# Bernat-C/MRI-Diffusion-SuperResolution

Hardware: AMD Instinct MI355X
Metric: MRI slices/sec (50-step DDIM, 256^2, bs=32) (higher is better)
Workload: dtype bf16; 1 GPU; configs[1]: 256x256 1-ch synthetic MRI slices -> 4x32x32 latents, SD-1.5-size UNet (859.5M params, random init) + rank-4 LoRA, 50-step DDIM, bs=32 per GPU; ddim_steps=50, parallelism=slice-sharded x1 (no collective), lora=explicit adapters, down-projection + rank-r update inside the projection GEMMs, tile_table=profiles/r03_tune_cache.tsv, hipgraph=True

## Files before the change

### include/mrisr.h

```cpp
#ifndef MRISR_H
#define MRISR_H
#include <stddef.h>
#include <stdint.h>

#ifdef __cplusplus
extern "C" {
#endif

typedef enum { MRISR_F32 = 0, MRISR_BF16 = 1, MRISR_F16 = 2, MRISR_I64 = 3 } mrisr_dtype;
typedef enum { MRISR_NCHW = 0, MRISR_NHWC = 1 } mrisr_layout;

typedef struct {
    void* data;
    int32_t dtype;
    int32_t layout;
    int32_t ndim;
    int64_t shape[4];
} mrisr_tensor;

typedef struct {
    int32_t in_channels;
    int32_t out_channels;
    int32_t num_levels;
    int32_t block_out_channels[4];
// ... 246 lines not shown
                        const float* bias_dev, int n, int act, mrisr_tensor* y_rows, void* stream);
int mrisr_op_groupnorm(const mrisr_tensor* x_nhwc, const mrisr_tensor* x2_nhwc, const float* gamma_dev,
                       const float* beta_dev, int groups, float eps, int silu, mrisr_tensor* y_nhwc, void* stream);
int mrisr_op_layernorm(const mrisr_tensor* x_rows, const float* gamma_dev, const float* beta_dev, float eps,
                       mrisr_tensor* y_rows, void* stream);
int mrisr_op_attention(const mrisr_tensor* q, const mrisr_tensor* k, const mrisr_tensor* v, int heads, int flash,
                       mrisr_tensor* out, void* stream);

int mrisr_op_attention_bwd(const mrisr_tensor* q, const mrisr_tensor* k, const mrisr_tensor* v, const mrisr_tensor* dout,
                           int heads, mrisr_tensor* dq, mrisr_tensor* dk, mrisr_tensor* dv, void* stream);

int mrisr_op_groupnorm_bwd(int dtype, const void* x0, int c0, const void* x1, int c1, int B, int HW, const float* gamma_dev,
                           const float* beta_dev, int groups, float eps, int silu, const void* dy, void* dx0, int acc0, void* dx1,
                           int acc1, float* g_gamma, float* g_beta, void* stream);
int mrisr_op_layernorm_bwd(int dtype, const void* x, const void* dy, void* dx, const float* gamma_dev, int M, int C, float eps,
                           int accumulate, float* g_gamma, float* g_beta, void* stream);
int mrisr_op_geglu(int dtype, int backward, const void* pre, const void* dout, void* out, int64_t M, int half, void* stream);
int mrisr_op_pointwise_bwd(int kind, int dtype, const void* a, const void* b, void* out, float* out_f32, int64_t n, int B, int H, int W,
                           int C, int flag, int ld_out, int off, void* stream);
int mrisr_op_lora_wgrad(int dtype, const void* P, int ldp, const float* Q, int ldq, int M, int C, int mode, int r, int nmod, int secN,
                        float* out0, float* out1, float* out2, float scale, void* stream);
int mrisr_op_lora_wgrad_geglu(int dtype, const void* P, int ldp, const float* Q, int ldq, int M, int half, int r, float* out, float scale,
                              void* stream);
int mrisr_op_lora_wgrad_hr(int dtype, const void* P, int ldp, const void* Q, int ldq, int M, int C, int mode, int r, int nmod, int secN,
                           float* out0, float* out1, float* out2, float scale, int geglu_half, void* stream);
int mrisr_op_dora_scale(int dtype, const float* W, const float* A, const float* B, const float* mag, float scale, float* g, void* out, int ld,
                        int n, int k, int r, int geglu_half, int merged, void* stream);
int mrisr_op_dora_mag_grad(int dtype, const void* P, int ldp, const void* Y, int ldy, const void* R, int ldr, const float* bias, const float* mag,
                           float* gm, int M, int C, int geglu_half, void* stream);
int mrisr_op_attn_identity(int dtype, const void* vt, void* out, int B, int H, int N, int hd, int npad, int dpad, int first_sample, int n_samples,
                           void* stream);
int mrisr_op_freeu(int dtype, const void* hidden, const void* skip, void* hidden_out, void* skip_out, int B, int H, int W, int Ch, int Cs,
                   float b, float s, void* stream);
int mrisr_op_transpose(int dtype, const void* src, void* dst, int R, int C, int ld_src, int ld_dst, int64_t bs_src, int64_t bs_dst,
                       int batch, int r_valid, void* stream);
int mrisr_op_softmax_bwd(int dtype, const void* p, const float* dp, void* ds, int ld, int64_t rows, int nk, float scale, void* stream);
int mrisr_op_small_dense_bwd(int dtype, int which, const float* dY, int ldy, const void* xw, int ldx, int rows, int N, int K, int silu_in,
                             const float* pre, int ldpre, float* out, float* gB, int ld_out, void* stream);
int mrisr_op_conv_wgrad(int dtype, const void* x, int xB, int xH, int xW, int cin_src, const void* dY, int ldy, int col0, int cout_src,
                        int ks, int stride, float* gW, float* gB, int cout, int cin, int geglu_half, void* stream);
int mrisr_op_conv_dgrad(int dtype, const void* dy, int B, int H, int W, int cout, const float* w_oihw_dev, int cin, int mode, void* dx,
                        int accumulate, void* stream);
int mrisr_op_conv_lora_down(int dtype, const void* x_nhwc, int B, int H, int W, int cin, const float* a_dev, int r, float* z, int route,
                            void* stream);
int mrisr_op_conv_lora_dgrad(int dtype, const float* dz, int B, int H, int W, int r, const float* a_dev, int cin, void* dx_nhwc, int accumulate,
                             void* stream);
int mrisr_op_conv3x3_lora(const mrisr_tensor* x, const float* w_oihw_dev, const float* bias_dev, const float* a_dev, const float* b_dev, int r,
                          float scale, const float* rowvec_dev, const mrisr_tensor* resid, int cout, int splitk, int tile, mrisr_tensor* y,
                          void* stream);


int mrisr_op_guided_step(int step_kind, mrisr_tensor* x, mrisr_tensor* x2, const mrisr_tensor* eps2, const mrisr_tensor* lr,
                         const mrisr_tensor* noise, const float* coef_row_host, float clip, float guidance_scale,
                         float guidance_rescale, void* stream);

int mrisr_op_pag_step(int step_kind, mrisr_tensor* x, mrisr_tensor* x3, const mrisr_tensor* eps3, const mrisr_tensor* lr,
                      const mrisr_tensor* noise, const float* coef_row_host, float clip, float guidance_scale, float pag_scale,
                      float guidance_rescale, void* stream);

int mrisr_op_pag_multistep_step(int step_kind, mrisr_tensor* x, mrisr_tensor* x3, const mrisr_tensor* eps3, const mrisr_tensor* lr,
                                mrisr_tensor* hist, mrisr_tensor* xc, const float* row_host, int solver_order, int slot, float guidance_scale,
                                float pag_scale, float guidance_rescale, void* stream);

int mrisr_op_multistep_step(int step_kind, mrisr_tensor* x, mrisr_tensor* x2, const mrisr_tensor* eps, const mrisr_tensor* lr,
                            mrisr_tensor* hist, mrisr_tensor* xc, const float* row_host, int solver_order, int slot, float guidance_scale,
                            float guidance_rescale, void* stream);
// ... 10 lines not shown
```

### include/mrisr_debug.h

```cpp
#ifndef MRISR_DEBUG_H
#define MRISR_DEBUG_H
#ifdef __cplusplus
extern "C" {
#endif

void mrisr_debug_force_split(int splitk);
void mrisr_debug_force_tile(int tile);
void mrisr_debug_prefer_tile(int tile);
void mrisr_debug_gemm_flags(int flags);
void mrisr_debug_set_tile_eff(int tile, double eff);
void mrisr_debug_set_tuned(const char* key, int tile, int splitk);
void mrisr_debug_gn_fused(int on);

int mrisr_autotune_stats(int* shapes, double* ms);
void mrisr_autotune_release(void);

int mrisr_bench_gemm(int M, int N, int K, int conv, int B, int H, int W, int stride, int ups, int c1, int tile, int splitk,
                     int iters, float* ms_out);

void mrisr_debug_sk_inkernel(int on);

void mrisr_debug_subpix(int min_rows);

void mrisr_debug_temb_table(int on);

void mrisr_debug_mlp_proj(int on);

void mrisr_debug_gn_slabs(int on);

void mrisr_debug_sc_fused(int on);

void mrisr_debug_ff_proj_fused(int on);

void mrisr_debug_xattn_tail(int on);
void mrisr_debug_xattn_tail_stamps(void* dev_buf);

int mrisr_bench_mlp(int M, int hidden, int iters, float* ms_out);

#ifdef __cplusplus
}
#endif
#endif
```

### mri-diffusion-superresolution_amd/csrc/capi_ops.hip

```cpp
#include <algorithm>
#include <cmath>
#include <cstring>
#include <memory>
#include <vector>

#include "api.h"
#include "model.h"
#include "train_ops.h"

using namespace mrisr;

namespace {
struct OpScratch {
    std::vector<std::unique_ptr<DevBuf>> bufs;
    void* alloc(size_t bytes, bool zero = false) {
        bufs.emplace_back(new DevBuf());
        if (bufs.back()->reserve(bytes ? bytes : 1, zero)) return nullptr;
        return bufs.back()->p;
    }
};
template <typename T>
int op_gemm_run(OpScratch& sc, hipStream_t st, GemmArgs& g) {
    return gemm_run<T>(g, st, false, [&sc](size_t n) { return sc.alloc(n); });
}
// ... 12 lines not shown
        const int dd = (int)(i % hd);
        const int h = (int)((i / hd) % H);
        const int tok = (int)((i / ((long long)hd * H)) % N);
        const int b = (int)(i / ((long long)hd * H * N));
        const size_t bh = (size_t)b * H + h;
        if (!tr) dst[(bh * npad + tok) * dpad + dd] = x[i];
        else dst[(bh * dpad + dd) * npad + tok] = x[i];
    }
}

template <typename T>
static int op_conv3x3_t(const mrisr_tensor* x, const mrisr_tensor* x2, const float* w, const float* bias, int cout,
                        int stride, int ups, int act, int splitk, mrisr_tensor* y, hipStream_t st) {
    const int B = (int)x->shape[0], C0 = (int)x->shape[1], H = (int)x->shape[2], W = (int)x->shape[3];
    const int C1 = x2 ? (int)x2->shape[1] : 0;
    const int Cin = C0 + C1;
    DevBuf wp, part;
    TRY(wp.reserve((size_t)cout * Cin * 9 * sizeof(T), false));
    TRY(launch_pack_conv3x3<T>(w, wp.p, cout, Cin, 3, st));
    if (!x2 && !ups && Cin % (128 / (int)sizeof(T)) != 0) {
        DirectConvArgs a;
        a.x = x->data; a.w = wp.p; a.bias = bias; a.y = y->data; a.B = B; a.Hin = H; a.Win = W; a.Cin = Cin;
        a.Hout = (H - 1) / stride + 1; a.Wout = (W - 1) / stride + 1; a.Cout = cout; a.ks = 3; a.stride = stride; a.pad = 1; a.act = act;
        MRISR_REQUIRE(y->shape[1] == cout && y->shape[2] == a.Hout && y->shape[3] == a.Wout, "conv output shape");
        TRY(launch_direct_conv<T>(a, st));
        MRISR_CHECK_HIP(hipStreamSynchronize(st));
        return 0;
    }
    if (ups == 2) {
        MRISR_REQUIRE(sizeof(T) == 2 && !x2 && stride == 1 && act == ACT_NONE && (4 * Cin) % 64 == 0 && cout % 8 == 0, "sub-pixel upsample conv: bf16, single source");
        MRISR_REQUIRE(y->shape[1] == cout && y->shape[2] == 2 * H && y->shape[3] == 2 * W, "conv output shape");
        DevBuf sp, planes;
        TRY(sp.reserve((size_t)16 * cout * Cin * sizeof(T), false));
        TRY(planes.reserve((size_t)4 * B * H * W * cout * sizeof(T), false));
        TRY(launch_pack_conv_subpix<T>(w, sp.p, cout, Cin, st));
        GemmArgs g;
        ga_rows(g, x->data, C0, C0); ga_conv3(g, B, H, W); g.kw = 2; g.subpix = 1;
        ga_batch(g, 4, 0, (long long)cout * 4 * Cin, (long long)B * H * W * cout); ga_weight(g, sp.p, B * H * W, cout, 4 * Cin);
        g.bias = bias; ga_out(g, planes.p, cout);
        TRY(gemm_run<T>(g, st, false, devbuf_alloc(part)));
        TRY(launch_subpix_shuffle<T>(planes.p, y->data, B, H, W, cout, st));
        MRISR_CHECK_HIP(hipStreamSynchronize(st));
        return 0;
    }
    GemmArgs g;
    ga_rows(g, x->data, C0, C0);
    if (x2) ga_rows2(g, x2->data, C1, C1);
    ga_conv3(g, B, H, W, stride, ups);
    MRISR_REQUIRE(y->shape[1] == cout && y->shape[2] == g.Hout && y->shape[3] == g.Wout, "conv output shape");
    ga_weight(g, wp.p, B * g.Hout * g.Wout, cout, 9 * Cin); g.bias = bias; g.act = act; ga_out(g, y->data, cout);
    TRY(op_plan<T>(g, splitk, false, part));
    TRY(launch_gemm<T>(g, st));
    MRISR_CHECK_HIP(hipStreamSynchronize(st));
    return 0;
}

extern "C" void mrisr_debug_force_tile(int t);
struct ForcedTile {
    explicit ForcedTile(int t) { mrisr_debug_force_tile(t); }
    ~ForcedTile() { mrisr_debug_force_tile(0); }
    ForcedTile(const ForcedTile&) = delete;
    ForcedTile& operator=(const ForcedTile&) = delete;
};

static int op_conv3x3_sc_t(const mrisr_tensor* x, const mrisr_tensor* x2, const float* w, const float* bias, const mrisr_tensor* xs,
                           const mrisr_tensor* xs2, const float* w_sc, const float* bias_sc, int cout, int splitk, int tile, int fused,
                           mrisr_tensor* y, hipStream_t st) {
    typedef bf16 T;
    const int B = (int)x->shape[0], C0 = (int)x->shape[1], H = (int)x->shape[2], W = (int)x->shape[3];
    const int C1 = x2 ? (int)x2->shape[1] : 0, Cin = C0 + C1;
    const int S0 = (int)xs->shape[1], S1 = xs2 ? (int)xs2->shape[1] : 0, Cs = S0 + S1;
    MRISR_REQUIRE(xs->shape[0] == B && xs->shape[2] == H && xs->shape[3] == W && (!xs2 || (xs2->shape[0] == B && xs2->shape[2] == H && xs2->shape[3] == W)),
                  "shortcut sources: the conv input's batch and image size");
    MRISR_REQUIRE(y->shape[1] == cout && y->shape[2] == H && y->shape[3] == W, "conv output shape");
// ... 826 lines not shown
    hipStream_t st = (hipStream_t)stream;
    MRISR_REQUIRE(src && dst && R >= 1 && C >= 1 && batch >= 1 && batch <= 65535, "transpose: null / empty operand");
    MRISR_REQUIRE(ld_src >= C && ld_dst >= R && r_valid >= 0 && r_valid <= R, "transpose: pitches cover the rows, r_valid <= R");
    MRISR_REQUIRE(batch == 1 || (bs_src >= (long long)(R - 1) * ld_src + C && bs_dst >= (long long)(C - 1) * ld_dst + R),
                  "transpose: batch strides cover one matrix");
    TRY(BWD_DISPATCH(dtype, launch_transpose, src, dst, R, C, ld_src, ld_dst, (long long)bs_src, (long long)bs_dst, batch, r_valid, st));
    MRISR_CHECK_HIP(hipStreamSynchronize(st));
    return 0;
    API_END
}

int mrisr_op_attn_identity(int dtype, const void* vt, void* out, int B, int H, int N, int hd, int npad, int dpad, int first_sample, int n_samples,
                           void* stream) {
    API_BEGIN
    TRY(bwd_dtype_ok(dtype));
    hipStream_t st = (hipStream_t)stream;
    TRY(BWD_DISPATCH(dtype, launch_attn_identity, vt, out, B, H, N, hd, npad, dpad, first_sample, n_samples, st));
    MRISR_CHECK_HIP(hipStreamSynchronize(st));
    return 0;
    API_END
}

int mrisr_op_freeu(int dtype, const void* hidden, const void* skip, void* hidden_out, void* skip_out, int B, int H, int W, int Ch, int Cs, float b,
                   float s, void* stream) {
    API_BEGIN
    TRY(bwd_dtype_ok(dtype));
    hipStream_t st = (hipStream_t)stream;
    TRY(BWD_DISPATCH(dtype, launch_freeu, hidden, skip, hidden_out, skip_out, B, H, W, Ch, Cs, b, s, st));
    MRISR_CHECK_HIP(hipStreamSynchronize(st));
    return 0;
    API_END
}

int mrisr_op_softmax_bwd(int dtype, const void* p, const float* dp, void* ds, int ld, int64_t rows, int nk, float scale, void* stream) {
    API_BEGIN
    TRY(bwd_dtype_ok(dtype));
    hipStream_t st = (hipStream_t)stream;
    MRISR_REQUIRE(p && dp && ds && rows >= 1 && nk >= 1 && nk <= ld, "softmax backward: null / empty operand, nk <= ld");
    MRISR_REQUIRE(ld % 4 != 0 || ld > 4096 || (al16(p) && al16(dp) && al16(ds)), "softmax backward: aligned rows for the vector kernel");
    TRY(BWD_DISPATCH(dtype, launch_softmax_bwd, p, dp, ds, ld, (long long)rows, nk, scale, st));
    MRISR_CHECK_HIP(hipStreamSynchronize(st));
    return 0;
    API_END
}

int mrisr_op_small_dense_bwd(int dtype, int which, const float* dY, int ldy, const void* xw, int ldx, int rows, int N, int K, int silu_in,
                             const float* pre, int ldpre, float* out, float* gB, int ld_out, void* stream) {
    API_BEGIN
    TRY(bwd_dtype_ok(dtype));
    hipStream_t st = (hipStream_t)stream;
    MRISR_REQUIRE(dY && xw && out && (which == 0 || which == 1), "small dense backward: null operand, which 0 / 1");
    MRISR_REQUIRE(rows >= 1 && rows <= 64 && N >= 1 && K >= 1 && ldy >= N, "small dense backward: 1..64 rows, dY pitch covers N");
    if (which == 0) {
        MRISR_REQUIRE(ldx >= K, "small wgrad: X pitch covers K");
        TRY(launch_small_wgrad(dY, ldy, static_cast<const float*>(xw), ldx, rows, N, K, silu_in ? 1 : 0, out, gB, st));
    } else {
        MRISR_REQUIRE(ld_out >= K && (!pre || ldpre >= K), "small dgrad: dX / pre pitches cover K");
        TRY(BWD_DISPATCH(dtype, launch_small_dgrad, dY, ldy, xw, rows, N, K, pre, ldpre, out, ld_out, st));
    }
    MRISR_CHECK_HIP(hipStreamSynchronize(st));
    return 0;
    API_END
}

int mrisr_op_conv_wgrad(int dtype, const void* x, int xB, int xH, int xW, int cin_src, const void* dY, int ldy, int col0, int cout_src,
                        int ks, int stride, float* gW, float* gB, int cout, int cin, int geglu_half, void* stream) {
// ... 216 lines not shown
```

### mri-diffusion-superresolution_amd/csrc/common.h

```cpp
#pragma once
#include <hip/hip_runtime.h>
#include <stdint.h>
#include <string>

#include "lora_hr.h"

namespace mrisr {

typedef __bf16 bf16;
typedef __attribute__((ext_vector_type(8))) __bf16 bf16x8;
typedef __attribute__((ext_vector_type(4))) __bf16 bf16x4;
typedef __attribute__((ext_vector_type(4))) float f32x4;
typedef __attribute__((ext_vector_type(16))) float f32x16;

enum DType : int { DT_F32 = 0, DT_BF16 = 1, DT_F16 = 2, DT_I64 = 3 };

template <typename T> struct TypeTag;
template <> struct TypeTag<float> { static constexpr int id = DT_F32; };
template <> struct TypeTag<bf16> { static constexpr int id = DT_BF16; };

__device__ __forceinline__ float to_f32(float x) { return x; }
__device__ __forceinline__ float to_f32(bf16 x) { return (float)x; }
template <typename T> __device__ __forceinline__ T from_f32(float x);
template <> __device__ __forceinline__ float from_f32<float>(float x) { return x; }
// ... 38 lines not shown
        hipError_t _e = (expr);                                                                    \
        if (_e != hipSuccess) {                                                                    \
            ::mrisr::set_error(std::string(#expr) + ": " + hipGetErrorString(_e));                 \
            return 1;                                                                              \
        }                                                                                          \
    } while (0)
#define MRISR_REQUIRE(cond, msg)                                                                   \
    do {                                                                                           \
        if (!(cond)) {                                                                             \
            ::mrisr::set_error(std::string("requirement failed: ") + #cond + " - " + (msg));       \
            return 2;                                                                              \
        }                                                                                          \
    } while (0)

enum GemmAct : int { ACT_NONE = 0, ACT_RELU = 1, ACT_SILU = 2, ACT_GEGLU = 3 };
enum GemmOut : int { OUT_ROWS = 0, OUT_HEADS = 1, OUT_F32 = 2, OUT_NONE = 3  };

struct GemmArgs {
    const void* a0 = nullptr;
    const void* a1 = nullptr;
    int c0 = 0, c1 = 0;
    int lda0 = 0, lda1 = 0;
    int conv = 0;
    int B = 0, Hin = 0, Win = 0, Hout = 0, Wout = 0, stride = 1, ups = 0;
    int pad = 1;
    int zstuff = 0;
    const void* s0 = nullptr;
    const void* s1 = nullptr;
    int cs0 = 0, cs1 = 0;
    int lds0 = 0, lds1 = 0;
    const void* w = nullptr;
    int M = 0, N = 0, K = 0;
    int kw = 3, subpix = 0;
    int batch = 1;
    long long a_bs = 0, w_bs = 0;
    int heads = 1;
    long long o_bs = 0, o_hs = 0;
    int splitk = 1;
    float* partial = nullptr;
    unsigned* sk_counters = nullptr;
    int defer_reduce = 0;
    int pretouch = 0;
    float alpha = 1.0f;
    const float* bias = nullptr;
    const float* rowvec = nullptr;
    int rowvec_div = 1, rowvec_ld = 0;
    int act = ACT_NONE;
    const void* resid = nullptr;
    int ldr = 0;
    int out_mode = OUT_ROWS;
    void* out = nullptr;
    int ldo = 0;
    void* sec_ptr[3] = {nullptr, nullptr, nullptr};
    int sec_tr[3] = {0, 0, 0};
    int secC = 0, hd = 0, dpad = 0, ntok = 0, npad = 0, nheads = 0;
    double alg_flops = 0.0, alg_bytes = 0.0;
    int tile = 0;
    int stage_out = 1;
    const float* lora_z = nullptr;
    const float* lora_b = nullptr;
    int lora_r = 0, lora_zld = 0, lora_secN = 1;
    const void* lora_a = nullptr;
    int lora_R = 0;
    float* lora_zout = nullptr;
    const float* ln_gamma = nullptr;
    const float* ln_beta = nullptr;
// ... 17 lines not shown
    const float* ln_gamma = nullptr; const float* ln_beta = nullptr; float ln_eps = 1e-5f;
    const void* w1 = nullptr; const float* b1 = nullptr;
    const void* w2p = nullptr; const float* b2 = nullptr;
    const void* resid = nullptr; int ldr = 0;
    void* out = nullptr; int ldo = 0;
    int C = 0, H = 0, N2 = 0;
    const void* wp = nullptr; const float* bp = nullptr;
    const void* xres = nullptr; int ldxr = 0;
    void* out2 = nullptr; int ldo2 = 0;
};
bool mlp_fused_ok(int C, int H, int N2);
bool mlp_proj_enabled();
int launch_pack_mlp_w2(const void* w2_bf16, void* dst, int N2, int H, hipStream_t st);
int launch_mlp_fused(const MlpArgs& m, hipStream_t st);
struct XTailArgs {
    const void* ao = nullptr; int ldao = 0;
    void* t = nullptr; int ldt = 0;
    int M = 0, ntok = 0;
    const void* w1 = nullptr; const float* b1 = nullptr; const void* a1 = nullptr; const float* lb1 = nullptr;
    const float* ln_g = nullptr; const float* ln_b = nullptr; float ln_eps = 1e-5f;
    const void* wq = nullptr; const float* bq = nullptr; const void* aq = nullptr; const float* lbq = nullptr;
    const void* kvp = nullptr; int nk = 0; float scale = 1.f;
    const void* w2 = nullptr; const float* b2 = nullptr; const void* a2 = nullptr; const float* lb2 = nullptr;
    int lora_r = 0;
};
int xattn_tail_prepare();
bool xattn_tail_enabled();
bool xattn_tail_ok(int C, int heads, int M, int ntok, int nk);
size_t xattn_tail_kv_bytes(int B);
int launch_pack_xattn_kv(const void* kc, const void* vtc, void* dst, int B, int ctx_pad, int dpad, int nk, hipStream_t st);
int launch_xattn_tail(const XTailArgs& x, hipStream_t st);
bool gemm_tile_lora_in_kernel(int tile, int r, int R);
int gemm_rp_tile(const GemmArgs& g);
bool gemm_sc_tail_ok(const GemmArgs& g);
bool sc_fused_enabled();
bool ff_proj_fused_enabled();
int gemm_choose(GemmArgs& g, bool is_bf16);

struct GroupNormArgs {
    const void* x0 = nullptr;
    const void* x1 = nullptr;
    int c0 = 0, c1 = 0;
    int B = 0, HW = 0, groups = 32;
    float eps = 1e-5f;
    const float* gamma = nullptr;
    const float* beta = nullptr;
    int silu = 0;
    void* y = nullptr;
    float* partial = nullptr;
    int nsplit = 1;
};
extern int g_plan_salt;
int groupnorm_nsplit(int B, int HW);
struct GnSlabSrc {
    const float* partial = nullptr;
    int splitk = 1;
    float alpha = 1.f;
    const float* bias = nullptr;
    const float* rowvec = nullptr;
    int rowvec_ld = 0, rowvec_div = 1;
    const void* resid = nullptr;
    int ldr = 0;
    void* raw_out = nullptr;
};
bool groupnorm_slabs_ok(int C, int groups, int HW);
int launch_groupnorm_slabs(const GroupNormArgs& a, const GnSlabSrc& s, hipStream_t st);
bool gn_fused_geometry(int c0, int c1, int groups, int HW, int* slab, int* slots, int* rl, int* nv, int ve = 8);
template <typename T> int launch_groupnorm(const GroupNormArgs& a, hipStream_t st);
template <typename T>
int launch_layernorm(const void* x, void* y, const float* gamma, const float* beta, int M, int C, float eps,
                     hipStream_t st);
template <typename T>
int launch_softmax_rows(const float* s, int ld, void* p, int ldp, long long rows, int nk, hipStream_t st);

struct GroupNormBwdArgs {
    const void* x0 = nullptr;
    const void* x1 = nullptr;
    int c0 = 0, c1 = 0, B = 0, HW = 0, groups = 32;
    float eps = 1e-5f;
    const float* gamma = nullptr;
    const float* beta = nullptr;
    int silu = 0;
    const void* dy = nullptr;
    void* dx0 = nullptr;
    void* dx1 = nullptr;
    int acc0 = 0, acc1 = 0;
    const float* fwd_partial = nullptr;
    float* bwd_partial = nullptr;
    int nsplit = 1;
};
template <typename T> int launch_groupnorm_bwd(const GroupNormBwdArgs& a, hipStream_t st);
template <typename T>
int launch_layernorm_bwd(const void* x, const void* dy, void* dx, const float* gamma, int M, int C, float eps, int accumulate,
                         hipStream_t st);
template <typename T> int launch_geglu_bwd(const void* pre, const void* dout, void* dpre, long long M, int half, hipStream_t st);
template <typename T> int launch_geglu_fwd(const void* pre, void* out, long long M, int half, hipStream_t st);
template <typename T>
int launch_rows_to_heads(const void* x, int ldx, int col_off, void* dst, int B, int N, int H, int hd, int npad, int dpad, hipStream_t st);
// ... 95 lines not shown
    void* dv = nullptr;
    int ldq = 0, ldkv = 0;
    int B = 0, H = 0, nq = 0, nk = 0, npad = 0, nkpad = 0, hd = 0, dpad = 0;
    float scale = 1.0f;
};
int launch_attention_bwd_bf16(const AttnBwdArgs& a, hipStream_t st);
int launch_attention_bwd_prep(const void* dO_rows, const void* O_rows, void* doh, float* dsum, int B, int N, int H, int hd, int npad,
                              int dpad, hipStream_t st);

template <typename T>
int launch_gemv_rows(const float* x, int ldx, const void* w, const float* bias, float* y, int ldy, int rows, int N,
                     int K, int silu_in, hipStream_t st, int f32_inputs = 0);
template <typename T>
int launch_lora_down(const void* x, int ldx, const void* A, float* z, int M, int K, int R, hipStream_t st);
int conv_lora_kpad(int R);
size_t conv_lora_down_scratch_bytes(int M, int cin, int R, int elem_size, int route = 0);
template <typename T>
int launch_conv_lora_down(const void* x, const void* A, float* z, int B, int H, int W, int cin, int R, float* scratch, hipStream_t st, int route = 0);
template <typename T>
int launch_conv_lora_dgrad(const float* dz, const void* A, const void* bank, void* dx, int B, int H, int W, int cin, int R, int accumulate,
                           hipStream_t st);
template <typename T>
int launch_conv_lora_pack(const float* A, const float* Bm, float s, void* Av, void* bank, float* sB, void* sBT, int cin, int cout, int r, hipStream_t st);
template <typename T> int launch_cast_rows(const float* src, void* dst, long long n, hipStream_t st);
int launch_timestep_embedding(const long long* t, int t_is_scalar, float* out, int rows, int dim, hipStream_t st);
int launch_select_row(const float* table, const int* step, int first, float* out, int n, hipStream_t st);
struct DirectConvArgs {
    const void* x = nullptr;
    const void* w = nullptr;
    const float* bias = nullptr;
    void* y = nullptr;
    int B = 0, Hin = 0, Win = 0, Cin = 0, Hout = 0, Wout = 0, Cout = 0, ks = 3, stride = 1, pad = 1, act = 0;
    const void* add = nullptr;
};
template <typename T> int launch_direct_conv(const DirectConvArgs& a, hipStream_t st);
int direct_conv_prepare();
template <typename T>
int launch_nchw_to_nhwc(const void* src, int src_dtype, void* dst, int B, int C, int H, int W, hipStream_t st);
template <typename T>
int launch_nhwc_to_nchw(const void* src, void* dst, int dst_dtype, int B, int C, int H, int W, float scale,
                        hipStream_t st);
template <typename T> int launch_add_inplace(void* x, const void* y, long long n, hipStream_t st);
template <typename T> int launch_scale_inplace(void* p, float s, long long n, hipStream_t st);
template <typename T> int launch_pixel_unshuffle_nchw(const void* src, int src_dtype, void* dst, int B, int C, int H,
                                                      int W, int r, hipStream_t st);
template <typename T>
int launch_pack_rows(const float* src, int rows, int cols, void* dst, int ld_dst, int row_off, int col_off,
                     int row_map, int half, float scale, hipStream_t st);
template <typename T>
int launch_pack_conv3x3(const float* src, void* dst, int Cout, int Cin, int ks, hipStream_t st);
template <typename T>
int launch_pack_conv_subpix(const float* src, void* dst, int Cout, int Cin, hipStream_t st);
template <typename T>
int launch_subpix_shuffle(const void* planes, void* out, int B, int H, int W, int C, hipStream_t st);
template <typename T>
int launch_pack_conv3x3_padded(const float* src, void* dst, int Cout, int Cin, int ks, int Cout_pad, int Cin_pad, hipStream_t st);
int launch_pack_bias_geglu(const float* src, float* dst, int half, hipStream_t st);
int launch_compose_ff_proj(const float* wp, const float* w2, const float* b2, const float* bp, void* dst_bf16, int ld_dst, float* bias_dst,
                           int C, int K4, hipStream_t st);
template <typename T> int launch_fill_zero(void* p, long long n, hipStream_t st);
int launch_quant_rows_fp8(const void* src_bf16, int rows, int cols, void* dst8, float* scales, hipStream_t st);

int launch_ddim_step(float* x, const float* eps, const float* coef_table, const int* step_idx, long long n,
                     hipStream_t st);
int launch_ddpm_step(float* x, const float* eps, const float* noise, const float* coef_table, const int* step_idx, float clip,
                     long long n, hipStream_t st);
int launch_resshift_step(float* x, const float* eps, const float* lr, const float* noise, const float* coef_table,
                         const int* step_idx, long long n, hipStream_t st);
// ... 23 lines not shown
```

### mri-diffusion-superresolution_amd/csrc/gemm.hip

```cpp
#include "common.h"
#include "prof.h"

#include <cstdio>
#include <cstdlib>
#include <cstring>
#include <map>
#include <mutex>
#include <unordered_map>

namespace mrisr {

static void* g_zero_page = nullptr;
static constexpr size_t kZeroPageBytes = 128 * 1024;
const void* zero_page() { return g_zero_page; }
int init_zero_page() {
    if (g_zero_page) return 0;
    MRISR_CHECK_HIP(hipMalloc(&g_zero_page, kZeroPageBytes));
    MRISR_CHECK_HIP(hipMemset(g_zero_page, 0, kZeroPageBytes));
    return 0;
}

typedef const __attribute__((address_space(1))) void* gptr_t;
typedef __attribute__((address_space(3))) void* lptr_t;

// ... 385 lines not shown
    preload_cols<NF>(g, n0 + wn0 + fg * 4, pb);
    if (g.act == ACT_GEGLU) {
#pragma unroll
        for (int i = 0; i < NF; i += 2)
#pragma unroll
            for (int j = 0; j < MF; ++j) {
                const int m = m0 + wm0 + j * 16 + fr;
                const int n = n0 + wn0 + i * 16 + fg * 4;
                if (m < g.M && n < g.N) {
                    float v[4] = {acc[i][j][0], acc[i][j][1], acc[i][j][2], acc[i][j][3]};
                    float vg[4] = {acc[i + 1][j][0], acc[i + 1][j][1], acc[i + 1][j][2], acc[i + 1][j][3]};
                    epilogue4<T>(g, z, m, n, v, vg, nullptr, nullptr, false, true, nullptr, 0, 0, 0, pb[i], pb[i + 1 < NF ? i + 1 : i]);
                }
            }
        return;
    }
#pragma unroll
    for (int i = 0; i < NF; ++i)
#pragma unroll
        for (int j = 0; j < MF; ++j) {
            const int m = m0 + wm0 + j * 16 + fr;
            const int n = n0 + wn0 + i * 16 + fg * 4;
            if (m < g.M && n < g.N) {
                float v[4] = {acc[i][j][0], acc[i][j][1], acc[i][j][2], acc[i][j][3]};
                epilogue4<T>(g, z, m, n, v, nullptr, nullptr, nullptr, false, true, nullptr, 0, 0, 0, pb[i]);
            }
        }
}

template <int BM, int BN, int NT = 256>
__device__ __forceinline__ void copy_out_tile(const GemmArgs& g, const bf16* otile, int pitch, int m0, int n0, int z, bool add_resid) {
    __syncthreads();
    constexpr int CPR = BN / 8;
    bf16* out = reinterpret_cast<bf16*>(g.out) + (size_t)z * g.o_bs;
    const bf16* res = add_resid ? reinterpret_cast<const bf16*>(g.resid) + (size_t)z * g.o_bs : nullptr;
    constexpr int TOTAL = BM * CPR, IT = (TOTAL + NT - 1) / NT, BATCH = IT < 5 ? IT : 5;
    for (int it0 = 0; it0 < IT; it0 += BATCH) {
        bf16x8 rv[BATCH];
#pragma unroll
        for (int u = 0; u < BATCH; ++u) {
            const int idx = (int)threadIdx.x + (it0 + u) * NT;
            const int row = idx / CPR, ch = idx - row * CPR;
            const int m = m0 + row, n = n0 + ch * 8;
            if (res && idx < TOTAL && m < g.M && n + 8 <= g.N) rv[u] = *reinterpret_cast<const bf16x8*>(res + (size_t)m * g.ldr + n);
        }
#pragma unroll
        for (int u = 0; u < BATCH; ++u) {
            const int idx = (int)threadIdx.x + (it0 + u) * NT;
            const int row = idx / CPR, ch = idx - row * CPR;
            const int m = m0 + row, n = n0 + ch * 8;
            if (idx >= TOTAL || m >= g.M || n >= g.N) continue;
            const bf16* src = otile + row * pitch + ch * 8;
            bf16* dst = out + (size_t)m * g.ldo + n;
            if (n + 8 <= g.N) {
                bf16x8 v = *reinterpret_cast<const bf16x8*>(src);
                if (res) {
#pragma unroll
                    for (int e = 0; e < 8; ++e) v[e] = (bf16)((float)v[e] + (float)rv[u][e]);
                }
                *reinterpret_cast<bf16x8*>(dst) = v;
            } else {
                bf16x4 v = *reinterpret_cast<const bf16x4*>(src);
                if (res) {
                    const bf16x4 r = *reinterpret_cast<const bf16x4*>(res + (size_t)m * g.ldr + n);
#pragma unroll
                    for (int e = 0; e < 4; ++e) v[e] = (bf16)((float)v[e] + (float)r[e]);
                }
                *reinterpret_cast<bf16x4*>(dst) = v;
            }
        }
    }
}

template <int BM, int BN>
__device__ __forceinline__ void copy_out_heads(const GemmArgs& g, const bf16* otile, int m0, int n0, bool tr) {
    __syncthreads();
    const int s = n0 / g.secC;
    bf16* base = reinterpret_cast<bf16*>(s == 0 ? g.sec_ptr[0] : (s == 1 ? g.sec_ptr[1] : g.sec_ptr[2]));
    if (!tr) {
        constexpr int CPR = BN / 8, P = BN + 8;
        for (int idx = threadIdx.x; idx < BM * CPR; idx += 256) {
            const int row = idx / CPR, ch = idx - row * CPR;
            const int m = m0 + row, n = n0 + ch * 8;
            if (m >= g.M || n >= g.N) continue;
            const int c = n - s * g.secC, h = c / g.hd, dd = c - h * g.hd;
            const int b = m / g.ntok, tok = m - b * g.ntok;
// ... 2611 lines not shown
#define TILE_PREPARE_HALO(a, b, c, d, e) 0
#define TILE_PREPARE_HALO8(a, b, c, d, e) 0
#define TILE_PREPARE_WS(a, b, c, d, e) 0
#define TILE_PREPARE_RP(a, b, c, d, e) 0
#define X(id, fam, a, b, c, d, e, eff, cand) if (TILE_PREPARE_##fam(a, b, c, d, e)) return 1;
    TILES(X)
#undef X
    if (direct_conv_prepare()) return 1;
    if (xattn_tail_prepare()) return 1;
    return mlp_fused_prepare();
}

static long long tile_count(const GemmArgs& g) { return (long long)((g.M + 63) / 64) * ((g.N + 63) / 64); }
static constexpr int kSkCounters = 16384;
static int g_sk_inkernel = -1;
extern "C" void mrisr_debug_sk_inkernel(int on) { g_sk_inkernel = on; }
static std::mutex g_sk_mu;
static std::unordered_map<hipStream_t, unsigned*> g_sk_map;
static unsigned* sk_counters_for(hipStream_t st) {
    static const int env = [] { const char* e = getenv("MRISR_SK_INKERNEL"); return e ? atoi(e) : 0; }();
    if (g_sk_inkernel < 0 ? !env : !g_sk_inkernel) return nullptr;
    std::lock_guard<std::mutex> lk(g_sk_mu);
    auto it = g_sk_map.find(st);
    if (it != g_sk_map.end()) return it->second;
    hipStreamCaptureStatus cs = hipStreamCaptureStatusNone;
    if (st && (hipStreamIsCapturing(st, &cs) != hipSuccess || cs != hipStreamCaptureStatusNone)) return nullptr;
    unsigned* p = nullptr;
    if (hipMalloc(&p, kSkCounters * sizeof(unsigned)) != hipSuccess) return nullptr;
    if (hipMemset(p, 0, kSkCounters * sizeof(unsigned)) != hipSuccess || hipDeviceSynchronize() != hipSuccess) { (void)hipFree(p); return nullptr; }
    g_sk_map[st] = p;
    return p;
}

template <typename T>
int launch_gemm(const GemmArgs& g_in, hipStream_t st) {
    constexpr bool is_bf16 = sizeof(T) == 2;
    constexpr int BK = 128 / (int)sizeof(T);
    GemmArgs g = g_in;
    MRISR_REQUIRE(g.K % BK == 0, "K must be a multiple of the 128-byte K tile");
    MRISR_REQUIRE(g.N % 4 == 0, "N must be a multiple of 4");
    MRISR_REQUIRE(g.c0 % BK == 0 && g.c1 % BK == 0, "channel extents must be multiples of the K tile");
    MRISR_REQUIRE(g.splitk == 1 || g.partial != nullptr, "split-K needs a partial buffer");
    MRISR_REQUIRE(g.splitk == 1 || g.act != ACT_GEGLU, "GEGLU epilogue cannot be split");
    MRISR_REQUIRE(zero_page() != nullptr, "zero page not initialised");
    if (g.conv) { MRISR_REQUIRE(g.K == g.kw * g.kw * (g.c0 + g.c1) + g.cs0 + g.cs1 && (g.kw == 3 || g.kw == 2), "conv K"); }
    else { MRISR_REQUIRE(g.K == g.c0 + g.c1, "plain K"); }
    if (g.kw != 3 || g.subpix) {
        MRISR_REQUIRE(is_bf16 && g.conv && !g.c1 && g.stride == 1 && !g.ups && !g.zstuff && g.splitk == 1 && (!g.subpix || g.batch == 4),
                      "2 x 2 / sub-pixel conv: bf16 buffer-addressed kernels, single source, stride 1, un-split, four parity batches");
    }
    int tile = g.tile ? g.tile : g_force_tile, s;
    if (!tile) plan(g, is_bf16, g.splitk, &tile, &s);
    tile = tile_for_launch(g, is_bf16, tile);
    const char* why = nullptr;
    MRISR_REQUIRE(tile_admits(g, is_bf16, tile, &why), why);
    static const int stage_env = [] { const char* e = getenv("MRISR_STAGE_OUT"); return e ? atoi(e) : 2; }();
    g.stage_out = stage_env;
    g.dbg = g_gemm_flags;
    {
        static const int on = [] { const char* e = getenv("MRISR_PRETOUCH"); return e ? atoi(e) : 1; }();
        static const long long min_b = [] { const char* e = getenv("MRISR_PRETOUCH_MIN_KB"); return (e ? atoll(e) : 512ll) * 1024; }();
        static const int cap = [] { const char* e = getenv("MRISR_PRETOUCH_CAP"); return e ? atoi(e) : 32; }();
        g.pretouch = (on && is_bf16 && g.batch == 1 && (long long)g.N * g.K * 2 >= min_b) ? cap : 0;
    }
    g.sk_counters = nullptr;
    if (g.splitk > 1 && is_bf16 && !g.defer_reduce && find_tile(tile)->reduces_in_kernel() && !g.cs0) {
        const long long ntiles = tile_count(g) * (long long)g.batch;
        if (ntiles > 0 && ntiles <= kSkCounters) g.sk_counters = sk_counters_for(st);
    }
    int rc = 1;
    switch (tile) {
#define X(id, fam, a, b, c, d, e, eff, cand) case id: rc = TILE_LAUNCH_##fam(a, b, c, d, e)(g, st); break;
        TILES(X)
#undef X
    }
    if (rc) return rc;
    if (g.splitk > 1 && !g.sk_counters && !g.defer_reduce) return launch_splitk_reduce<T>(g, st);
    return 0;
}

template <typename T>
int launch_splitk_reduce(const GemmArgs& g, hipStream_t st) {
    const long long total = (long long)g.M * (g.N / 4);
    int blocks = (int)((total + 255) / 256);
    if (blocks > 4096) blocks = 4096;
    ProfScope ps("splitk_reduce", 0.0, (double)g.batch * g.M * g.N * (4.0 * g.splitk + sizeof(T)), st);
    hipLaunchKernelGGL(splitk_reduce_kernel<T>, dim3(blocks, 1, g.batch), dim3(256), 0, st, g);
    MRISR_CHECK_HIP(hipGetLastError());
    return 0;
}

template int launch_gemm<float>(const GemmArgs&, hipStream_t);
template int launch_gemm<bf16>(const GemmArgs&, hipStream_t);
template int launch_splitk_reduce<float>(const GemmArgs&, hipStream_t);
template int launch_splitk_reduce<bf16>(const GemmArgs&, hipStream_t);

}
```

### mri-diffusion-superresolution_amd/csrc/misc.hip

```cpp
#include "common.h"
#include "prof.h"

namespace mrisr {

__device__ __forceinline__ float wsum(float v) {
#pragma unroll
    for (int o = 32; o > 0; o >>= 1) v += __shfl_xor(v, o);
    return v;
}

template <typename T, int RB>
__global__ __launch_bounds__(256) void gemv_rows_kernel(const float* __restrict__ x, int ldx,
                                                        const T* __restrict__ w, const float* __restrict__ bias,
                                                        float* __restrict__ y, int ldy, int rows, int N, int K,
                                                        int silu_in) {
    constexpr int VE = 16 / (int)sizeof(T);
    const int lane = threadIdx.x & 63;
    const int n = blockIdx.x * 4 + (threadIdx.x >> 6);
    if (n >= N) return;
    for (int r0 = 0; r0 < rows; r0 += RB) {
        float acc[RB];
#pragma unroll
        for (int r = 0; r < RB; ++r) acc[r] = 0.f;
        for (int k = lane * VE; k < K; k += 64 * VE) {
// ... 372 lines not shown
        }
    }
}

__global__ __launch_bounds__(256) void conv_in_mfma_kernel(const DirectConvArgs a) {
    extern __shared__ __attribute__((aligned(16))) char sm_raw[];
    bf16* wl = reinterpret_cast<bf16*>(sm_raw);
    const int OP = a.Cout + 8;
    bf16* ot = wl + (size_t)a.Cout * 40 + (size_t)(threadIdx.x >> 6) * 16 * OP;
    float* bl = reinterpret_cast<float*>(wl + (size_t)a.Cout * 40 + (size_t)4 * 16 * OP);
    const bf16* x = reinterpret_cast<const bf16*>(a.x);
    const bf16* w = reinterpret_cast<const bf16*>(a.w);
    bf16* y = reinterpret_cast<bf16*>(a.y);
    for (int i = threadIdx.x; i < a.Cout * 10; i += 256) {
        const int n = i / 10, j = i - n * 10;
        const uint2 v = j < 9 ? *reinterpret_cast<const uint2*>(w + (size_t)n * 36 + j * 4) : make_uint2(0u, 0u);
        *reinterpret_cast<uint2*>(wl + (size_t)n * 40 + j * 4) = v;
    }
    for (int i = threadIdx.x; i < a.Cout; i += 256) bl[i] = a.bias ? a.bias[i] : 0.f;
    __syncthreads();
    const int lane = threadIdx.x & 63, fr = lane & 15, fg = lane >> 4;
    const int M = a.B * a.Hout * a.Wout;
    const int ngroups = (M + 15) / 16;
    const int NFR = a.Cout / 16, CPR = a.Cout / 8;
    for (int pg = blockIdx.x * 4 + (threadIdx.x >> 6); pg < ngroups; pg += gridDim.x * 4) {
        const int m = pg * 16 + fr;
        bf16x8 af0 = bf16x8{0, 0, 0, 0, 0, 0, 0, 0}, af1 = af0;
        if (m < M) {
            const int ox = m % a.Wout, oy = (m / a.Wout) % a.Hout, b = m / (a.Wout * a.Hout);
            auto tap4 = [&](int t) -> uint2 {
                const int ky = t / 3, kx = t - ky * 3;
                const int iy = oy + ky - 1, ix = ox + kx - 1;
                if (iy < 0 || iy >= a.Hin || ix < 0 || ix >= a.Win) return make_uint2(0u, 0u);
                return *reinterpret_cast<const uint2*>(x + (((size_t)b * a.Hin + iy) * a.Win + ix) * 4);
            };
            const uint2 p0 = tap4(fg * 2), p1 = tap4(fg * 2 + 1);
            af0 = __builtin_bit_cast(bf16x8, make_uint4(p0.x, p0.y, p1.x, p1.y));
            if (fg == 0) {
                const uint2 p8 = tap4(8);
                af1 = __builtin_bit_cast(bf16x8, make_uint4(p8.x, p8.y, 0u, 0u));
            }
        }
        for (int i = 0; i < NFR; ++i) {
            const bf16* wr = wl + (size_t)(i * 16 + fr) * 40;
            const bf16x8 wf0 = *reinterpret_cast<const bf16x8*>(wr + fg * 8);
            bf16x8 wf1 = bf16x8{0, 0, 0, 0, 0, 0, 0, 0};
            if (fg == 0) wf1 = *reinterpret_cast<const bf16x8*>(wr + 32);
            f32x4 acc = f32x4{0.f, 0.f, 0.f, 0.f};
            acc = __builtin_amdgcn_mfma_f32_16x16x32_bf16(wf0, af0, acc, 0, 0, 0);
            acc = __builtin_amdgcn_mfma_f32_16x16x32_bf16(wf1, af1, acc, 0, 0, 0);
            const int n = i * 16 + fg * 4;
            const f32x4 b4 = *reinterpret_cast<const f32x4*>(bl + n);
            bf16x4 ad = bf16x4{0, 0, 0, 0};
            if (a.add && m < M) ad = *reinterpret_cast<const bf16x4*>(reinterpret_cast<const bf16*>(a.add) + (size_t)m * a.Cout + n);
            bf16x4 o;
#pragma unroll
            for (int r = 0; r < 4; ++r) {
                float v = acc[r] + b4[r];
                if (a.act == ACT_SILU) v = silu_f(v);
                else if (a.act == ACT_RELU) v = fmaxf(v, 0.f);
                o[r] = (bf16)(v + (float)ad[r]);
            }
            *reinterpret_cast<bf16x4*>(ot + fr * OP + n) = o;
        }
        asm volatile("s_waitcnt lgkmcnt(0)" ::: "memory");
        __builtin_amdgcn_wave_barrier();
        for (int c = lane; c < 16 * CPR; c += 64) {
            const int row = c / CPR, col = (c - row * CPR) * 8;
            const int mo = pg * 16 + row;
            if (mo >= M) continue;
            *reinterpret_cast<bf16x8*>(y + (size_t)mo * a.Cout + col) = *reinterpret_cast<const bf16x8*>(ot + row * OP + col);
        }
        asm volatile("s_waitcnt lgkmcnt(0)" ::: "memory");
        __builtin_amdgcn_wave_barrier();
    }
}

int direct_conv_prepare() {
    static bool done = false;
    if (!done) {
        MRISR_CHECK_HIP(hipFuncSetAttribute((const void*)conv_in_mfma_kernel, hipFuncAttributeMaxDynamicSharedMemorySize, 80 * 1024));
        done = true;
    }
    return 0;
}

template <typename T>
int launch_direct_conv(const DirectConvArgs& a, hipStream_t st) {
    const size_t wbytes = (size_t)a.ks * a.ks * a.Cin * a.Cout * sizeof(T);
    if (sizeof(T) == 2 && a.ks == 3 && a.Cin == 4 && a.stride == 1 && a.pad == 1 && a.Cout % 16 == 0 && a.Hout == a.Hin && a.Wout == a.Win) {
        const size_t smem = ((size_t)a.Cout * 40 + (size_t)4 * 16 * (a.Cout + 8)) * 2 + (size_t)a.Cout * 4;
        if (smem <= 80 * 1024 && (long long)a.B * a.Hout * a.Wout * a.Cout < (1ll << 31)) {
            if (direct_conv_prepare()) return 1;
            const long long M = (long long)a.B * a.Hout * a.Wout;
            long long blocks = ((M + 15) / 16 + 3) / 4;
            if (blocks > 256) blocks = 256;
            ProfScope ps("conv_in_mfma", 2.0 * M * a.Cout * 36, 2.0 * (M * 4.0 + (double)M * a.Cout), st);
            hipLaunchKernelGGL(conv_in_mfma_kernel, dim3((unsigned)blocks), dim3(256), smem, st, a);
            MRISR_CHECK_HIP(hipGetLastError());
            return 0;
        }
    }
    if (a.Cout % 8 == 0 && wbytes <= 48 * 1024) {
        const long long items = (long long)a.B * a.Hout * a.Wout * (a.Cout / 8);
        long long blocks = (items + 255) / 256;
        if (blocks > 2048) blocks = 2048;
        ProfScope ps("small_conv", 2.0 * items * 8 * a.ks * a.ks * a.Cin,
                     sizeof(T) * ((double)a.B * a.Hin * a.Win * a.Cin + (double)items * 8), st);
        hipLaunchKernelGGL(small_conv_kernel<T>, dim3((unsigned)blocks), dim3(256), wbytes, st, a);
        MRISR_CHECK_HIP(hipGetLastError());
        return 0;
    }
    const long long total = (long long)a.B * a.Hout * a.Wout * a.Cout;
    long long blocks = (total + 255) / 256;
    if (blocks > 65535 * 4) blocks = 65535 * 4;
    ProfScope ps("direct_conv", 2.0 * total * a.ks * a.ks * a.Cin,
                 sizeof(T) * ((double)a.B * a.Hin * a.Win * a.Cin + (double)total), st);
    hipLaunchKernelGGL(direct_conv_kernel<T>, dim3((unsigned)blocks), dim3(256), 0, st, a);
    MRISR_CHECK_HIP(hipGetLastError());
    return 0;
}


__device__ __forceinline__ float load_any(const void* p, int dt, size_t i) {
// ... 340 lines not shown
```

### mri-diffusion-superresolution_amd/csrc/norm.hip

```cpp
#include "common.h"
#include "prof.h"

namespace mrisr {

template <typename T> struct Vec;
template <> struct Vec<bf16> {
    static constexpr int N = 8;
    typedef bf16x8 type;
};
template <> struct Vec<float> {
    static constexpr int N = 4;
    typedef f32x4 type;
};

template <typename T, int VPT>
__global__ __launch_bounds__(256) void gn_stats_kernel(const GroupNormArgs a, int slots, int RL) {
    constexpr int VE = Vec<T>::N;
    typedef typename Vec<T>::type vec_t;
    extern __shared__ float sm[];
    const int C = a.c0 + a.c1;
    const int b = blockIdx.y, sp = blockIdx.x;
    const int tid = threadIdx.x;
    const int slot = tid % slots, rl = tid / slots;
    const int rows_per = (a.HW + a.nsplit - 1) / a.nsplit;
// ... 133 lines not shown
template <int NVM, int VE, bool SLAB = false, int NT = 256>
__global__ __launch_bounds__(NT) void gn_fused_kernel(const GroupNormArgs a, int slab, int slots, int RL, int nslab, int xcd_map, const GnSlabSrc ss = GnSlabSrc()) {
    typedef bf16 T;
    typedef __attribute__((ext_vector_type(VE))) __bf16 vec_t;
    __shared__ float part[NT * 16];
    __shared__ float seg[2 * 1280];
    __shared__ double gsum[2 * 80];
    __shared__ float mean_s[80], rstd_s[80];
    const int C = a.c0 + a.c1;
    const int Cg = C / a.groups;
    int b, sl;
    if (xcd_map) {
        const int L = blockIdx.x;
        b = (L & 7) + 8 * (L / (8 * nslab));
        sl = (L >> 3) % nslab;
    } else {
        b = blockIdx.x / nslab;
        sl = blockIdx.x - b * nslab;
    }
    const int ch0 = sl * slab;
    const int tid = threadIdx.x;
    const int slot = tid % slots, rl = tid / slots;
    const bool active = rl < RL;
    const int ch = ch0 + slot * VE;
    const T* src;
    int ld;
    if (ch < a.c0) { src = reinterpret_cast<const T*>(a.x0) + (size_t)b * a.HW * a.c0 + ch; ld = a.c0; }
    else { src = reinterpret_cast<const T*>(a.x1) + (size_t)b * a.HW * a.c1 + (ch - a.c0); ld = a.c1; }
    vec_t xv[NVM];
    float s1[VE], s2[VE];
#pragma unroll
    for (int e = 0; e < VE; ++e) s1[e] = s2[e] = 0.f;
    if (active) {
        if constexpr (SLAB) {
            typedef __attribute__((ext_vector_type(VE))) float fvec_t;
            const size_t MN = (size_t)a.B * a.HW * C;
            fvec_t bv;
#pragma unroll
            for (int e = 0; e < VE; ++e) bv[e] = 0.f;
            if (ss.bias) bv = *reinterpret_cast<const fvec_t*>(ss.bias + ch);
#pragma unroll
            for (int i = 0; i < NVM; ++i) {
                const int r = rl + i * RL;
                if (r < a.HW) {
                    const size_t mrow = (size_t)b * a.HW + r;
                    const float* pp = ss.partial + mrow * C + ch;
                    fvec_t v;
#pragma unroll
                    for (int e = 0; e < VE; ++e) v[e] = 0.f;
                    for (int sp = 0; sp < ss.splitk; ++sp) {
                        const fvec_t t = *reinterpret_cast<const fvec_t*>(pp + (size_t)sp * MN);
#pragma unroll
                        for (int e = 0; e < VE; ++e) v[e] += t[e];
                    }
#pragma unroll
                    for (int e = 0; e < VE; ++e) v[e] = v[e] * ss.alpha + bv[e];
                    if (ss.rowvec) {
                        const fvec_t t = *reinterpret_cast<const fvec_t*>(ss.rowvec + (mrow / ss.rowvec_div) * ss.rowvec_ld + ch);
#pragma unroll
                        for (int e = 0; e < VE; ++e) v[e] += t[e];
                    }
                    if (ss.resid) {
                        const vec_t t = *reinterpret_cast<const vec_t*>(reinterpret_cast<const T*>(ss.resid) + mrow * ss.ldr + ch);
#pragma unroll
                        for (int e = 0; e < VE; ++e) v[e] += (float)t[e];
                    }
#pragma unroll
                    for (int e = 0; e < VE; ++e) xv[i][e] = (bf16)v[e];
                    if (ss.raw_out) *reinterpret_cast<vec_t*>(reinterpret_cast<T*>(ss.raw_out) + mrow * C + ch) = xv[i];
                }
            }
        } else {
#pragma unroll
        for (int i = 0; i < NVM; ++i) {
            const int r = rl + i * RL;
            if (r < a.HW) xv[i] = *reinterpret_cast<const vec_t*>(src + (size_t)r * ld);
        }
        }
#pragma unroll
        for (int i = 0; i < NVM; ++i) {
            if (rl + i * RL < a.HW) {
#pragma unroll
                for (int e = 0; e < VE; ++e) {
                    const float f = (float)xv[i][e];
                    s1[e] += f;
                    s2[e] += f * f;
                }
            }
        }
    }
#pragma unroll
    for (int e = 0; e < VE; ++e) {
        part[tid * 16 + e] = s1[e];
        part[tid * 16 + 8 + e] = s2[e];
    }
    __syncthreads();
    const int nout = 2 * slab;
    int nseg = NT / nout;
    if (nseg < 1) nseg = 1;
    if (nseg > RL) nseg = RL;
    const int seg_len = (RL + nseg - 1) / nseg;
    for (int t = tid; t < nout * nseg; t += NT) {
// ... 167 lines not shown
            }
#undef GN_GO
            MRISR_CHECK_HIP(hipGetLastError());
            return 0;
        }
    }
    {
    ProfScope ps(prof_intern(n1), 0.0, act_bytes, st);
    switch (vpt) {
        case 1: hipLaunchKernelGGL((gn_stats_kernel<T, 1>), grid, dim3(256), smem, st, a, slots, RL); break;
        case 2: hipLaunchKernelGGL((gn_stats_kernel<T, 2>), grid, dim3(256), smem, st, a, slots, RL); break;
        case 3: hipLaunchKernelGGL((gn_stats_kernel<T, 3>), grid, dim3(256), smem, st, a, slots, RL); break;
        default: hipLaunchKernelGGL((gn_stats_kernel<T, 4>), grid, dim3(256), smem, st, a, slots, RL); break;
    }
    }
    MRISR_CHECK_HIP(hipGetLastError());
    int bx = 1024 / (a.B > 0 ? a.B : 1) + 1;
    int rows_per_block = (a.HW + bx - 1) / bx;
    if (rows_per_block < RL) rows_per_block = RL;
    bx = (a.HW + rows_per_block - 1) / rows_per_block;
    ProfScope ps2(prof_intern(n2), 0.0, 2.0 * act_bytes, st);
    switch (vpt) {
        case 1: hipLaunchKernelGGL((gn_apply_kernel<T, 1>), dim3(bx, a.B), dim3(256), 0, st, a, slots, RL, rows_per_block); break;
        case 2: hipLaunchKernelGGL((gn_apply_kernel<T, 2>), dim3(bx, a.B), dim3(256), 0, st, a, slots, RL, rows_per_block); break;
        case 3: hipLaunchKernelGGL((gn_apply_kernel<T, 3>), dim3(bx, a.B), dim3(256), 0, st, a, slots, RL, rows_per_block); break;
        default: hipLaunchKernelGGL((gn_apply_kernel<T, 4>), dim3(bx, a.B), dim3(256), 0, st, a, slots, RL, rows_per_block); break;
    }
    MRISR_CHECK_HIP(hipGetLastError());
    return 0;
}

static int g_gn_slabs = -1;
extern "C" void mrisr_debug_gn_slabs(int on) { g_gn_slabs = on; ++g_plan_salt; }
static bool gn_slabs_geometry(int C, int groups, int HW, int B, int* ve, int* slab, int* slots, int* rl, int* nv) {
    if (!gn_fused_geometry(C, 0, groups, HW, slab, slots, rl, nv, 8)) return false;
    *ve = 8;
    int s4 = 0, sl4 = 0, rl4 = 0, nv4 = 0;
    if (B * (C / *slab) < 512 && gn_fused_geometry(C, 0, groups, HW, &s4, &sl4, &rl4, &nv4, 4) && C / s4 > C / *slab) {
        *ve = 4; *slab = s4; *slots = sl4; *rl = rl4; *nv = nv4;
    }
    return *nv <= 8;
}
bool groupnorm_slabs_ok(int C, int groups, int HW) {
    static const int env = [] { const char* e = getenv("MRISR_GN_SLABS"); return e ? atoi(e) : 1; }();
    if (g_gn_slabs < 0 ? !env : !g_gn_slabs) return false;
    if (C % groups || groups > 64 || C % 8) return false;
    int ve, slab, slots, rl, nv;
    return gn_slabs_geometry(C, groups, HW, 32, &ve, &slab, &slots, &rl, &nv);
}
int launch_groupnorm_slabs(const GroupNormArgs& a, const GnSlabSrc& s, hipStream_t st) {
    const int C = a.c0;
    MRISR_REQUIRE(a.c1 == 0 && a.x1 == nullptr && C % a.groups == 0 && a.groups <= 64 && C % 8 == 0, "GroupNorm from slabs: one source, whole groups");
    MRISR_REQUIRE(s.partial && s.splitk >= 1 && a.partial != nullptr && a.nsplit >= 1 && (!s.rowvec || s.rowvec_div >= 1) && (!s.resid || s.ldr % 8 == 0), "GroupNorm from slabs: operands");
    int ve, slab, slots, rl, nv;
    MRISR_REQUIRE(gn_slabs_geometry(C, a.groups, a.HW, a.B, &ve, &slab, &slots, &rl, &nv), "GroupNorm from slabs: geometry (groupnorm_slabs_ok)");
    const int nslab = C / slab;
    const int xmap = (a.B % 8) == 0 ? 1 : 0;
    std::string nf = "groupnorm_from_slabs";
    if (prof_enabled() && prof_shapes()) {
        char buf[96];
        snprintf(buf, sizeof(buf), " B=%d HW=%d C=%d s=%d", a.B, a.HW, C, s.splitk);
        nf += buf;
    }
    const double act_bytes = (double)a.B * a.HW * C * 2.0;
    ProfScope ps(prof_intern(nf), 0.0, act_bytes * (2.0 * s.splitk + 1.0 + (s.raw_out ? 1.0 : 0.0) + (s.resid ? 1.0 : 0.0)), st);
    const dim3 fg(a.B * nslab);
#define GNS_GO(NV, VEV) hipLaunchKernelGGL((gn_fused_kernel<NV, VEV, true>), fg, dim3(256), 0, st, a, slab, slots, rl, nslab, xmap, s)
    if (ve == 8) { if (nv <= 2) GNS_GO(2, 8); else if (nv <= 4) GNS_GO(4, 8); else GNS_GO(8, 8); }
    else { if (nv <= 2) GNS_GO(2, 4); else if (nv <= 4) GNS_GO(4, 4); else GNS_GO(8, 4); }
#undef GNS_GO
    MRISR_CHECK_HIP(hipGetLastError());
    return 0;
}

__device__ __forceinline__ float wave_sum(float v) {
#pragma unroll
    for (int o = 32; o > 0; o >>= 1) v += __shfl_xor(v, o);
    return v;
}
__device__ __forceinline__ float wave_max(float v) {
#pragma unroll
    for (int o = 32; o > 0; o >>= 1) v = fmaxf(v, __shfl_xor(v, o));
    return v;
}

template <typename T, int MAXV>
__global__ __launch_bounds__(256) void layernorm_kernel(const T* __restrict__ x, T* __restrict__ y,
                                                        const float* __restrict__ gamma,
                                                        const float* __restrict__ beta, int M, int C, float eps) {
    constexpr int VE = Vec<T>::N;
    typedef typename Vec<T>::type vec_t;
    const int lane = threadIdx.x & 63;
    const int row = blockIdx.x * 4 + (threadIdx.x >> 6);
    if (row >= M) return;
    const int nvec = C / VE;
    float v[MAXV][VE];
    float s = 0.f;
#pragma unroll
// ... 228 lines not shown
```

### mri-diffusion-superresolution_amd/csrc/runner.h

```cpp
#pragma once
#include <climits>
#include <cmath>
#include <cstdlib>

#include "api.h"
#include "gemm_args.h"
#include "model.h"

namespace mrisr {

extern int g_subpix_override;

inline bool fuse_ln() {
    static int v = -1;
    if (v < 0) { const char* e = getenv("MRISR_FUSE_LN"); v = (e && e[0] == '0') ? 0 : 1; }
    return v == 1;
}
inline bool lora_in_kernel() {
    static int v = -1;
    if (v < 0) { const char* e = getenv("MRISR_LORA_INKERNEL"); v = (e && e[0] == '0') ? 0 : 1; }
    return v == 1;
}

template <typename T>
struct Runner {
    Model& m;
    hipStream_t st;
    bool dry;
    Runner(Model& mm, hipStream_t s, bool d) : m(mm), st(s), dry(d) {}

    void* alloc(size_t bytes) {
        void* p = m.arena.alloc(bytes);
        if (!p) set_error("workspace arena exhausted");
        return p;
    }
    Act new_act(int B, int H, int W, int C) {
        Act a;
        a.B = B; a.H = H; a.W = W; a.C = C;
        a.p = alloc(a.numel() * sizeof(T));
        return a;
    }

    int gn(const Act& x0, const Act* x1, const NormW& nw, bool silu, float eps, Act* out, float** partial_out = nullptr,
           int* nsplit_out = nullptr) {
        const int C = x0.C + (x1 ? x1->C : 0);
        MRISR_REQUIRE(nw.c == C, "GroupNorm channel mismatch");
        *out = new_act(x0.B, x0.H, x0.W, C);
        GroupNormArgs a;
        a.x0 = x0.p; a.c0 = x0.C;
        a.x1 = x1 ? x1->p : nullptr; a.c1 = x1 ? x1->C : 0;
        a.B = x0.B; a.HW = x0.H * x0.W; a.groups = m.cfg.norm_num_groups; a.eps = eps;
        a.gamma = nw.g; a.beta = nw.b; a.silu = silu ? 1 : 0; a.y = out->p;
        a.nsplit = groupnorm_nsplit(a.B, a.HW);
        a.partial = static_cast<float*>(alloc((size_t)a.B * a.nsplit * a.groups * 2 * sizeof(float)));
        if (!out->p || !a.partial) return 7;
        if (partial_out) *partial_out = a.partial;
        if (nsplit_out) *nsplit_out = a.nsplit;
        if (dry) return 0;
        return launch_groupnorm<T>(a, st);
    }

    auto arena_alloc() { return [this](size_t n) { return alloc(n); }; }
    int run_gemm(GemmArgs& g) { return gemm_run<T>(g, st, dry, arena_alloc()); }

    int conv3(const Act& x, const Act* x1, const ConvW& cw, int stride, int ups, const float* rowvec, int rowvec_ld,
              int rowvec_div, const Act* resid, int act, Act* out, const float* lz = nullptr) {
        const int Cin = x.C + (x1 ? x1->C : 0);
        MRISR_REQUIRE(cw.cin == Cin && cw.ks == 3, "conv3x3 weight mismatch");
        GemmArgs g = conv3_args(x, x1, cw, stride, ups, rowvec, rowvec_ld, rowvec_div, resid, act);
        *out = new_act(x.B, g.Hout, g.Wout, cw.cout);
        if (!out->p) return 7;
        g.out = out->p;
        if (lz) ga_lora_epilogue(g, cw, lz);
        return run_gemm(g);
    }
    static GemmArgs conv3_args(const Act& x, const Act* x1, const ConvW& cw, int stride, int ups, const float* rowvec, int rowvec_ld,
                               int rowvec_div, const Act* resid, int act) {
        GemmArgs g;
        ga_rows(g, x); ga_rows2(g, x1); ga_conv3(g, x, stride, ups);
        ga_weight(g, cw.w, x.B * g.Hout * g.Wout, cw.cout, 9 * (x.C + (x1 ? x1->C : 0))); g.bias = cw.b; g.act = act;
        ga_rowvec(g, rowvec, rowvec_ld, rowvec_div); ga_resid(g, resid); g.ldo = cw.cout;
        return g;
    }
    int conv_lora_z(const Act& x, const ConvW& cw, float** z) {
        MRISR_REQUIRE(cw.r && cw.loraA && cw.loraB && x.C == cw.cin, "conv LoRA: adapter views");
        const int M = (int)x.rows();
        *z = static_cast<float*>(alloc((size_t)M * cw.r * sizeof(float)));
        const size_t sb = conv_lora_down_scratch_bytes(M, x.C, cw.r, (int)sizeof(T));
        float* scr = sb ? static_cast<float*>(alloc(sb)) : nullptr;
        if (!*z || (sb && !scr)) return 7;
        if (dry) return 0;
        return launch_conv_lora_down<T>(x.p, cw.loraA, *z, x.B, x.H, x.W, x.C, cw.r, scr, st);
    }

    int conv3_gn(const Act& x, const Act* x1, const ConvW& cw, const float* rowvec, int rowvec_ld, int rowvec_div, const Act* resid,
                 const NormW& nw, bool silu, float eps, Act* raw, Act* out) {
        const int Cin = x.C + (x1 ? x1->C : 0);
        MRISR_REQUIRE(cw.cin == Cin && cw.ks == 3 && nw.c == cw.cout, "conv3x3 + GroupNorm weight mismatch");
        GemmArgs g = conv3_args(x, x1, cw, 1, 0, rowvec, rowvec_ld, rowvec_div, resid, ACT_NONE);
        bool fuse = sizeof(T) == 2 && !m.keep && groupnorm_slabs_ok(cw.cout, m.cfg.norm_num_groups, x.H * x.W);
        if (fuse) {
            g.out = kUnallocated;
            TRY(gemm_choose(g, true));
            fuse = g.splitk > 1;
        }
        if (!fuse) {
            Act h;
            TRY(conv3(x, x1, cw, 1, 0, rowvec, rowvec_ld, rowvec_div, resid, ACT_NONE, &h));
            if (raw) *raw = h;
            return gn(h, nullptr, nw, silu, eps, out);
        }
        Act h;
        h.B = x.B; h.H = x.H; h.W = x.W; h.C = cw.cout; h.p = nullptr;
        if (raw) { h = new_act(x.B, x.H, x.W, cw.cout); if (!h.p) return 7; *raw = h; }
        *out = new_act(x.B, x.H, x.W, cw.cout);
        if (!out->p) return 7;
        GroupNormArgs a;
        a.x0 = nullptr; a.c0 = cw.cout; a.B = x.B; a.HW = x.H * x.W; a.groups = m.cfg.norm_num_groups; a.eps = eps;
        a.gamma = nw.g; a.beta = nw.b; a.silu = silu ? 1 : 0; a.y = out->p;
        a.nsplit = groupnorm_nsplit(a.B, a.HW);
        a.partial = static_cast<float*>(alloc((size_t)a.B * a.nsplit * a.groups * 2 * sizeof(float)));
        TRY(gemm_alloc_partial(g, arena_alloc()));
        if (!a.partial) return 7;
        if (dry) return 0;
        g.defer_reduce = 1;
        TRY(launch_gemm<T>(g, st));
        GnSlabSrc ss;
        ss.partial = g.partial; ss.splitk = g.splitk; ss.alpha = g.alpha; ss.bias = g.bias; ss.rowvec = g.rowvec; ss.rowvec_ld = g.rowvec_ld;
        ss.rowvec_div = g.rowvec_div; ss.resid = g.resid; ss.ldr = g.ldr; ss.raw_out = h.p;
        return launch_groupnorm_slabs(a, ss, st);
    }

    static int subpix_min_rows() {
        static const int v = [] { const char* e = getenv("MRISR_SUBPIX"); return e ? atoi(e) : 2048; }();
        return g_subpix_override >= 0 ? g_subpix_override : v;
    }
    int upsample_conv(const Act& x, const Level& lv, Act* out) {
        const int minr = subpix_min_rows();
        if (!(sizeof(T) == 2 && lv.up_sp && !m.keep && minr > 0 && (long long)x.rows() >= minr))
            return conv3(x, nullptr, lv.up, 1, 1, nullptr, 0, 1, nullptr, ACT_NONE, out);
        const ConvW& cw = lv.up;
        MRISR_REQUIRE(cw.cin == x.C, "upsampler weight mismatch");
        *out = new_act(x.B, 2 * x.H, 2 * x.W, cw.cout);
        if (!out->p) return 7;
        const size_t mk = m.arena.mark();
        const long long plane = (long long)x.rows() * cw.cout;
        T* planes = static_cast<T*>(alloc((size_t)4 * plane * sizeof(T)));
        if (!planes) return 7;
        GemmArgs g;
        ga_rows(g, x); ga_conv3(g, x); g.kw = 2; g.subpix = 1; ga_batch(g, 4, 0, (long long)cw.cout * 4 * cw.cin, plane);
        ga_weight(g, lv.up_sp, (int)x.rows(), cw.cout, 4 * x.C); g.bias = cw.b; ga_out(g, planes, cw.cout);
        g.alg_flops = 2.0 * 4.0 * g.M * (double)g.N * g.K;
        TRY(run_gemm(g));
        if (!dry) TRY(launch_subpix_shuffle<T>(planes, out->p, x.B, x.H, x.W, cw.cout, st));
        m.arena.release(mk);
        return 0;
    }

    int linear(const void* x, int M, int lda, const LinW& lw, int act, const void* resid, int ldr, GemmArgs* custom,
               void* out, int ldo, float** z_out = nullptr, const NormW* ln = nullptr, void* ln_scratch = nullptr) {
        GemmArgs g = custom ? *custom : GemmArgs();
        const size_t mk = m.arena.mark();
        ga_rows(g, x, lw.k, lda); ga_weight(g, lw.w, M, lw.n, lw.k); g.alg_flops = 2.0 * M * (double)lw.n * (lw.k + lw.r);
        g.bias = lw.b; g.act = act; ga_resid(g, resid, ldr);
        if (g.out_mode != OUT_HEADS) ga_out(g, out, ldo);
        if (lw.R && !(lw.r == 4 && lw.R <= 16 && lora_in_kernel())) g.no_rp = 1;
        if (lw.w8 && sizeof(T) == 2 && (!m.keep || m.cfg.fp8_train) && !g.no_rp) {
            GemmArgs probe = g;
            probe.w8 = lw.w8; probe.w_scale = lw.w_scale;
            if (lw.R) { probe.lora_a = lw.loraA; probe.lora_b = lw.loraB; probe.lora_r = lw.r; probe.lora_R = lw.R; probe.lora_a8 = lw.loraA8; probe.lora_a_scale = lw.loraA_scale; }
            if (gemm_rp_tile(probe)) { g.w8 = lw.w8; g.w_scale = lw.w_scale; g.lora_a8 = lw.loraA8; g.lora_a_scale = lw.loraA_scale; }
        }
        if (ln) {
            MRISR_REQUIRE(ln->c == lw.k && lda == lw.k, "LayerNorm width vs the projection's K");
            GemmArgs probe = g;
            if (lw.R) { probe.lora_a = lw.loraA; probe.lora_b = lw.loraB; probe.lora_r = lw.r; probe.lora_R = lw.R; }
            if (sizeof(T) == 2 && !m.keep && fuse_ln() && (!lw.R || (lw.R <= 16 && lora_in_kernel())) && gemm_rp_tile(probe)) {
                g.ln_gamma = ln->g; g.ln_beta = ln->b; g.ln_eps = 1e-5f;
            } else {
                MRISR_REQUIRE(ln_scratch, "LayerNorm scratch rows");
                TRY(layernorm(x, *ln, M, lw.k, ln_scratch));
                g.a0 = x = ln_scratch;
            }
        }
        if (!lw.R) {
// ... 51 lines not shown
        TRY(conv3(t->xn, nullptr, r.c1, 1, 0, m.tproj_out + r.temb_off, m.tproj_total, div, nullptr, ACT_NONE, &t->h, t->z1));
        TRY(gn(t->h, nullptr, r.n2, true, m.cfg.norm_eps, &t->hn, &t->p2, &t->ns2));
        Act res = x;
        if (r.has_sc) {
            GemmArgs g = resnet_shortcut_args(x, x1, r.sc.w, r.sc.b, r.cin, r.cout, o.p);
            TRY(run_gemm(g));
            res = o;
        } else {
            MRISR_REQUIRE(!x1, "concat input requires a shortcut conv");
        }
        if (r.c2.r) TRY(conv_lora_z(t->hn, r.c2, &t->z2));
        GemmArgs g = resnet_conv2_args(t->hn.p, x.B, x.H, x.W, r.cout, r.c2.w, r.c2.b, res.p, o.p);
        if (t->z2) ga_lora_epilogue(g, r.c2, t->z2);
        return run_gemm(g);
    }

    int resnet(const ResW& r, const Act& x, const Act* x1, Act* out, const NormW* next = nullptr, float next_eps = 0.f, Act* next_out = nullptr) {
        Act o = new_act(x.B, x.H, x.W, r.cout);
        if (!o.p) return 7;
        if (next_out) next_out->p = nullptr;
        if (r.c1.r || r.c2.r) {
            const size_t mk0 = m.arena.mark();
            ResTape t;
            TRY(resnet_literal(r, x, x1, o, &t));
            if (!m.keep) m.arena.release(mk0);
            *out = o;
            return 0;
        }
        GemmArgs g2;
        bool fuse2 = false;
        GroupNormArgs a2;
        GemmArgs gt = resnet_conv2_args(kUnallocated, x.B, x.H, x.W, r.cout, r.c2sc, r.b2sc, nullptr, o.p, r.cin, &x, x1);
        const bool sc_tail = sizeof(T) == 2 && !m.keep && r.has_sc && r.c2sc && sc_fused_enabled() && x.C + (x1 ? x1->C : 0) == r.cin && gemm_sc_tail_ok(gt);
        if (next && next_out && sizeof(T) == 2 && !m.keep && next->c == r.cout && groupnorm_slabs_ok(r.cout, m.cfg.norm_num_groups, x.H * x.W)) {
            g2 = sc_tail ? gt
                         : resnet_conv2_args(kUnallocated, x.B, x.H, x.W, r.cout, r.c2.w, r.c2.b, kUnallocated, kUnallocated);
            TRY(gemm_choose(g2, true));
            fuse2 = g2.splitk > 1;
            if (fuse2) {
                *next_out = new_act(x.B, x.H, x.W, r.cout);
                a2.nsplit = groupnorm_nsplit(x.B, x.H * x.W);
                a2.partial = static_cast<float*>(alloc((size_t)x.B * a2.nsplit * m.cfg.norm_num_groups * 2 * sizeof(float)));
                if (!next_out->p || !a2.partial) return 7;
            }
        }
        const size_t mk = m.arena.mark();
        Act xn, h, hn;
        TRY(gn(x, x1, r.n1, true, m.cfg.norm_eps, &xn));
        const int div = m.t_scalar ? INT_MAX : x.H * x.W;
        TRY(conv3_gn(xn, nullptr, r.c1, m.tproj_out + r.temb_off, m.tproj_total, div, nullptr, r.n2, true, m.cfg.norm_eps, nullptr, &hn));
        Act res = x;
        if (sc_tail) {
            res.p = nullptr;
        } else if (r.has_sc) {
            GemmArgs g = resnet_shortcut_args(x, x1, r.sc.w, r.sc.b, r.cin, r.cout, o.p);
            MRISR_REQUIRE(r.sc.R == 0, "shortcut has no LoRA");
            TRY(run_gemm(g));
            res = o;
        } else {
            MRISR_REQUIRE(!x1, "concat input requires a shortcut conv");
        }
        if (fuse2) {
            g2.a0 = hn.p; g2.resid = res.p; g2.out = o.p;
            TRY(gemm_alloc_partial(g2, arena_alloc()));
            if (!dry) {
                g2.defer_reduce = 1;
                TRY(launch_gemm<T>(g2, st));
                a2.x0 = nullptr; a2.c0 = r.cout; a2.B = x.B; a2.HW = x.H * x.W; a2.groups = m.cfg.norm_num_groups; a2.eps = next_eps;
                a2.gamma = next->g; a2.beta = next->b; a2.silu = 0; a2.y = next_out->p;
                GnSlabSrc ss;
                ss.partial = g2.partial; ss.splitk = g2.splitk; ss.alpha = g2.alpha; ss.bias = g2.bias; ss.resid = res.p; ss.ldr = r.cout; ss.raw_out = o.p;
                TRY(launch_groupnorm_slabs(a2, ss, st));
            }
        } else if (sc_tail) {
            gt.a0 = hn.p;
            TRY(run_gemm(gt));
        } else {
            GemmArgs g = resnet_conv2_args(hn.p, x.B, x.H, x.W, r.cout, r.c2.w, r.c2.b, res.p, o.p);
            TRY(run_gemm(g));
        }
        if (!m.keep) m.arena.release(mk);
        *out = o;
        return 0;
    }

    static AttnGeom attn_geom(const HeadBuf& hb, int nk, int nkpad) {
        AttnGeom s;
        s.B = hb.B; s.H = hb.H; s.N = hb.N; s.npad = hb.npad; s.hd = hb.hd; s.dpad = hb.dpad; s.nk = nk; s.nkpad = nkpad;
        return s;
    }
    int attention(const HeadBuf& hb, const void* k, const void* vt, int nk, int nkpad, void* out_rows) {
        const AttnGeom s = attn_geom(hb, nk, nkpad);
        const size_t mk = m.arena.mark();
        if (m.cfg.flash_attention && sizeof(T) == 2) {
            const bool fp8 = m.cfg.fp8_attention;
            AttnArgs a;
            TRY(attn_flash_args(a, s, hb.q, k, vt, out_rows, nullptr, fp8, arena_alloc()));
            const int rc = attn_flash_launch(a, fp8, dry, st);
            if (!m.keep) m.arena.release(mk);
            return rc;
        }
        const size_t cnt = (size_t)s.B * s.H * s.N * nkpad;
        float* S = static_cast<float*>(alloc(cnt * sizeof(float)));
        if (!S) return 7;
        void* P = S;
        if (sizeof(T) == 2) {
// ... 27 lines not shown
    void heads_args(GemmArgs* g, const HeadBuf& hb, void* s0, int tr0, void* s1, int tr1, void* s2, int tr2, int ntok,
                    int npad) {
        g->out_mode = OUT_HEADS;
        g->sec_ptr[0] = s0; g->sec_ptr[1] = s1; g->sec_ptr[2] = s2;
        g->sec_tr[0] = tr0; g->sec_tr[1] = tr1; g->sec_tr[2] = tr2;
        g->secC = hb.H * hb.hd; g->hd = hb.hd; g->dpad = hb.dpad; g->ntok = ntok; g->npad = npad; g->nheads = hb.H;
    }

    int project_context(XfW& x, const HeadBuf& hb) {
        GemmArgs g;
        heads_args(&g, hb, x.kc, 0, x.vtc, 1, nullptr, 0, m.ctx_len, m.ctx_pad);
        TRY(linear(m.ctx_rows, m.ws_B * m.ctx_len, m.cfg.cross_attention_dim, x.kv2, ACT_NONE, nullptr, 0, &g,
                   nullptr, 0));
        if (x.kvp && !dry && m.ctx_len <= 80 && hb.hd == 40 && sizeof(T) == 2)
            TRY(launch_pack_xattn_kv(x.kc, x.vtc, x.kvp, m.ws_B, m.ctx_pad, hb.dpad, m.ctx_len, st));
        return 0;
    }

    bool fused_middle(const XfW& xw, const HeadBuf& hb, int M) const {
        if (sizeof(T) != 2 || m.keep || !xw.q2p || !xw.kvp || !xattn_tail_enabled() || m.cfg.fp8_attention || !m.cfg.flash_attention) return false;
        if (!xattn_tail_ok(xw.C, hb.H, M, hb.N, m.ctx_len) || hb.hd != 40) return false;
        const int R = xw.out1.R;
        if (xw.q2.R != R || xw.out2.R != R) return false;
        if (R && !(R == 4 && xw.out1.r == 4 && xw.q2.r == 4 && xw.out2.r == 4 && lora_in_kernel())) return false;
        if (xw.out1.w8 || xw.q2.w8 || xw.out2.w8) return false;
        return true;
    }

    int transformer(XfW& xw, const Act& x, Act* out, const Act* pre_normed = nullptr) {
        const int C = xw.C, M = (int)x.rows();
        const HeadBuf& hb = m.head_buf(x.H * x.W, C);
        Act o = new_act(x.B, x.H, x.W, C);
        if (!o.p) return 7;
        const size_t mk = m.arena.mark();
        Act xn;
        if (pre_normed && pre_normed->p) xn = *pre_normed;
        else TRY(gn(x, nullptr, xw.norm, false, 1e-6f, &xn));
        T* t = static_cast<T*>(alloc((size_t)M * C * sizeof(T)));
        T* nrm = static_cast<T*>(alloc((size_t)M * C * sizeof(T)));
        T* ao = static_cast<T*>(alloc((size_t)M * C * sizeof(T)));
        if (!t || !nrm || !ao) return 7;
        TRY(linear(xn.p, M, C, xw.proj_in, ACT_NONE, nullptr, 0, nullptr, t, C));
        {
            GemmArgs g;
            heads_args(&g, hb, hb.q, 0, hb.k, 0, hb.vt, 1, hb.N, hb.npad);
            TRY(linear(t, M, C, xw.qkv, ACT_NONE, nullptr, 0, &g, nullptr, 0, nullptr, &xw.ln1, nrm));
        }
        TRY(self_attention(xw, hb, ao));
        if (fused_middle(xw, hb, M)) {
            XTailArgs a;
            a.ao = ao; a.ldao = C; a.t = t; a.ldt = C; a.M = M; a.ntok = hb.N;
            a.w1 = xw.out1.w; a.b1 = xw.out1.b; a.a1 = xw.out1.loraA; a.lb1 = xw.out1.loraB;
            a.ln_g = xw.ln2.g; a.ln_b = xw.ln2.b; a.ln_eps = 1e-5f;
            a.wq = xw.q2p; a.bq = xw.q2.b; a.aq = xw.q2.loraA; a.lbq = xw.q2.loraB;
            a.kvp = xw.kvp; a.nk = m.ctx_len; a.scale = 1.0f / sqrtf((float)hb.hd);
            a.w2 = xw.out2p; a.b2 = xw.out2.b; a.a2 = xw.out2.loraA; a.lb2 = xw.out2.loraB;
            a.lora_r = xw.out1.R ? 4 : 0;
            if (!dry) TRY(launch_xattn_tail(a, st));
        } else {
        TRY(linear(ao, M, C, xw.out1, ACT_NONE, t, C, nullptr, t, C));
        {
            GemmArgs g;
            heads_args(&g, hb, hb.q, 0, nullptr, 0, nullptr, 0, hb.N, hb.npad);
            TRY(linear(t, M, C, xw.q2, ACT_NONE, nullptr, 0, &g, nullptr, 0, nullptr, &xw.ln2, nrm));
        }
        TRY(attention(hb, xw.kc, xw.vtc, m.ctx_len, m.ctx_pad, ao));
        TRY(linear(ao, M, C, xw.out2, ACT_NONE, t, C, nullptr, t, C));
        }
        bool proj_done = false;
        if (xw.ff2p && !m.keep && mlp_fused_ok(C, 4 * C, C)) {
            MlpArgs a;
            a.x = t; a.ldx = C; a.M = M; a.ln_gamma = xw.ln3.g; a.ln_beta = xw.ln3.b; a.ln_eps = 1e-5f;
            a.w1 = xw.ff1.w; a.b1 = xw.ff1.b; a.w2p = xw.ff2p; a.b2 = xw.ff2.b;
            a.resid = t; a.ldr = C; a.out = t; a.ldo = C; a.C = C; a.H = 4 * C; a.N2 = C;
            if (xw.proj_outp && M % 128 == 0 && mlp_proj_enabled()) {
                a.wp = xw.proj_outp; a.bp = xw.proj_out.b; a.xres = x.p; a.ldxr = C; a.out2 = o.p; a.ldo2 = C;
                proj_done = true;
            }
            if (!dry) TRY(launch_mlp_fused(a, st));
        } else {
            T* ff = static_cast<T*>(alloc((size_t)M * 4 * C * sizeof(T)));
            if (!ff) return 7;
            if (xw.ff1.R) {
                T* pre = static_cast<T*>(alloc((size_t)M * 8 * C * sizeof(T)));
                if (!pre) return 7;
                TRY(linear(t, M, C, xw.ff1, ACT_NONE, nullptr, 0, nullptr, pre, 8 * C, nullptr, &xw.ln3, nrm));
                if (!dry) TRY(launch_geglu_fwd<T>(pre, ff, M, 4 * C, st));
            } else {
                TRY(linear(t, M, C, xw.ff1, ACT_GEGLU, nullptr, 0, nullptr, ff, 4 * C, nullptr, &xw.ln3, nrm));
            }
            if (sizeof(T) == 2 && !m.keep && xw.ffpo && !xw.ff2.R && !xw.proj_out.R && ff_proj_fused_enabled()) {
                GemmArgs g;
                ga_rows(g, ff, 4 * C, 4 * C); ga_rows2(g, t, C, C); ga_weight(g, xw.ffpo, M, C, 5 * C); g.bias = xw.bffpo;
                ga_resid(g, x.p, C); ga_out(g, o.p, C);
                g.no_rp = 1;
                g.alg_flops = 2.0 * M * (double)C * (5 * C);
                TRY(run_gemm(g));
                proj_done = true;
            } else {
                TRY(linear(ff, M, 4 * C, xw.ff2, ACT_NONE, t, C, nullptr, t, C));
            }
        }
        if (!proj_done) TRY(linear(t, M, C, xw.proj_out, ACT_NONE, x.p, C, nullptr, o.p, C));
        if (!m.keep) m.arena.release(mk);
        *out = o;
        return 0;
    }

    int time_embed(const long long* t_dev, int t_scalar, int B) {
        const int rows = t_scalar ? 1 : B;
        const int c0 = m.cfg.block_out_channels[0], temb = 4 * c0;
        float* s = static_cast<float*>(alloc((size_t)rows * c0 * sizeof(float)));
        float* y1 = static_cast<float*>(alloc((size_t)rows * temb * sizeof(float)));
        float* emb = static_cast<float*>(alloc((size_t)rows * temb * sizeof(float)));
        m.tproj_out = static_cast<float*>(alloc((size_t)rows * m.tproj_total * sizeof(float)));
        if (!s || !y1 || !emb || !m.tproj_out) return 7;
        m.t_scalar = t_scalar;
        m.te_s = s; m.te_y1 = y1; m.te_emb = emb;
        if (dry) return 0;
        if (m.tproj_table && t_scalar && !m.keep)
            return launch_select_row(m.tproj_table, m.tproj_step, m.tproj_first, m.tproj_out, m.tproj_total, st);
        TRY(launch_timestep_embedding(t_dev, t_scalar, s, rows, c0, st));
        TRY(launch_gemv_rows<T>(s, c0, m.te1.w, m.te1.b, y1, temb, rows, temb, c0, 0, st));
        TRY(launch_gemv_rows<T>(y1, temb, m.te2.w, m.te2.b, emb, temb, rows, temb, temb, 1, st));
        TRY(launch_gemv_rows<T>(emb, temb, m.tproj.w, m.tproj.b, m.tproj_out, m.tproj_total, rows, m.tproj_total, temb, 1, st));
        return 0;
    }

    int time_embed_table(const long long* ts_dev, int rows, float* scratch, float* table) {
        const int c0 = m.cfg.block_out_channels[0], temb = 4 * c0;
        for (int r0 = 0; r0 < rows; r0 += 64) {
            const int nr = std::min(64, rows - r0);
            float* s = scratch;
            float* y1 = s + (size_t)64 * c0;
            float* emb = y1 + (size_t)64 * temb;
            TRY(launch_timestep_embedding(ts_dev + r0, 0, s, nr, c0, st));
            TRY(launch_gemv_rows<T>(s, c0, m.te1.w, m.te1.b, y1, temb, nr, temb, c0, 0, st));
            TRY(launch_gemv_rows<T>(y1, temb, m.te2.w, m.te2.b, emb, temb, nr, temb, temb, 1, st));
            TRY(launch_gemv_rows<T>(emb, temb, m.tproj.w, m.tproj.b, table + (size_t)r0 * m.tproj_total, m.tproj_total, nr, m.tproj_total, temb, 1, st));
        }
        return 0;
    }

    int direct(const Act& x, const ConvW& cw, int stride, int act, const Act* add, Act* out) {
        const int pad = cw.ks / 2;
        const int Ho = (x.H + 2 * pad - cw.ks) / stride + 1, Wo = (x.W + 2 * pad - cw.ks) / stride + 1;
        *out = new_act(x.B, Ho, Wo, cw.cout);
        if (!out->p) return 7;
        MRISR_REQUIRE(cw.cin == x.C, "direct conv channel mismatch");
        DirectConvArgs a;
        a.x = x.p; a.w = cw.w; a.bias = cw.b; a.y = out->p; a.B = x.B; a.Hin = x.H; a.Win = x.W; a.Cin = x.C;
        a.Hout = Ho; a.Wout = Wo; a.Cout = cw.cout; a.ks = cw.ks; a.stride = stride; a.pad = pad; a.act = act;
        a.add = add ? add->p : nullptr;
        if (dry) return 0;
        return launch_direct_conv<T>(a, st);
    }

    int import_act(const mrisr_tensor& t, Act* out, bool copy_if_nhwc) {
        MRISR_REQUIRE(t.ndim == 4, "expected a 4-D tensor");
        const int B = (int)t.shape[0], C = (int)t.shape[1], H = (int)t.shape[2], W = (int)t.shape[3];
        if (t.layout == MRISR_NHWC) {
            MRISR_REQUIRE(t.dtype == m.cfg.compute_dtype, "NHWC tensors must be in the compute dtype");
            if (!copy_if_nhwc) {
                out->p = t.data; out->B = B; out->H = H; out->W = W; out->C = C;
                return 0;
            }
        }
        *out = new_act(B, H, W, C);
        if (!out->p) return 7;
        if (dry) return 0;
        if (t.layout == MRISR_NHWC) {
            MRISR_CHECK_HIP(hipMemcpyAsync(out->p, t.data, out->numel() * sizeof(T), hipMemcpyDeviceToDevice, st));
            return 0;
        }
        return launch_nchw_to_nhwc<T>(t.data, t.dtype, out->p, B, C, H, W, st);
    }
    int export_act(const Act& a, const mrisr_tensor& t, float scale) {
        MRISR_REQUIRE(t.ndim == 4 && t.shape[0] == a.B && t.shape[1] == a.C && t.shape[2] == a.H && t.shape[3] == a.W,
                      "output tensor shape mismatch");
        if (dry) return 0;
        if (t.layout == MRISR_NHWC) {
            MRISR_REQUIRE(t.dtype == m.cfg.compute_dtype && scale == 1.0f, "NHWC outputs: compute dtype, scale 1");
            MRISR_CHECK_HIP(hipMemcpyAsync(t.data, a.p, a.numel() * sizeof(T), hipMemcpyDeviceToDevice, st));
            return 0;
        }
        return launch_nhwc_to_nchw<T>(a.p, t.data, t.dtype, a.B, a.C, a.H, a.W, scale, st);
    }
    int add_external(Act& x, const mrisr_tensor& t) {
        const size_t mk = m.arena.mark();
        Act r;
        TRY(import_act(t, &r, false));
        MRISR_REQUIRE(r.B == x.B && r.C == x.C && r.H == x.H && r.W == x.W, "residual shape mismatch");
        if (!dry) TRY(launch_add_inplace<T>(x.p, r.p, (long long)x.numel(), st));
        if (!m.keep) m.arena.release(mk);
        return 0;
    }

    int encoder(Act x, const mrisr_tensor* intrablock, int n_intra, std::vector<Act>* skips, Act* out, int last_skip = -1) {
        skips->push_back(x);
        int ib = 0;
        auto done = [&] { return last_skip >= 0 && (int)skips->size() > last_skip; };
        for (int i = 0; i < m.cfg.num_levels && !done(); ++i) {
            Level& lv = m.down[i];
            const bool has_attn = !lv.xf.empty();
            const int block_last = (int)skips->size() - 1 + (int)lv.res.size() + (lv.has_down ? 1 : 0);
            for (size_t j = 0; j < lv.res.size() && !done(); ++j) {
                Act y, xn_next;
                xn_next.p = nullptr;
                if (has_attn) TRY(resnet(lv.res[j], x, nullptr, &y, &lv.xf[j].norm, 1e-6f, &xn_next));
                else TRY(resnet(lv.res[j], x, nullptr, &y));
                x = y;
                if (has_attn) {
                    TRY(transformer(lv.xf[j], x, &y, &xn_next));
                    x = y;
                    if (j + 1 == lv.res.size() && ib < n_intra) TRY(add_external(x, intrablock[ib++]));
                }
                skips->push_back(x);
            }
            if (lv.has_down && !done()) {
                Act y;
                TRY(conv3(x, nullptr, lv.down, 2, 0, nullptr, 0, 1, nullptr, ACT_NONE, &y));
                x = y;
                skips->push_back(x);
            }
            if (!has_attn && ib < n_intra && (last_skip < 0 || last_skip >= block_last)) {
                TRY(add_external(x, intrablock[ib++]));
            }
        }
        *out = x;
        return 0;
    }
    int mid(Act x, Act* out) {
        Act y, xn_next;
        xn_next.p = nullptr;
        TRY(resnet(m.mid_r0, x, nullptr, &y, &m.mid_xf.norm, 1e-6f, &xn_next));
        x = y;
        TRY(transformer(m.mid_xf, x, &y, &xn_next));
        x = y;
        TRY(resnet(m.mid_r1, x, nullptr, &y));
        *out = y;
        return 0;
    }

    int set_context(const mrisr_tensor& ehs) {
        MRISR_REQUIRE(ehs.ndim == 3 && ehs.shape[2] == m.cfg.cross_attention_dim, "encoder_hidden_states shape");
        MRISR_REQUIRE((int)ehs.shape[0] == m.ws_B && (int)ehs.shape[1] == m.ctx_len, "context shape vs planned workspace");
        if (!dry) TRY(launch_nchw_to_nhwc<T>(ehs.data, ehs.dtype, m.ctx_rows, m.ws_B * m.ctx_len, m.cfg.cross_attention_dim, 1, 1, st));
        auto each = [&](XfW& x) -> int { return project_context(x, m.head_buf_for_C(x.C)); };
        for (auto& lv : m.down) for (auto& x : lv.xf) TRY(each(x));
        TRY(each(m.mid_xf));
        for (auto& lv : m.up) for (auto& x : lv.xf) TRY(each(x));
        m.ctx_valid = true;
        return 0;
    }

    int freeu(const Act& x, const Act& sk, float b, float s) {
        MRISR_REQUIRE(!m.keep, "FreeU: not while a training forward is being recorded");
        MRISR_REQUIRE(x.B == sk.B && x.H == sk.H && x.W == sk.W, "FreeU: hidden and skip geometry differ");
        MRISR_REQUIRE(x.C % 16 == 0 && sk.C % 8 == 0, "FreeU: hidden channels must be a multiple of 16, skip channels of 8");
        if (dry) return 0;
        return launch_freeu<T>(x.p, sk.p, x.p, sk.p, x.B, x.H, x.W, x.C, sk.C, b, s, st);
    }

    int unet_forward(const mrisr_tensor& sample, const long long* t_dev, int t_scalar, const mrisr_tensor* ehs,
                     const mrisr_tensor* down_res, int n_down, const mrisr_tensor* mid_res,
                     const mrisr_tensor* intrablock, int n_intra, const mrisr_tensor& out, const UNetCache& fc = UNetCache()) {
        m.arena.reset();
        const int B = (int)sample.shape[0];
        const bool store = fc.mode == CACHE_STORE, use = fc.mode == CACHE_USE;
        const int q0 = m.num_skips() - 1 - fc.depth;
        if (store || use) {
            MRISR_REQUIRE(q0 >= 0 && fc.depth >= 1 && fc.p, "feature cache: depth 1 .. num_skips - 1 and a buffer");
            MRISR_REQUIRE(n_down == 0 && !mid_res, "a feature cache together with ControlNet residuals is not supported");
        }
        if (ehs) TRY(set_context(*ehs));
        MRISR_REQUIRE(dry || m.ctx_valid, "no encoder_hidden_states given and none cached");
        TRY(time_embed(t_dev, t_scalar, B));
        Act s, x;
        TRY(import_act(sample, &s, false));
        TRY(direct(s, m.conv_in, 1, ACT_NONE, nullptr, &x));
        std::vector<Act> skips;
        TRY(encoder(x, intrablock, n_intra, &skips, &x, use ? fc.depth : -1));
        if (n_down > 0) {
            MRISR_REQUIRE(n_down == (int)skips.size(), "down_block_additional_residuals count");
            for (int k = 0; k < n_down; ++k) {
                if (skips[k].p == x.p) {
                    Act c = new_act(x.B, x.H, x.W, x.C);
                    if (!c.p) return 7;
                    if (!dry) MRISR_CHECK_HIP(hipMemcpyAsync(c.p, x.p, x.numel() * sizeof(T), hipMemcpyDeviceToDevice, st));
                    skips[k] = c;
                }
                TRY(add_external(skips[k], down_res[k]));
            }
        }
        if (!use) TRY(mid(x, &x));
        if (mid_res) TRY(add_external(x, *mid_res));
        int q = 0;
        for (int i = 0; i < m.cfg.num_levels; ++i) {
            Level& lv = m.up[i];
            for (size_t j = 0; j < lv.res.size(); ++j, ++q) {
                if (use && q < q0) continue;
                if ((store || use) && q == q0) {
                    int64_t cs[4];
                    TRY(m.cache_shape(fc.depth, B, (int)sample.shape[2], (int)sample.shape[3], cs));
                    if (store) {
                        MRISR_REQUIRE(x.B == cs[0] && x.C == cs[1] && x.H == cs[2] && x.W == cs[3], "feature cache shape");
                        if (!dry) MRISR_CHECK_HIP(hipMemcpyAsync(fc.p, x.p, x.numel() * sizeof(T), hipMemcpyDeviceToDevice, st));
                    } else {
                        x.p = fc.p; x.B = (int)cs[0]; x.C = (int)cs[1]; x.H = (int)cs[2]; x.W = (int)cs[3];
                    }
                }
                Act sk = skips.back();
                skips.pop_back();
                if (m.freeu.on && i < 2) TRY(freeu(x, sk, m.freeu.b[i], m.freeu.s[i]));
                Act y, xn_next;
                xn_next.p = nullptr;
                if (!lv.xf.empty()) TRY(resnet(lv.res[j], x, &sk, &y, &lv.xf[j].norm, 1e-6f, &xn_next));
                else TRY(resnet(lv.res[j], x, &sk, &y));
                x = y;
                if (!lv.xf.empty()) {
                    TRY(transformer(lv.xf[j], x, &y, &xn_next));
                    x = y;
                }
            }
            if (lv.has_up && !(use && q <= q0)) {
                Act y;
                TRY(upsample_conv(x, lv, &y));
                x = y;
            }
        }
        Act xn, y;
        TRY(gn(x, nullptr, m.norm_out, true, m.cfg.norm_eps, &xn));
        if (m.conv_out.cout % 4 == 0) TRY(conv3(xn, nullptr, m.conv_out, 1, 0, nullptr, 0, 1, nullptr, ACT_NONE, &y));
        else TRY(direct(xn, m.conv_out, 1, ACT_NONE, nullptr, &y));
        return export_act(y, out, 1.0f);
    }

    int set_cond(const mrisr_tensor& cond) {
        const size_t mk = m.arena.mark();
        Act e, y;
        TRY(import_act(cond, &e, false));
        for (size_t k = 0; k < m.ce.size(); ++k) {
            const bool last = k + 1 == m.ce.size();
            const int act = last ? ACT_NONE : ACT_SILU;
            constexpr int KQ = 128 / (int)sizeof(T);
            if (e.C % KQ == 0 && m.ce[k].cout % 4 == 0) TRY(conv3(e, nullptr, m.ce[k], m.ce_stride[k], 0, nullptr, 0, 1, nullptr, act, &y));
            else TRY(direct(e, m.ce[k], m.ce_stride[k], act, nullptr, &y));
            e = y;
        }
        MRISR_REQUIRE(e.numel() * sizeof(T) <= m.cond_emb_bytes, "condition embedding larger than planned");
        if (!dry) MRISR_CHECK_HIP(hipMemcpyAsync(m.cond_emb, e.p, e.numel() * sizeof(T), hipMemcpyDeviceToDevice, st));
        if (!m.keep) m.arena.release(mk);
        m.cond_valid = true;
        return 0;
    }

    int controlnet_forward(const mrisr_tensor& sample, const long long* t_dev, int t_scalar, const mrisr_tensor* ehs,
                           const mrisr_tensor* cond, float scale, mrisr_tensor* down_out, int n_down,
                           mrisr_tensor* mid_out) {
        m.arena.reset();
        const int B = (int)sample.shape[0];
        if (ehs) TRY(set_context(*ehs));
        if (cond) TRY(set_cond(*cond));
        MRISR_REQUIRE(dry || (m.ctx_valid && m.cond_valid), "context / condition image neither given nor cached");
        TRY(time_embed(t_dev, t_scalar, B));
        Act s, x;
        TRY(import_act(sample, &s, false));
        Act ce;
        ce.p = m.cond_emb; ce.B = B; ce.H = s.H; ce.W = s.W; ce.C = m.cfg.block_out_channels[0];
        TRY(direct(s, m.conv_in, 1, ACT_NONE, &ce, &x));
        std::vector<Act> skips;
        TRY(encoder(x, nullptr, 0, &skips, &x));
        TRY(mid(x, &x));
        MRISR_REQUIRE(n_down == (int)skips.size(), "ControlNet output count");
        for (int k = 0; k < n_down; ++k) {
            const size_t mk = m.arena.mark();
            Act o = new_act(skips[k].B, skips[k].H, skips[k].W, skips[k].C);
            if (!o.p) return 7;
            TRY(linear(skips[k].p, (int)skips[k].rows(), skips[k].C, m.cn_down[k], ACT_NONE, nullptr, 0, nullptr, o.p, o.C));
            TRY(export_act(o, down_out[k], scale));
            if (!m.keep) m.arena.release(mk);
        }
        Act o = new_act(x.B, x.H, x.W, x.C);
        if (!o.p) return 7;
        TRY(linear(x.p, (int)x.rows(), x.C, m.cn_mid, ACT_NONE, nullptr, 0, nullptr, o.p, o.C));
        return export_act(o, *mid_out, scale);
    }
};

}
```

### mri-diffusion-superresolution_amd/csrc/runtime.h

```cpp
#pragma once
#include <cstdint>
#include <map>
#include <memory>
#include <string>
#include <vector>

#include "../../include/mrisr.h"
#include "common.h"

namespace mrisr {

struct DevBuf {
    void* p = nullptr;
    size_t bytes = 0;
    DevBuf() = default;
    DevBuf(const DevBuf&) = delete;
    DevBuf& operator=(const DevBuf&) = delete;
    ~DevBuf() { release(); }
    void release() {
        if (p) (void)hipFree(p);
        p = nullptr;
        bytes = 0;
    }
    int reserve(size_t n, bool zero) {
// ... 54 lines not shown
    void* loraAd = nullptr;
    float* loraB = nullptr;
    void* loraBT = nullptr;
    long long offLA = -1, offLB = -1;
};
struct LinW {
    void* w = nullptr;
    const float* b = nullptr;
    int n = 0, k = 0;
    int geglu_half = 0;
    int r = 0, R = 0, secN = 1;
    int rp = 0;
    int kw() const { return rp ? k + R : k; }
    void* loraA = nullptr;
    const float* loraB = nullptr;
    void* w8 = nullptr;
    float* w_scale = nullptr;
    void* loraA8 = nullptr;
    float* loraA_scale = nullptr;
    std::vector<std::string> mod_names;
    std::vector<int> mod_lora;
    std::vector<long long> offA, offB;
    void* wT = nullptr;
    void* loraBT = nullptr;
    float* loraAT = nullptr;
    float* loraB_rw = nullptr;
    float* dora_g = nullptr;
    std::vector<long long> offM;
};

struct Act {
    void* p = nullptr;
    int B = 0, H = 0, W = 0, C = 0;
    size_t rows() const { return (size_t)B * H * W; }
    size_t numel() const { return rows() * C; }
};

inline int dtype_size(int dt) { return dt == MRISR_F32 ? 4 : (dt == MRISR_I64 ? 8 : 2); }

int tile_axis(int n, int t, int o, int window, std::vector<int>& origins, std::vector<float>& weights);
struct TilePlan {
    int H = 0, W = 0, th = 0, tw = 0;
    std::vector<int> oy, ox;
    std::vector<float> nwy, nwx;
    std::vector<uint32_t> words;
    size_t off_nwy = 0, off_nwx = 0;
    int T() const { return (int)(oy.size() * ox.size()); }
    int build(int H_, int W_, int tile_h, int tile_w, int overlap_h, int overlap_w, int window);
    int check();
    void pack();
    size_t bytes() const { return words.size() * sizeof(uint32_t); }
    TileGrid grid(const void* dev) const;
};

}
```

### mri-diffusion-superresolution_amd/csrc/sampler.hip

```cpp
#include <algorithm>
#include <cmath>
#include <cstring>
#include <memory>
#include <vector>

#include "api.h"
#include "model.h"
#include "prof.h"
#include "step_plan.h"

namespace mrisr {

__device__ __forceinline__ float wsum(float v) {
#pragma unroll
    for (int o = 32; o > 0; o >>= 1) v += __shfl_xor(v, o);
    return v;
}
static inline unsigned nblocks(long long total) {
    long long b = (total + 255) / 256;
    return (unsigned)(b > 16384 ? 16384 : (b < 1 ? 1 : b));
}

__global__ void ddim_step_kernel(float* x, const float* eps, const float* coef, const int* step, long long n) {
    const int s = *step;
// ... 319 lines not shown
}
__global__ void advance_step_kernel(int* step) { *step += 1; }
int launch_advance_step(int* step_idx, hipStream_t st) {
    hipLaunchKernelGGL(advance_step_kernel, dim3(1), dim3(1), 0, st, step_idx);
    MRISR_CHECK_HIP(hipGetLastError());
    return 0;
}
__global__ void resshift_forward_kernel(const float* hr, const float* lr, const float* noise, const float* ac,
                                        const long long* t, int t_is_scalar, float* out, int B, long long per) {
    const long long n = (long long)B * per;
    for (long long i = blockIdx.x * 256ll + threadIdx.x; i < n; i += (long long)gridDim.x * 256) {
        const int b = (int)(i / per);
        const float a = ac[t_is_scalar ? t[0] : t[b]];
        const float ra = sqrtf(a);
        out[i] = ra * hr[i] + (1.f - ra) * lr[i] + sqrtf(1.f - a) * noise[i];
    }
}
int launch_resshift_forward(const float* hr, const float* lr, const float* noise, const float* alphas_cumprod,
                            const long long* t, int t_is_scalar, float* out, int B, long long per_sample,
                            hipStream_t st) {
    hipLaunchKernelGGL(resshift_forward_kernel, dim3(nblocks((long long)B * per_sample)), dim3(256), 0, st, hr, lr,
                       noise, alphas_cumprod, t, t_is_scalar, out, B, per_sample);
    MRISR_CHECK_HIP(hipGetLastError());
    return 0;
}

}

using namespace mrisr;

struct mrisr_model : public Model {};

__global__ void load_t_kernel(long long* cur_t, const long long* table, const int* step) { *cur_t = table[*step]; }

static int g_temb_table = -1;
extern "C" void mrisr_debug_temb_table(int on) { g_temb_table = on; }
static bool temb_table_enabled() {
    static const int env = [] { const char* e = getenv("MRISR_TEMB_TABLE"); return e ? atoi(e) : 1; }();
    return g_temb_table < 0 ? env != 0 : g_temb_table != 0;
}
static void unipc_rho(const double* rks, int p, double h, int k, double* rho) {
    const double hh = -h, Bh = std::expm1(hh);
    double A[3][4];
    double phik = std::expm1(hh) / hh - 1.0, fact = 1.0;
    for (int j = 1; j <= p; ++j) {
        if (j <= k) {
            for (int c = 0; c < k; ++c) A[j - 1][c] = std::pow(rks[c], j - 1);
            A[j - 1][k] = phik * fact / Bh;
        }
        fact *= j + 1;
        phik = phik / hh - 1.0 / fact;
    }
    for (int c = 0; c < k; ++c) {
        int piv = c;
        for (int r = c + 1; r < k; ++r) if (std::fabs(A[r][c]) > std::fabs(A[piv][c])) piv = r;
        for (int q = 0; q <= k; ++q) std::swap(A[c][q], A[piv][q]);
        for (int r = c + 1; r < k; ++r) {
            const double f = A[r][c] / A[c][c];
            for (int q = c; q <= k; ++q) A[r][q] -= f * A[c][q];
        }
    }
    for (int r = k - 1; r >= 0; --r) {
        double v = A[r][k];
        for (int q = r + 1; q < k; ++q) v -= A[r][q] * rho[q];
        rho[r] = v / A[r][r];
    }
// ... 353 lines not shown
                      pag ? "pag run: controlnet_cond must be [K B, C, 8h, 8w] (the [B] images K times)"
                      : guided ? "guided run: controlnet_cond must be [2B, C, 8h, 8w] (the [B] images twice)"
                             : "controlnet_cond must be [B, C, 8h, 8w] with the latents' batch");
    {
        int need = 0;
        for (int i = s->first; i < s->last; ++i)
            if (s->sigma[i] != 0.f) need = i + 1;
        if (a.noise) {
            MRISR_REQUIRE(a.noise->dtype == MRISR_F32 && a.noise->ndim >= 1 && numel(a.noise) % n == 0,
                          "step_noise: f32, a stack of latents-shaped slabs");
            MRISR_REQUIRE(numel(a.noise) / n >= need, "step_noise has fewer slabs than the last stochastic step needs");
        }
    }
    for (int i = 0; i < a.n_intrablock && !tiled; ++i)
        MRISR_REQUIRE(a.intrablock[i].ndim == 4 && a.intrablock[i].shape[0] == NB,
                      pag ? "pag run: adapter features must be [K B, ...] (the [B] features K times)"
                      : guided ? "guided run: adapter features must be [2B, ...] (the [B] features twice)"
                             : "adapter features must carry the latents' batch");
    MRISR_REQUIRE(a.n_intrablock >= 0 && a.n_intrablock <= PLAN_MAX_INTRA, "more adapter features than a step plan holds");
    MRISR_REQUIRE(!s->cnet || s->cnet->num_skips() + 1 <= PLAN_MAX_RES, "more ControlNet residuals than a step plan holds");

    p.kind = s->kind; p.K = K; p.pag = pag;
    p.B = B; p.T = T; p.C = Cl; p.h = h; p.w = w; p.fh = fh; p.fw = fw; p.L = (int)ehs->shape[1];
    p.cnet = s->cnet != nullptr;
    p.cdt = U.cfg.compute_dtype;
    p.first = s->first;
    p.x = static_cast<float*>(latents->data);
    p.lr = a.lr ? static_cast<const float*>(a.lr->data) : nullptr;
    p.noise = a.noise ? static_cast<const float*>(a.noise->data) : nullptr;
    p.d_coef = static_cast<const float*>(s->d_coef.p);
    p.d_step = static_cast<int*>(s->d_step.p);
    p.d_curt = static_cast<long long*>(s->d_curt.p);
    p.d_ts = static_cast<const long long*>(s->d_ts.p);
    if (s->kind == MRISR_STEP_DDPM) p.clip = s->clip;
    if (guided) { p.guidance_scale = s->guidance_scale; p.guidance_rescale = s->guidance_rescale; }
    if (pag) { p.pag_mask = s->pag_mask; p.pag_scale = s->pag_scale; }
    if (U.freeu.on) {
        p.freeu = 1;
        p.freeu_s[0] = U.freeu.s[0]; p.freeu_s[1] = U.freeu.s[1]; p.freeu_b[0] = U.freeu.b[0]; p.freeu_b[1] = U.freeu.b[1];
    }
    if (s->multistep()) {
        p.order = s->ms.order;
        p.final_zero = s->ms.final_zero; p.lower_order_final = s->ms.lower_order_final;
        p.n_disabled = (int)s->ms.disable_corrector.size();
        for (int i = 0; i < p.n_disabled && i < 32; ++i) p.disabled[i] = s->ms.disable_corrector[i];
    }
    if (cached) { p.cached = 1; p.cache_depth = s->cache_depth; }
    if (tiled) {
        p.tile_h = s->tile_h; p.tile_w = s->tile_w; p.tile_oh = s->tile_oh; p.tile_ow = s->tile_ow; p.tile_window = s->tile_window;
    }
    return 0;
}

static int run_operands(mrisr_sampler* s, const RunArgs& a, StepPlan& p, hipStream_t st) {
    Model& U = *s->unet;
    const int FB = p.K * p.B * p.T, esz = dtype_size(p.cdt);
    TRY(gemm_prepare());
    TRY(U.set_context(a.ehs, FB, p.fh, p.fw, st));
    if (s->cnet) {
        Model& C = *s->cnet;
        TRY(C.set_context(a.ehs, FB, p.fh, p.fw, st));
        TRY(C.set_cond(a.cond, p.L, st));
        p.n_res = C.num_skips();
        s->res_bufs.resize(p.n_res + 1);
        for (int k = 0; k <= p.n_res; ++k) {
            int64_t shape[4];
// ... 35 lines not shown
        TRY(s->d_xt.reserve(tile_elems * sizeof(float), false));
        TRY(s->d_et.reserve(tile_elems * sizeof(float), false));
        MRISR_CHECK_HIP(hipMemcpyAsync(s->d_tiles.p, s->tiles.words.data(), s->tiles.bytes(), hipMemcpyHostToDevice, st));
        const TileGrid g = s->tiles.grid(s->d_tiles.p);
        p.tile_oy = g.oy; p.tile_ox = g.ox; p.tile_nwy = g.nwy; p.tile_nwx = g.nwx;
        p.tile_ky = g.ky; p.tile_kx = g.kx; p.tile_vec4 = g.vec4;
        p.d_xt = static_cast<float*>(s->d_xt.p); p.d_et = static_cast<float*>(s->d_et.p);
    }
    if (p.cached) {
        int64_t cs[4];
        TRY(U.cache_shape(p.cache_depth, NB, p.h, p.w, cs));
        TRY(s->d_cache.reserve((size_t)cs[0] * cs[1] * cs[2] * cs[3] * dtype_size(p.cdt), false));
        p.d_cache = s->d_cache.p;
    }
    if (p.K > 1) {
        TRY(s->d_x2.reserve((size_t)p.K * n * sizeof(float), false));
        for (int k = 0; k < p.K; ++k)
            MRISR_CHECK_HIP(hipMemcpyAsync(static_cast<float*>(s->d_x2.p) + (size_t)k * n, p.x, (size_t)n * sizeof(float), hipMemcpyDeviceToDevice, st));
        p.d_x2 = static_cast<float*>(s->d_x2.p);
    }
    if (s->multistep()) {
        TRY(s->d_hist.reserve((size_t)p.order * n * sizeof(float), false));
        MRISR_CHECK_HIP(hipMemsetAsync(s->d_hist.p, 0, (size_t)p.order * n * sizeof(float), st));
        p.hist = static_cast<float*>(s->d_hist.p);
        if (s->kind == MRISR_STEP_UNIPC) {
            TRY(s->d_xc.reserve((size_t)n * sizeof(float), false));
            MRISR_CHECK_HIP(hipMemsetAsync(s->d_xc.p, 0, (size_t)n * sizeof(float), st));
            p.xc = static_cast<float*>(s->d_xc.p);
        }
        MRISR_CHECK_HIP(hipMemcpyAsync(s->d_coef.p, s->ms_rows.data(), sizeof(float) * s->ms_rows.size(), hipMemcpyHostToDevice, st));
    }
    MRISR_CHECK_HIP(hipMemsetAsync(s->d_step.p, 0, 16, st));
    MRISR_CHECK_HIP(hipMemcpyAsync(s->d_step.p, &s->first, sizeof(int), hipMemcpyHostToDevice, st));
    return 0;
}

static int run_temb_table(mrisr_sampler* s, StepPlan& p, hipStream_t st) {
    if (!temb_table_enabled()) return 0;
    const int rows = s->last - s->first;
    auto build = [&](Model& M, DevBuf& buf) -> int {
        const size_t scratch = (size_t)64 * M.cfg.block_out_channels[0] * 9;
        TRY(buf.reserve((scratch + (size_t)rows * M.tproj_total) * sizeof(float), false));
        float* sc = static_cast<float*>(buf.p);
        TRY(M.build_tproj_table(static_cast<const long long*>(s->d_ts.p) + s->first, rows, sc, sc + scratch, st));
        M.tproj_table = sc + scratch; M.tproj_step = static_cast<const int*>(s->d_step.p); M.tproj_first = s->first;
        return 0;
    };
    TRY(build(*s->unet, s->tp_unet));
    p.tproj_unet = s->unet->tproj_table;
    if (s->cnet) { TRY(build(*s->cnet, s->tp_cnet)); p.tproj_cnet = s->cnet->tproj_table; }
    return 0;
}

static int step_body(const StepPlan& p, Model& U, Model* C, int cache_mode, hipStream_t st) {
    const int NB = p.K * p.B, FB = NB * p.T;
    const long long per = (long long)p.C * p.h * p.w, n = (long long)p.B * per;
    const bool tiled = p.T > 1;
    mrisr_tensor tt{};
    tt.data = p.d_curt; tt.dtype = MRISR_I64; tt.ndim = 0;
    const float* canvas = p.K > 1 ? p.d_x2 : p.x;
    mrisr_tensor xin{};
    xin.data = tiled ? p.d_xt : const_cast<float*>(canvas);
    xin.dtype = MRISR_F32; xin.layout = MRISR_NCHW; xin.ndim = 4;
    xin.shape[0] = FB; xin.shape[1] = p.C; xin.shape[2] = p.fh; xin.shape[3] = p.fw;
    mrisr_tensor eps_t = xin;
    eps_t.data = tiled ? p.d_et : p.d_eps;
    TileGrid tg;
    if (tiled) {
        tg.H = p.h; tg.W = p.w; tg.th = p.fh; tg.tw = p.fw; tg.ky = p.tile_ky; tg.kx = p.tile_kx;
        tg.oy = p.tile_oy; tg.ox = p.tile_ox; tg.nwy = p.tile_nwy; tg.nwx = p.tile_nwx;
        tg.vec4 = p.tile_vec4 != 0;
    }
    mrisr_tensor res[PLAN_MAX_RES], intra[PLAN_MAX_INTRA];
    for (int k = 0; k <= p.n_res && p.cnet; ++k) res[k] = plan_tensor(p.res[k], p.cdt);
    for (int i = 0; i < p.n_intra; ++i) intra[i] = plan_tensor(p.intra[i], p.cdt);
    UNetCache fc;
    fc.mode = cache_mode; fc.depth = p.cache_depth; fc.p = p.d_cache;

    hipLaunchKernelGGL(load_t_kernel, dim3(1), dim3(1), 0, st, p.d_curt, p.d_ts, static_cast<const int*>(p.d_step));
    if (tiled) TRY(launch_tile_gather(canvas, p.d_xt, tg, NB, p.C, st));
    if (p.cnet) TRY(C->forward_controlnet(&xin, &tt, nullptr, nullptr, 1.0f, res, p.n_res, &res[p.n_res], st));
    TRY(U.forward_unet(&xin, &tt, nullptr, p.cnet ? res : nullptr, p.n_res, p.cnet ? &res[p.n_res] : nullptr, intra, p.n_intra, &eps_t, st,
                       p.cached ? &fc : nullptr));
    if (tiled) TRY(launch_tile_blend(p.d_et, p.d_eps, tg, NB, p.C, st));
    const bool multistep = p.kind > MRISR_STEP_DDPM;
    if (p.K > 1) {
        const float g = p.pag && p.K == 2 ? 1.f + p.pag_scale : p.guidance_scale;
        TRY(launch_guided_step(p.K, p.kind, p.x, p.d_x2, p.d_eps, p.lr, p.noise, p.d_coef, p.d_step, p.clip, g, p.K == 3 ? p.pag_scale : 0.f,
                               p.guidance_rescale, p.B, per, st, p.hist, p.xc, p.order));
    } else if (multistep)
        TRY(launch_multistep_step(p.x, p.d_eps, p.lr, p.d_coef, p.d_step, p.hist, p.xc, p.order, n, st));
    else if (p.kind == MRISR_STEP_DDIM)
        TRY(launch_ddim_step(p.x, p.d_eps, p.d_coef, p.d_step, n, st));
    else if (p.kind == MRISR_STEP_DDPM)
        TRY(launch_ddpm_step(p.x, p.d_eps, p.noise, p.d_coef, p.d_step, p.clip, n, st));
    else
        TRY(launch_resshift_step(p.x, p.d_eps, p.lr, p.noise, p.d_coef, p.d_step, n, st));
    return launch_advance_step(p.d_step, st);
}

static int run_steps(mrisr_sampler* s, const StepPlan& p, int use_graph, hipStream_t st) {
    Model& U = *s->unet;
    const bool cached = p.cached != 0;
    auto mode_of = [&](int i) { return !cached ? CACHE_NONE : ((i - s->first) % s->cache_interval == 0 ? CACHE_STORE : CACHE_USE); };
    if (!use_graph) {
        for (int i = s->first; i < s->last; ++i) TRY(step_body(p, U, s->cnet, mode_of(i), st));
        return 0;
    }
    if (!s->exec || (cached && !s->exec_shallow) || !same_plan(s->plan, p)) {
        s->drop_graphs();
        auto capture = [&](int cache_mode, hipGraphExec_t* exec) -> int {
            hipGraph_t graph = nullptr;
            MRISR_CHECK_HIP(hipStreamBeginCapture(st, hipStreamCaptureModeThreadLocal));
            int rc = step_body(p, U, s->cnet, cache_mode, st);
            hipError_t e = hipStreamEndCapture(st, &graph);
            if (rc) { if (graph) (void)hipGraphDestroy(graph); return rc; }
            MRISR_CHECK_HIP(e);
            MRISR_CHECK_HIP(hipGraphInstantiate(exec, graph, nullptr, nullptr, 0));
            (void)hipGraphDestroy(graph);
            ++s->n_captures;
            return 0;
        };
        TRY(capture(cached ? CACHE_STORE : CACHE_NONE, &s->exec));
        if (cached) TRY(capture(CACHE_USE, &s->exec_shallow));
        s->plan = p;
    }
    for (int i = s->first; i < s->last; ++i) MRISR_CHECK_HIP(hipGraphLaunch(mode_of(i) == CACHE_USE ? s->exec_shallow : s->exec, st));
    return 0;
}

static int sampler_run_impl(mrisr_sampler* s, const RunArgs& a, int use_graph, void* stream) {
// ... 148 lines not shown
```

### mri-diffusion-superresolution_amd/csrc/step_plan.h

```cpp
#pragma once
#include <cstring>
#include <type_traits>

namespace mrisr {

constexpr int PLAN_MAX_RES = 32;
constexpr int PLAN_MAX_INTRA = 8;

#pragma GCC diagnostic push
#pragma GCC diagnostic error "-Wpadded"
struct PlanTensor {
    const void* data;
    long long shape[4];
};
struct StepPlan {
    float* x;
    const float* lr;
    const float* noise;
    float* d_eps;
    float* d_x2;
    float* d_xt;
    float* d_et;
    const int* tile_oy;
    const int* tile_ox;
// ... 1 lines not shown
    const float* tile_nwx;
    float* hist;
    float* xc;
    void* d_cache;
    const float* d_coef;
    int* d_step;
    long long* d_curt;
    const long long* d_ts;
    unsigned long long ws_gen_unet, ws_gen_cnet;
    const float* tproj_unet;
    const float* tproj_cnet;
    PlanTensor res[PLAN_MAX_RES];
    PlanTensor intra[PLAN_MAX_INTRA];
    int kind;
    int K, pag;
    int B, T, C, h, w, fh, fw, L;
    int cnet;
    int n_res, n_intra;
    float clip;
    float guidance_scale, guidance_rescale;
    float pag_scale;
    unsigned pag_mask;
    int order;
    int cached, cache_depth;
    int tile_h, tile_w, tile_oh, tile_ow, tile_window;
    int tile_ky, tile_kx, tile_vec4;
    int freeu;
    float freeu_s[2], freeu_b[2];
    int first;
    int final_zero, lower_order_final;
    int n_disabled;
    int disabled[32];
    int cdt;
};
#pragma GCC diagnostic pop
static_assert(std::is_trivially_copyable<StepPlan>::value, "StepPlan is compared and copied as bytes");

inline StepPlan new_step_plan() {
    StepPlan p;
    std::memset(&p, 0, sizeof(p));
    return p;
}
inline bool same_plan(const StepPlan& a, const StepPlan& b) { return std::memcmp(&a, &b, sizeof(StepPlan)) == 0; }

}
```

### mri-diffusion-superresolution_amd/mrisr/_lib.py

```python
from __future__ import annotations

import ctypes as C
import os
from typing import Optional, Sequence

import torch

_HERE = os.path.dirname(os.path.abspath(__file__))
LIB_PATH = os.path.join(os.path.dirname(_HERE), "csrc", "libmrisr.so")

MRISR_F32, MRISR_BF16, MRISR_F16, MRISR_I64 = 0, 1, 2, 3
MRISR_NCHW, MRISR_NHWC = 0, 1
STEP_DDIM, STEP_RESSHIFT, STEP_DDPM, STEP_UNIPC, STEP_DPMSOLVERPP = 0, 1, 2, 3, 4
ACT_NONE, ACT_RELU, ACT_SILU, ACT_GEGLU = 0, 1, 2, 3
TILE_WINDOWS = {"uniform": 0, "gaussian": 1}

_DT = {torch.float32: MRISR_F32, torch.bfloat16: MRISR_BF16, torch.float16: MRISR_F16, torch.int64: MRISR_I64}


class Tensor(C.Structure):
    _fields_ = [("data", C.c_void_p), ("dtype", C.c_int32), ("layout", C.c_int32), ("ndim", C.c_int32),
                ("shape", C.c_int64 * 4)]


# ... 4 lines not shown
                ("norm_num_groups", C.c_int32), ("norm_eps", C.c_float), ("cond_channels", C.c_int32),
                ("cond_embed_channels", C.c_int32 * 4), ("compute_dtype", C.c_int32), ("lora_rank", C.c_int32),
                ("lora_fused", C.c_int32), ("flash_attention", C.c_int32), ("fp8_linears", C.c_int32),
                ("fp8_attention", C.c_int32), ("fp8_train", C.c_int32)]


class AdapterCfg(C.Structure):
    _fields_ = [("channels", C.c_int32 * 4), ("nums_rb", C.c_int32), ("cin", C.c_int32), ("ksize", C.c_int32),
                ("use_conv", C.c_int32), ("compute_dtype", C.c_int32)]


class VaeCfg(C.Structure):
    _fields_ = [("in_channels", C.c_int32), ("out_channels", C.c_int32), ("latent_channels", C.c_int32),
                ("num_levels", C.c_int32), ("block_out_channels", C.c_int32 * 4), ("layers_per_block", C.c_int32),
                ("norm_num_groups", C.c_int32), ("compute_dtype", C.c_int32), ("scaling_factor", C.c_float)]


class MrisrError(RuntimeError):
    pass


_lib: Optional[C.CDLL] = None

EXPORTS = [
    "mrisr_last_error", "mrisr_version", "mrisr_unet_create", "mrisr_controlnet_create", "mrisr_model_destroy",
    "mrisr_model_set_param", "mrisr_model_set_lora_scale", "mrisr_model_set_dora", "mrisr_model_finalize", "mrisr_model_num_params",
    "mrisr_model_workspace_bytes", "mrisr_unet_forward", "mrisr_model_set_context", "mrisr_model_num_skips",
    "mrisr_model_skip_shape", "mrisr_controlnet_forward", "mrisr_controlnet_set_cond", "mrisr_adapter_create",
    "mrisr_adapter_destroy", "mrisr_adapter_set_param", "mrisr_adapter_finalize", "mrisr_adapter_forward",
    "mrisr_resshift_forward", "mrisr_sampler_create", "mrisr_sampler_destroy", "mrisr_sampler_run", "mrisr_sampler_set_range", "mrisr_sampler_set_clip",
    "mrisr_sampler_set_guidance", "mrisr_sampler_run_guided", "mrisr_sampler_set_cache", "mrisr_unet_cache_shape", "mrisr_unet_forward_cached", "mrisr_op_guided_step", "mrisr_sampler_set_solver", "mrisr_op_multistep_step",
    "mrisr_model_set_pag", "mrisr_model_num_transformer_blocks", "mrisr_sampler_set_pag", "mrisr_sampler_run_pag", "mrisr_sampler_num_captures",
    "mrisr_op_attn_identity", "mrisr_op_pag_step", "mrisr_op_pag_multistep_step",
    "mrisr_model_set_freeu", "mrisr_op_freeu",
    "mrisr_tile_tables", "mrisr_sampler_set_tiles", "mrisr_op_tile_gather", "mrisr_op_tile_blend",
    "mrisr_adapter_train_prepare", "mrisr_adapter_train_num_trainable", "mrisr_adapter_train_num_tensors",
    "mrisr_adapter_train_tensor_info", "mrisr_adapter_train_bind", "mrisr_adapter_train_refresh", "mrisr_adapter_backward", "mrisr_adapter_backward_level", "mrisr_adapter_train_level_range",
    "mrisr_vae_create", "mrisr_vae_destroy", "mrisr_vae_set_param", "mrisr_vae_num_params", "mrisr_vae_finalize",
    "mrisr_vae_encode", "mrisr_vae_decode",
    "mrisr_image_metrics",
    "mrisr_resize_scratch_bytes", "mrisr_resize_slices", "mrisr_gaussian_blur_slices", "mrisr_low_field_scratch_bytes",
    "mrisr_simulate_low_field",
    "mrisr_train_prepare", "mrisr_train_num_trainable", "mrisr_train_num_tensors", "mrisr_train_tensor_info", "mrisr_train_tensor_shape",
    "mrisr_train_bind", "mrisr_train_refresh", "mrisr_train_step", "mrisr_train_set_intrablock_grads", "mrisr_train_set_controlnet_residuals", "mrisr_controlnet_train_prepare", "mrisr_controlnet_train_num_trainable", "mrisr_controlnet_train_num_tensors", "mrisr_controlnet_train_tensor_info", "mrisr_controlnet_train_bind", "mrisr_controlnet_train_refresh", "mrisr_controlnet_train_forward", "mrisr_controlnet_train_backward", "mrisr_optim_sumsq", "mrisr_optim_adamw", "mrisr_optim_ema",
    "mrisr_prof_enable", "mrisr_prof_reset", "mrisr_prof_report",
    "mrisr_op_conv3x3", "mrisr_op_conv3x3_sc", "mrisr_op_ff_proj", "mrisr_op_linear", "mrisr_op_ln_linear", "mrisr_op_linear_fp8", "mrisr_op_mlp", "mrisr_op_mlp_proj", "mrisr_op_xattn_tail", "mrisr_op_groupnorm", "mrisr_op_layernorm", "mrisr_op_attention",
    "mrisr_op_attention_bwd",
    "mrisr_op_groupnorm_bwd", "mrisr_op_layernorm_bwd", "mrisr_op_geglu", "mrisr_op_pointwise_bwd", "mrisr_op_lora_wgrad", "mrisr_op_lora_wgrad_geglu", "mrisr_op_lora_wgrad_hr", "mrisr_op_dora_scale", "mrisr_op_dora_mag_grad",
    "mrisr_op_transpose", "mrisr_op_softmax_bwd", "mrisr_op_small_dense_bwd", "mrisr_op_conv_wgrad", "mrisr_op_conv_dgrad",
    "mrisr_op_conv_lora_down", "mrisr_op_conv_lora_dgrad", "mrisr_op_conv3x3_lora",
    "mrisr_fit_create", "mrisr_fit_destroy", "mrisr_fit_set_step", "mrisr_fit_get_step", "mrisr_fit_num_captures", "mrisr_fit_micro",
    "mrisr_fit_apply", "mrisr_fit_make_batch", "mrisr_fit_create_adapter", "mrisr_fit_make_condition",
]


def lib() -> C.CDLL:
    global _lib
    if _lib is None:
        if not os.path.exists(LIB_PATH):
            raise MrisrError(f"{LIB_PATH} not found: build it with `python __graft_entry__.py` (hipcc, gfx950). "
                             "There is no CPU fallback.")
        L = C.CDLL(LIB_PATH)
        L.mrisr_last_error.restype = C.c_char_p
        L.mrisr_version.restype = C.c_char_p
        L.mrisr_model_num_params.restype = C.c_int64
        L.mrisr_model_workspace_bytes.restype = C.c_int64
        L.mrisr_model_destroy.restype = None
# ... 15 lines not shown
        L.mrisr_op_layernorm_bwd.argtypes = [I, P, P, P, P, I, I, F, I, P, P, P]
        L.mrisr_op_geglu.argtypes = [I, I, P, P, P, Q, I, P]
        L.mrisr_op_pointwise_bwd.argtypes = [I, I, P, P, P, P, Q, I, I, I, I, I, I, I, P]
        L.mrisr_op_lora_wgrad.argtypes = [I, P, I, P, I, I, I, I, I, I, I, P, P, P, F, P]
        L.mrisr_op_lora_wgrad_geglu.argtypes = [I, P, I, P, I, I, I, I, P, F, P]
        L.mrisr_op_lora_wgrad_hr.argtypes = [I, P, I, P, I, I, I, I, I, I, I, P, P, P, F, I, P]
        L.mrisr_op_dora_scale.argtypes = [I, P, P, P, P, F, P, P, I, I, I, I, I, I, P]
        L.mrisr_op_dora_mag_grad.argtypes = [I, P, I, P, I, P, I, P, P, P, I, I, I, P]
        L.mrisr_model_set_dora.argtypes = [P, I]
        L.mrisr_op_transpose.argtypes = [I, P, P, I, I, I, I, Q, Q, I, I, P]
        L.mrisr_op_softmax_bwd.argtypes = [I, P, P, P, I, Q, I, F, P]
        L.mrisr_op_small_dense_bwd.argtypes = [I, I, P, I, P, I, I, I, I, I, P, I, P, P, I, P]
        L.mrisr_op_conv_wgrad.argtypes = [I, P, I, I, I, I, P, I, I, I, I, I, P, P, I, I, I, P]
        L.mrisr_op_conv_dgrad.argtypes = [I, P, I, I, I, I, P, I, I, P, I, P]
        L.mrisr_op_conv_lora_down.argtypes = [I, P, I, I, I, I, P, I, P, I, P]
        L.mrisr_op_conv_lora_dgrad.argtypes = [I, P, I, I, I, I, P, I, P, I, P]
        L.mrisr_op_conv3x3_lora.argtypes = [P, P, P, P, P, I, F, P, P, I, I, I, P, P]
        L.mrisr_op_mlp_proj.argtypes = [P, P, P, P, P, P, P, I, I, P, P, P, P, P]
        L.mrisr_op_xattn_tail.argtypes = [P, P, I] + [P] * 10 + [I] + [P] * 6 + [I, F, P]
        L.mrisr_tile_tables.argtypes = [I, I, I, I, P, P, P]
        L.mrisr_sampler_set_tiles.argtypes = [P, I, I, I, I, I]
        L.mrisr_op_tile_gather.argtypes = [P, P, P, I, P, I, P]
        L.mrisr_op_tile_blend.argtypes = [P, P, P, I, P, I, P, P, P]
        L.mrisr_model_set_pag.argtypes = [P, C.c_uint32, I, I]
        L.mrisr_model_num_transformer_blocks.argtypes = [P]
        L.mrisr_sampler_set_pag.argtypes = [P, C.c_uint32, F]
        L.mrisr_sampler_run_pag.argtypes = [P, P, P, P, P, P, P, I, I, I, P]
        L.mrisr_sampler_num_captures.argtypes = [P]
        L.mrisr_op_attn_identity.argtypes = [I, P, P, I, I, I, I, I, I, I, I, P]
        L.mrisr_op_pag_step.argtypes = [I, P, P, P, P, P, P, F, F, F, F, P]
        L.mrisr_op_pag_multistep_step.argtypes = [I, P, P, P, P, P, P, P, I, I, F, F, F, P]
        L.mrisr_model_set_freeu.argtypes = [P, I, F, F, F, F]
        L.mrisr_op_freeu.argtypes = [I, P, P, P, P, I, I, I, I, I, F, F, P]
        L.mrisr_resize_scratch_bytes.restype = C.c_size_t
        L.mrisr_resize_scratch_bytes.argtypes = [C.c_int] * 6
        L.mrisr_resize_slices.argtypes = [C.c_void_p, C.c_int, C.c_int, C.c_int, C.c_void_p, C.c_int, C.c_int, C.c_int, C.c_void_p,
                                          C.c_size_t, C.c_void_p]
        L.mrisr_gaussian_blur_slices.argtypes = [C.c_void_p, C.c_int, C.c_int, C.c_int, C.c_float, C.c_float, C.c_void_p, C.c_void_p,
                                                 C.c_void_p]
        L.mrisr_low_field_scratch_bytes.restype = C.c_size_t
        L.mrisr_low_field_scratch_bytes.argtypes = [C.c_int, C.c_int, C.c_int, C.c_float]
        L.mrisr_simulate_low_field.argtypes = [C.c_void_p, C.c_int, C.c_int, C.c_int, C.c_float, C.c_void_p, C.c_void_p, C.c_size_t,
                                               C.c_void_p]
        L.mrisr_vae_destroy.restype = None
        L.mrisr_vae_destroy.argtypes = [C.c_void_p]
        L.mrisr_vae_num_params.restype = C.c_int64
        L.mrisr_vae_num_params.argtypes = [C.c_void_p]
        for name in ("mrisr_model_destroy", "mrisr_adapter_destroy", "mrisr_sampler_destroy",
                     "mrisr_model_num_params", "mrisr_model_workspace_bytes", "mrisr_model_num_skips"):
            getattr(L, name).argtypes = [C.c_void_p]
        _lib = L
    return _lib


def check(rc: int):
    if rc != 0:
        raise MrisrError(f"libmrisr error {rc}: {lib().mrisr_last_error().decode()}")


def stream_ptr() -> C.c_void_p:
    return C.c_void_p(torch.cuda.current_stream().cuda_stream)


def as_tensor(t: Optional[torch.Tensor], layout: int = MRISR_NCHW, shape: Optional[Sequence[int]] = None) -> Tensor:
    d = Tensor()
    if t is None:
# ... 38 lines not shown
```

Baseline: 66.94 slices/s.

## Fuse split-K reduces into GroupNorm slabs, trim step-edge kernels, in-place subpixel output

Activations can now carry a pending split-K reduction (a debt) that the next GroupNorm settles by reading the f32 partials directly. It also handles concatenated second sources. conv_in reads the f32 NCHW sample directly, and conv_out's split-K reduce writes straight into the f32 NCHW output. The per-step load_t kernel is merged into the advance kernel. Together these drop several small kernels and round-trips per UNet step, at the cost of more complex bookkeeping. A sub-pixel upsample path that stores interleaved output is also added but stays off by default.

```diff
diff --git a/include/mrisr.h b/include/mrisr.h
--- a/include/mrisr.h
+++ b/include/mrisr.h
@@ -302,6 +302,9 @@
                            void* stream);
 int mrisr_op_freeu(int dtype, const void* hidden, const void* skip, void* hidden_out, void* skip_out, int B, int H, int W, int Ch, int Cs,
                    float b, float s, void* stream);
+int mrisr_op_groupnorm_slabs(const float* partial, int splitk, const float* bias_dev, const float* rowvec_dev, int rowvec_ld, int rowvec_div,
+                             const void* resid, const void* x1, int c0, int c1, int B, int HW, const float* gamma_dev, const float* beta_dev,
+                             int groups, float eps, int silu, int fused, void* raw_out, void* y, void* stream);
 int mrisr_op_transpose(int dtype, const void* src, void* dst, int R, int C, int ld_src, int ld_dst, int64_t bs_src, int64_t bs_dst,
                        int batch, int r_valid, void* stream);
 int mrisr_op_softmax_bwd(int dtype, const void* p, const float* dp, void* ds, int ld, int64_t rows, int nk, float scale, void* stream);
diff --git a/include/mrisr_debug.h b/include/mrisr_debug.h
--- a/include/mrisr_debug.h
+++ b/include/mrisr_debug.h
@@ -21,12 +21,16 @@
 void mrisr_debug_sk_inkernel(int on);
 
 void mrisr_debug_subpix(int min_rows);
+void mrisr_debug_subpix_inplace(int on);
+
+void mrisr_debug_step_edges(int on);
 
 void mrisr_debug_temb_table(int on);
 
 void mrisr_debug_mlp_proj(int on);
 
 void mrisr_debug_gn_slabs(int on);
+void mrisr_debug_owed_reduces(int* out3, int reset);
 
 void mrisr_debug_sc_fused(int on);
 
diff --git a/mri-diffusion-superresolution_amd/csrc/capi_ops.hip b/mri-diffusion-superresolution_amd/csrc/capi_ops.hip
--- a/mri-diffusion-superresolution_amd/csrc/capi_ops.hip
+++ b/mri-diffusion-superresolution_amd/csrc/capi_ops.hip
@@ -68,14 +68,20 @@
         MRISR_REQUIRE(y->shape[1] == cout && y->shape[2] == 2 * H && y->shape[3] == 2 * W, "conv output shape");
         DevBuf sp, planes;
         TRY(sp.reserve((size_t)16 * cout * Cin * sizeof(T), false));
-        TRY(planes.reserve((size_t)4 * B * H * W * cout * sizeof(T), false));
         TRY(launch_pack_conv_subpix<T>(w, sp.p, cout, Cin, st));
         GemmArgs g;
         ga_rows(g, x->data, C0, C0); ga_conv3(g, B, H, W); g.kw = 2; g.subpix = 1;
         ga_batch(g, 4, 0, (long long)cout * 4 * Cin, (long long)B * H * W * cout); ga_weight(g, sp.p, B * H * W, cout, 4 * Cin);
-        g.bias = bias; ga_out(g, planes.p, cout);
-        TRY(gemm_run<T>(g, st, false, devbuf_alloc(part)));
-        TRY(launch_subpix_shuffle<T>(planes.p, y->data, B, H, W, cout, st));
+        g.bias = bias; ga_out(g, y->data, cout);
+        if (gemm_subpix_inplace_ok(g)) {
+            g.subpix_out = 1;
+            TRY(gemm_run<T>(g, st, false, devbuf_alloc(part)));
+        } else {
+            TRY(planes.reserve((size_t)4 * B * H * W * cout * sizeof(T), false));
+            g.out = planes.p;
+            TRY(gemm_run<T>(g, st, false, devbuf_alloc(part)));
+            TRY(launch_subpix_shuffle<T>(planes.p, y->data, B, H, W, cout, st));
+        }
         MRISR_CHECK_HIP(hipStreamSynchronize(st));
         return 0;
     }
@@ -968,6 +974,41 @@
     API_END
 }
 
+int mrisr_op_groupnorm_slabs(const float* partial, int splitk, const float* bias_dev, const float* rowvec_dev, int rowvec_ld, int rowvec_div,
+                             const void* resid, const void* x1, int c0, int c1, int B, int HW, const float* gamma_dev, const float* beta_dev,
+                             int groups, float eps, int silu, int fused, void* raw_out, void* y, void* stream) {
+    API_BEGIN
+    MRISR_REQUIRE(partial && splitk >= 1 && raw_out && y && gamma_dev && beta_dev && B > 0 && HW > 0 && c0 > 0 && c1 >= 0 && (c1 == 0) == (x1 == nullptr),
+                  "GroupNorm from slabs: operands");
+    MRISR_REQUIRE(groups > 0 && groups <= 64 && (c0 + c1) % groups == 0 && c0 % 8 == 0 && c1 % 8 == 0 && (!rowvec_dev || (rowvec_div >= 1 && rowvec_ld >= c0)),
+                  "GroupNorm from slabs: whole groups, whole 16-byte vectors per source");
+    hipStream_t st = (hipStream_t)stream;
+    GroupNormArgs a;
+    a.x0 = nullptr; a.c0 = c0; a.x1 = x1; a.c1 = c1; a.B = B; a.HW = HW; a.groups = groups; a.eps = eps;
+    a.gamma = gamma_dev; a.beta = beta_dev; a.silu = silu; a.y = y;
+    a.nsplit = groupnorm_nsplit(B, HW);
+    DevBuf part;
+    TRY(part.reserve((size_t)B * a.nsplit * groups * 2 * sizeof(float), false));
+    a.partial = static_cast<float*>(part.p);
+    if (fused) {
+        MRISR_REQUIRE(groupnorm_slabs_ok(c0, c1, groups, HW, B), "GroupNorm from slabs: the one-launch geometry does not take this shape");
+        GnSlabSrc ss;
+        ss.partial = partial; ss.splitk = splitk; ss.bias = bias_dev; ss.rowvec = rowvec_dev; ss.rowvec_ld = rowvec_ld; ss.rowvec_div = rowvec_div;
+        ss.resid = resid; ss.ldr = c0; ss.raw_out = raw_out;
+        TRY(launch_groupnorm_slabs(a, ss, st));
+    } else {
+        GemmArgs g;
+        g.M = B * HW; g.N = c0; g.splitk = splitk; g.partial = const_cast<float*>(partial); g.bias = bias_dev;
+        ga_rowvec(g, rowvec_dev, rowvec_ld, rowvec_div > 0 ? rowvec_div : 1); ga_resid(g, resid, c0); ga_out(g, raw_out, c0);
+        TRY(launch_splitk_reduce<bf16>(g, st));
+        a.x0 = raw_out;
+        TRY(launch_groupnorm<bf16>(a, st));
+    }
+    MRISR_CHECK_HIP(hipStreamSynchronize(st));
+    return 0;
+    API_END
+}
+
 int mrisr_op_softmax_bwd(int dtype, const void* p, const float* dp, void* ds, int ld, int64_t rows, int nk, float scale, void* stream) {
     API_BEGIN
     TRY(bwd_dtype_ok(dtype));
diff --git a/mri-diffusion-superresolution_amd/csrc/common.h b/mri-diffusion-superresolution_amd/csrc/common.h
--- a/mri-diffusion-superresolution_amd/csrc/common.h
+++ b/mri-diffusion-superresolution_amd/csrc/common.h
@@ -94,6 +94,7 @@
     const void* w = nullptr;
     int M = 0, N = 0, K = 0;
     int kw = 3, subpix = 0;
+    int subpix_out = 0;
     int batch = 1;
     long long a_bs = 0, w_bs = 0;
     int heads = 1;
@@ -177,6 +178,7 @@
 int launch_xattn_tail(const XTailArgs& x, hipStream_t st);
 bool gemm_tile_lora_in_kernel(int tile, int r, int R);
 int gemm_rp_tile(const GemmArgs& g);
+bool gemm_subpix_inplace_ok(const GemmArgs& g);
 bool gemm_sc_tail_ok(const GemmArgs& g);
 bool sc_fused_enabled();
 bool ff_proj_fused_enabled();
@@ -208,7 +210,9 @@
     int ldr = 0;
     void* raw_out = nullptr;
 };
-bool groupnorm_slabs_ok(int C, int groups, int HW);
+bool groupnorm_slabs_ok(int c0, int c1, int groups, int HW, int B);
+int groupnorm_slabs_forms();
+extern int g_owed_paid[3];
 int launch_groupnorm_slabs(const GroupNormArgs& a, const GnSlabSrc& s, hipStream_t st);
 bool gn_fused_geometry(int c0, int c1, int groups, int HW, int* slab, int* slots, int* rl, int* nv, int ve = 8);
 template <typename T> int launch_groupnorm(const GroupNormArgs& a, hipStream_t st);
@@ -370,8 +374,12 @@
     void* y = nullptr;
     int B = 0, Hin = 0, Win = 0, Cin = 0, Hout = 0, Wout = 0, Cout = 0, ks = 3, stride = 1, pad = 1, act = 0;
     const void* add = nullptr;
+    int x_nchw_f32 = 0;
 };
 template <typename T> int launch_direct_conv(const DirectConvArgs& a, hipStream_t st);
+bool direct_conv_takes_nchw_f32(const DirectConvArgs& a, int elem_size);
+bool step_edges_enabled();
+int launch_splitk_reduce_nchw(const GemmArgs& g, float* dst, int HW, float scale, hipStream_t st);
 int direct_conv_prepare();
 template <typename T>
 int launch_nchw_to_nhwc(const void* src, int src_dtype, void* dst, int B, int C, int H, int W, hipStream_t st);
diff --git a/mri-diffusion-superresolution_amd/csrc/gemm.hip b/mri-diffusion-superresolution_amd/csrc/gemm.hip
--- a/mri-diffusion-superresolution_amd/csrc/gemm.hip
+++ b/mri-diffusion-superresolution_amd/csrc/gemm.hip
@@ -441,7 +441,8 @@
 __device__ __forceinline__ void copy_out_tile(const GemmArgs& g, const bf16* otile, int pitch, int m0, int n0, int z, bool add_resid) {
     __syncthreads();
     constexpr int CPR = BN / 8;
-    bf16* out = reinterpret_cast<bf16*>(g.out) + (size_t)z * g.o_bs;
+    const bool interleave = g.subpix_out != 0;
+    bf16* out = reinterpret_cast<bf16*>(g.out) + (interleave ? (size_t)0 : (size_t)z * g.o_bs);
     const bf16* res = add_resid ? reinterpret_cast<const bf16*>(g.resid) + (size_t)z * g.o_bs : nullptr;
     constexpr int TOTAL = BM * CPR, IT = (TOTAL + NT - 1) / NT, BATCH = IT < 5 ? IT : 5;
     for (int it0 = 0; it0 < IT; it0 += BATCH) {
@@ -460,7 +461,14 @@
             const int m = m0 + row, n = n0 + ch * 8;
             if (idx >= TOTAL || m >= g.M || n >= g.N) continue;
             const bf16* src = otile + row * pitch + ch * 8;
-            bf16* dst = out + (size_t)m * g.ldo + n;
+            size_t mo = (size_t)m;
+            if (interleave) {
+                const int hw = g.Hout * g.Wout;
+                const int b = m / hw, rem = m - b * hw;
+                const int oy = rem / g.Wout, ox = rem - oy * g.Wout;
+                mo = ((size_t)b * (2 * g.Hout) + 2 * oy + (z >> 1)) * (size_t)(2 * g.Wout) + 2 * ox + (z & 1);
+            }
+            bf16* dst = out + mo * g.ldo + n;
             if (n + 8 <= g.N) {
                 bf16x8 v = *reinterpret_cast<const bf16x8*>(src);
                 if (res) {
@@ -3138,6 +3146,19 @@
     return p;
 }
 
+static int stage_out_mode() {
+    static const int v = [] { const char* e = getenv("MRISR_STAGE_OUT"); return e ? atoi(e) : 2; }();
+    return v;
+}
+static int g_subpix_inplace = -1;
+extern "C" void mrisr_debug_subpix_inplace(int on) { g_subpix_inplace = on; ++g_plan_salt; }
+bool gemm_subpix_inplace_ok(const GemmArgs& g) {
+    static const int env = [] { const char* e = getenv("MRISR_SUBPIX_INPLACE"); return e ? atoi(e) : 0; }();
+    if (g_subpix_inplace < 0 ? !env : !g_subpix_inplace) return false;
+    return g.subpix && g.batch == 4 && g.conv && g.out_mode == OUT_ROWS && (g.ldo & 7) == 0 && g.heads == 1 && !g.resid && !g.lora_z && !g.lora_a &&
+           stage_out_mode() != 0;
+}
+
 template <typename T>
 int launch_gemm(const GemmArgs& g_in, hipStream_t st) {
     constexpr bool is_bf16 = sizeof(T) == 2;
@@ -3160,8 +3181,8 @@
     tile = tile_for_launch(g, is_bf16, tile);
     const char* why = nullptr;
     MRISR_REQUIRE(tile_admits(g, is_bf16, tile, &why), why);
-    static const int stage_env = [] { const char* e = getenv("MRISR_STAGE_OUT"); return e ? atoi(e) : 2; }();
-    g.stage_out = stage_env;
+    g.stage_out = stage_out_mode();
+    if (g.subpix_out) MRISR_REQUIRE(gemm_subpix_inplace_ok(g) && g.splitk == 1, "sub-pixel conv storing interleaved: bf16 rows through the staged copy-out, un-split, no residual");
     g.dbg = g_gemm_flags;
     {
         static const int on = [] { const char* e = getenv("MRISR_PRETOUCH"); return e ? atoi(e) : 1; }();
@@ -3196,6 +3217,43 @@
     return 0;
 }
 
+__global__ __launch_bounds__(256) void splitk_reduce_nchw_kernel(const GemmArgs g, float* __restrict__ dst, int HW, float scale) {
+    const int nq = g.N >> 2;
+    const long long total = (long long)g.M * nq;
+    for (long long i = blockIdx.x * 256ll + threadIdx.x; i < total; i += (long long)gridDim.x * 256) {
+        const int q = (int)(i / g.M);
+        const int m = (int)(i - (long long)q * g.M);
+        const int n = q * 4;
+        float v[4] = {0.f, 0.f, 0.f, 0.f}, b4[4] = {0.f, 0.f, 0.f, 0.f};
+        if (g.bias) load4<float>(g.bias + n, b4);
+        const float* p = g.partial + (size_t)m * g.N + n;
+        for (int s = 0; s < g.splitk; ++s) {
+            float t[4];
+            load4<float>(p + (size_t)s * g.M * g.N, t);
+#pragma unroll
+            for (int r = 0; r < 4; ++r) v[r] += t[r];
+        }
+        const int b = m / HW, pix = m - b * HW;
+#pragma unroll
+        for (int r = 0; r < 4; ++r) {
+            const float f = v[r] * g.alpha + b4[r];
+            dst[((size_t)b * g.N + n + r) * HW + pix] = scale * (float)from_f32<bf16>(f);
+        }
+    }
+}
+int launch_splitk_reduce_nchw(const GemmArgs& g, float* dst, int HW, float scale, hipStream_t st) {
+    MRISR_REQUIRE(g.splitk > 1 && g.partial && g.batch == 1 && g.heads == 1 && g.out_mode == OUT_ROWS && g.act == ACT_NONE && !g.rowvec && !g.resid &&
+                      !g.lora_z && !g.lora_a && g.N % 4 == 0 && HW > 0 && g.M % HW == 0 && dst,
+                  "split-K reduce into an f32 NCHW tensor: plain bf16 rows, bias only");
+    const long long total = (long long)g.M * (g.N / 4);
+    int blocks = (int)((total + 255) / 256);
+    if (blocks > 4096) blocks = 4096;
+    ProfScope ps("splitk_reduce_nchw", 0.0, (double)g.M * g.N * (4.0 * g.splitk + 4.0), st);
+    hipLaunchKernelGGL(splitk_reduce_nchw_kernel, dim3(blocks), dim3(256), 0, st, g, dst, HW, scale);
+    MRISR_CHECK_HIP(hipGetLastError());
+    return 0;
+}
+
 template int launch_gemm<float>(const GemmArgs&, hipStream_t);
 template int launch_gemm<bf16>(const GemmArgs&, hipStream_t);
 template int launch_splitk_reduce<float>(const GemmArgs&, hipStream_t);
diff --git a/mri-diffusion-superresolution_amd/csrc/misc.hip b/mri-diffusion-superresolution_amd/csrc/misc.hip
--- a/mri-diffusion-superresolution_amd/csrc/misc.hip
+++ b/mri-diffusion-superresolution_amd/csrc/misc.hip
@@ -428,6 +428,14 @@
                 const int ky = t / 3, kx = t - ky * 3;
                 const int iy = oy + ky - 1, ix = ox + kx - 1;
                 if (iy < 0 || iy >= a.Hin || ix < 0 || ix >= a.Win) return make_uint2(0u, 0u);
+                if (a.x_nchw_f32) {
+                    const size_t hw = (size_t)a.Hin * a.Win;
+                    const float* xf = reinterpret_cast<const float*>(a.x) + ((size_t)b * 4 * a.Hin + iy) * a.Win + ix;
+                    bf16x4 v;
+#pragma unroll
+                    for (int c = 0; c < 4; ++c) v[c] = from_f32<bf16>(xf[c * hw]);
+                    return __builtin_bit_cast(uint2, v);
+                }
                 return *reinterpret_cast<const uint2*>(x + (((size_t)b * a.Hin + iy) * a.Win + ix) * 4);
             };
             const uint2 p0 = tap4(fg * 2), p1 = tap4(fg * 2 + 1);
@@ -481,11 +489,24 @@
     return 0;
 }
 
+static size_t conv_in_mfma_smem(const DirectConvArgs& a) { return ((size_t)a.Cout * 40 + (size_t)4 * 16 * (a.Cout + 8)) * 2 + (size_t)a.Cout * 4; }
+bool direct_conv_takes_nchw_f32(const DirectConvArgs& a, int elem_size) {
+    return elem_size == 2 && a.ks == 3 && a.Cin == 4 && a.stride == 1 && a.pad == 1 && a.Cout % 16 == 0 && a.Hout == a.Hin && a.Wout == a.Win &&
+           conv_in_mfma_smem(a) <= 80 * 1024 && (long long)a.B * a.Hout * a.Wout * a.Cout < (1ll << 31);
+}
+static int g_step_edges = -1;
+extern "C" void mrisr_debug_step_edges(int on) { g_step_edges = on; ++g_plan_salt; }
+bool step_edges_enabled() {
+    static const int env = [] { const char* e = getenv("MRISR_STEP_EDGES"); return e ? atoi(e) : 1; }();
+    return g_step_edges < 0 ? env != 0 : g_step_edges != 0;
+}
+
 template <typename T>
 int launch_direct_conv(const DirectConvArgs& a, hipStream_t st) {
     const size_t wbytes = (size_t)a.ks * a.ks * a.Cin * a.Cout * sizeof(T);
+    MRISR_REQUIRE(!a.x_nchw_f32 || direct_conv_takes_nchw_f32(a, (int)sizeof(T)), "an f32 NCHW input: only the matrix-core conv_in form reads it");
     if (sizeof(T) == 2 && a.ks == 3 && a.Cin == 4 && a.stride == 1 && a.pad == 1 && a.Cout % 16 == 0 && a.Hout == a.Hin && a.Wout == a.Win) {
-        const size_t smem = ((size_t)a.Cout * 40 + (size_t)4 * 16 * (a.Cout + 8)) * 2 + (size_t)a.Cout * 4;
+        const size_t smem = conv_in_mfma_smem(a);
         if (smem <= 80 * 1024 && (long long)a.B * a.Hout * a.Wout * a.Cout < (1ll << 31)) {
             if (direct_conv_prepare()) return 1;
             const long long M = (long long)a.B * a.Hout * a.Wout;
diff --git a/mri-diffusion-superresolution_amd/csrc/norm.hip b/mri-diffusion-superresolution_amd/csrc/norm.hip
--- a/mri-diffusion-superresolution_amd/csrc/norm.hip
+++ b/mri-diffusion-superresolution_amd/csrc/norm.hip
@@ -189,9 +189,10 @@
 #pragma unroll
     for (int e = 0; e < VE; ++e) s1[e] = s2[e] = 0.f;
     if (active) {
-        if constexpr (SLAB) {
+        if (SLAB && ch < a.c0) {
             typedef __attribute__((ext_vector_type(VE))) float fvec_t;
-            const size_t MN = (size_t)a.B * a.HW * C;
+            const int C0 = a.c0;
+            const size_t MN = (size_t)a.B * a.HW * C0;
             fvec_t bv;
 #pragma unroll
             for (int e = 0; e < VE; ++e) bv[e] = 0.f;
@@ -201,7 +202,7 @@
                 const int r = rl + i * RL;
                 if (r < a.HW) {
                     const size_t mrow = (size_t)b * a.HW + r;
-                    const float* pp = ss.partial + mrow * C + ch;
+                    const float* pp = ss.partial + mrow * C0 + ch;
                     fvec_t v;
 #pragma unroll
                     for (int e = 0; e < VE; ++e) v[e] = 0.f;
@@ -224,7 +225,7 @@
                     }
 #pragma unroll
                     for (int e = 0; e < VE; ++e) xv[i][e] = (bf16)v[e];
-                    if (ss.raw_out) *reinterpret_cast<vec_t*>(reinterpret_cast<T*>(ss.raw_out) + mrow * C + ch) = xv[i];
+                    if (ss.raw_out) *reinterpret_cast<vec_t*>(reinterpret_cast<T*>(ss.raw_out) + mrow * C0 + ch) = xv[i];
                 }
             }
         } else {
@@ -458,28 +459,41 @@
 
 static int g_gn_slabs = -1;
 extern "C" void mrisr_debug_gn_slabs(int on) { g_gn_slabs = on; ++g_plan_salt; }
-static bool gn_slabs_geometry(int C, int groups, int HW, int B, int* ve, int* slab, int* slots, int* rl, int* nv) {
-    if (!gn_fused_geometry(C, 0, groups, HW, slab, slots, rl, nv, 8)) return false;
+int g_owed_paid[3] = {0, 0, 0};
+extern "C" void mrisr_debug_owed_reduces(int* out3, int reset) {
+    for (int i = 0; i < 3; ++i) {
+        if (out3) out3[i] = g_owed_paid[i];
+        if (reset) g_owed_paid[i] = 0;
+    }
+}
+static bool gn_slabs_geometry(int c0, int c1, int groups, int HW, int B, int* ve, int* slab, int* slots, int* rl, int* nv) {
+    const int C = c0 + c1;
+    if (!gn_fused_geometry(c0, c1, groups, HW, slab, slots, rl, nv, 8)) return false;
     *ve = 8;
     int s4 = 0, sl4 = 0, rl4 = 0, nv4 = 0;
-    if (B * (C / *slab) < 512 && gn_fused_geometry(C, 0, groups, HW, &s4, &sl4, &rl4, &nv4, 4) && C / s4 > C / *slab) {
+    if (B * (C / *slab) < 512 && gn_fused_geometry(c0, c1, groups, HW, &s4, &sl4, &rl4, &nv4, 4) && C / s4 > C / *slab) {
         *ve = 4; *slab = s4; *slots = sl4; *rl = rl4; *nv = nv4;
     }
     return *nv <= 8;
 }
-bool groupnorm_slabs_ok(int C, int groups, int HW) {
+int groupnorm_slabs_forms() {
     static const int env = [] { const char* e = getenv("MRISR_GN_SLABS"); return e ? atoi(e) : 1; }();
-    if (g_gn_slabs < 0 ? !env : !g_gn_slabs) return false;
-    if (C % groups || groups > 64 || C % 8) return false;
+    const int v = g_gn_slabs < 0 ? env : g_gn_slabs;
+    return v == 1 ? 2 : (v == 2 ? 1 : 0);
+}
+bool groupnorm_slabs_ok(int c0, int c1, int groups, int HW, int B) {
+    if (!groupnorm_slabs_forms()) return false;
+    const int C = c0 + c1;
+    if (c0 <= 0 || c1 < 0 || B <= 0 || C % groups || groups > 64 || c0 % 8 || c1 % 8) return false;
     int ve, slab, slots, rl, nv;
-    return gn_slabs_geometry(C, groups, HW, 32, &ve, &slab, &slots, &rl, &nv);
+    return gn_slabs_geometry(c0, c1, groups, HW, B, &ve, &slab, &slots, &rl, &nv);
 }
 int launch_groupnorm_slabs(const GroupNormArgs& a, const GnSlabSrc& s, hipStream_t st) {
-    const int C = a.c0;
-    MRISR_REQUIRE(a.c1 == 0 && a.x1 == nullptr && C % a.groups == 0 && a.groups <= 64 && C % 8 == 0, "GroupNorm from slabs: one source, whole groups");
+    const int C = a.c0 + a.c1;
+    MRISR_REQUIRE(a.c0 > 0 && (a.c1 == 0) == (a.x1 == nullptr) && C % a.groups == 0 && a.groups <= 64 && a.c0 % 8 == 0 && a.c1 % 8 == 0, "GroupNorm from slabs: whole groups, whole vectors per source");
     MRISR_REQUIRE(s.partial && s.splitk >= 1 && a.partial != nullptr && a.nsplit >= 1 && (!s.rowvec || s.rowvec_div >= 1) && (!s.resid || s.ldr % 8 == 0), "GroupNorm from slabs: operands");
     int ve, slab, slots, rl, nv;
-    MRISR_REQUIRE(gn_slabs_geometry(C, a.groups, a.HW, a.B, &ve, &slab, &slots, &rl, &nv), "GroupNorm from slabs: geometry (groupnorm_slabs_ok)");
+    MRISR_REQUIRE(gn_slabs_geometry(a.c0, a.c1, a.groups, a.HW, a.B, &ve, &slab, &slots, &rl, &nv), "GroupNorm from slabs: geometry (groupnorm_slabs_ok with this launch's batch)");
     const int nslab = C / slab;
     const int xmap = (a.B % 8) == 0 ? 1 : 0;
     std::string nf = "groupnorm_from_slabs";
@@ -488,8 +502,8 @@
         snprintf(buf, sizeof(buf), " B=%d HW=%d C=%d s=%d", a.B, a.HW, C, s.splitk);
         nf += buf;
     }
-    const double act_bytes = (double)a.B * a.HW * C * 2.0;
-    ProfScope ps(prof_intern(nf), 0.0, act_bytes * (2.0 * s.splitk + 1.0 + (s.raw_out ? 1.0 : 0.0) + (s.resid ? 1.0 : 0.0)), st);
+    const double act_bytes = (double)a.B * a.HW * C * 2.0, slab_bytes = (double)a.B * a.HW * a.c0 * 2.0;
+    ProfScope ps(prof_intern(nf), 0.0, act_bytes + (double)a.B * a.HW * a.c1 * 2.0 + slab_bytes * (2.0 * s.splitk + (s.raw_out ? 1.0 : 0.0) + (s.resid ? 1.0 : 0.0)), st);
     const dim3 fg(a.B * nslab);
 #define GNS_GO(NV, VEV) hipLaunchKernelGGL((gn_fused_kernel<NV, VEV, true>), fg, dim3(256), 0, st, a, slab, slots, rl, nslab, xmap, s)
     if (ve == 8) { if (nv <= 2) GNS_GO(2, 8); else if (nv <= 4) GNS_GO(4, 8); else GNS_GO(8, 8); }
diff --git a/mri-diffusion-superresolution_amd/csrc/runner.h b/mri-diffusion-superresolution_amd/csrc/runner.h
--- a/mri-diffusion-superresolution_amd/csrc/runner.h
+++ b/mri-diffusion-superresolution_amd/csrc/runner.h
@@ -2,6 +2,7 @@
 #include <climits>
 #include <cmath>
 #include <cstdlib>
+#include <deque>
 
 #include "api.h"
 #include "gemm_args.h"
@@ -22,12 +23,59 @@
     return v == 1;
 }
 
+struct SlabDebt {
+    GemmArgs g;
+    bool paid = false;
+};
+
 template <typename T>
 struct Runner {
     Model& m;
     hipStream_t st;
     bool dry;
     Runner(Model& mm, hipStream_t s, bool d) : m(mm), st(s), dry(d) {}
+
+    bool owing_on = false;
+    std::deque<SlabDebt> debts;
+    bool may_owe(int C, int HW, int B) const {
+        return owing_on && sizeof(T) == 2 && !m.keep && groupnorm_slabs_forms() == 2 && groupnorm_slabs_ok(C, 0, m.cfg.norm_num_groups, HW, B);
+    }
+    static bool owes(const Act& a) { return a.debt && !a.debt->paid; }
+    int pay(SlabDebt& d, int who = 1) {
+        if (d.paid) return 0;
+        d.paid = true;
+        if (dry) return 0;
+        ++g_owed_paid[who];
+        return launch_splitk_reduce<T>(d.g, st);
+    }
+    int settle(const Act& a) { return a.debt ? pay(*a.debt) : 0; }
+    int settle_all() {
+        for (auto& d : debts) TRY(pay(d));
+        return 0;
+    }
+    int launch_owing(const GemmArgs& g, Act* out) {
+        MRISR_REQUIRE(g.splitk > 1 && g.partial && g.out == out->p && g.ldo == out->C && g.N == out->C && g.out_mode == OUT_ROWS && g.act == ACT_NONE &&
+                          !g.lora_z && !g.lora_a && g.batch == 1, "a GEMM that owes its reduce: split, plain bf16 rows");
+        debts.push_back(SlabDebt{g, false});
+        out->debt = &debts.back();
+        if (dry) return 0;
+        GemmArgs d = g;
+        d.defer_reduce = 1;
+        return launch_gemm<T>(d, st);
+    }
+    static GnSlabSrc slab_src(const GemmArgs& g, void* raw_out) {
+        GnSlabSrc ss;
+        ss.partial = g.partial; ss.splitk = g.splitk; ss.alpha = g.alpha; ss.bias = g.bias; ss.rowvec = g.rowvec; ss.rowvec_ld = g.rowvec_ld;
+        ss.rowvec_div = g.rowvec_div; ss.resid = g.resid; ss.ldr = g.ldr; ss.raw_out = raw_out;
+        return ss;
+    }
+    int gn_slabs_or_reduce(GroupNormArgs& a, GemmArgs& g, void* raw, void* reduce_into) {
+        if (groupnorm_slabs_ok(a.c0, a.c1, a.groups, a.HW, a.B)) return launch_groupnorm_slabs(a, slab_src(g, raw), st);
+        g.out = reduce_into; g.ldo = a.c0;
+        TRY(launch_splitk_reduce<T>(g, st));
+        a.x0 = reduce_into;
+        return launch_groupnorm<T>(a, st);
+    }
 
     void* alloc(size_t bytes) {
         void* p = m.arena.alloc(bytes);
@@ -56,6 +104,18 @@
         if (!out->p || !a.partial) return 7;
         if (partial_out) *partial_out = a.partial;
         if (nsplit_out) *nsplit_out = a.nsplit;
+        if (x1) TRY(settle(*x1));
+        if (owes(x0)) {
+            SlabDebt& d = *x0.debt;
+            if (!groupnorm_slabs_ok(a.c0, a.c1, a.groups, a.HW, a.B)) {
+                TRY(pay(d, 2));
+            } else {
+                d.paid = true;
+                if (dry) return 0;
+                ++g_owed_paid[0];
+                return launch_groupnorm_slabs(a, slab_src(d.g, x0.p), st);
+            }
+        }
         if (dry) return 0;
         return launch_groupnorm<T>(a, st);
     }
@@ -64,14 +124,23 @@
     int run_gemm(GemmArgs& g) { return gemm_run<T>(g, st, dry, arena_alloc()); }
 
     int conv3(const Act& x, const Act* x1, const ConvW& cw, int stride, int ups, const float* rowvec, int rowvec_ld,
-              int rowvec_div, const Act* resid, int act, Act* out, const float* lz = nullptr) {
+              int rowvec_div, const Act* resid, int act, Act* out, const float* lz = nullptr, bool owing = false) {
         const int Cin = x.C + (x1 ? x1->C : 0);
         MRISR_REQUIRE(cw.cin == Cin && cw.ks == 3, "conv3x3 weight mismatch");
+        TRY(settle(x));
+        if (x1) TRY(settle(*x1));
+        if (resid) TRY(settle(*resid));
         GemmArgs g = conv3_args(x, x1, cw, stride, ups, rowvec, rowvec_ld, rowvec_div, resid, act);
         *out = new_act(x.B, g.Hout, g.Wout, cw.cout);
         if (!out->p) return 7;
         g.out = out->p;
         if (lz) ga_lora_epilogue(g, cw, lz);
+        if (owing && !lz && act == ACT_NONE && may_owe(cw.cout, g.Hout * g.Wout, x.B)) {
+            TRY(gemm_choose(g, true));
+            TRY(gemm_alloc_partial(g, arena_alloc()));
+            if (g.splitk > 1) return launch_owing(g, out);
+            return dry ? 0 : launch_gemm<T>(g, st);
+        }
         return run_gemm(g);
     }
     static GemmArgs conv3_args(const Act& x, const Act* x1, const ConvW& cw, int stride, int ups, const float* rowvec, int rowvec_ld,
@@ -98,7 +167,10 @@
         const int Cin = x.C + (x1 ? x1->C : 0);
         MRISR_REQUIRE(cw.cin == Cin && cw.ks == 3 && nw.c == cw.cout, "conv3x3 + GroupNorm weight mismatch");
         GemmArgs g = conv3_args(x, x1, cw, 1, 0, rowvec, rowvec_ld, rowvec_div, resid, ACT_NONE);
-        bool fuse = sizeof(T) == 2 && !m.keep && groupnorm_slabs_ok(cw.cout, m.cfg.norm_num_groups, x.H * x.W);
+        TRY(settle(x));
+        if (x1) TRY(settle(*x1));
+        if (resid) TRY(settle(*resid));
+        bool fuse = sizeof(T) == 2 && !m.keep && groupnorm_slabs_ok(cw.cout, 0, m.cfg.norm_num_groups, x.H * x.W, x.B);
         if (fuse) {
             g.out = kUnallocated;
             TRY(gemm_choose(g, true));
@@ -125,10 +197,7 @@
         if (dry) return 0;
         g.defer_reduce = 1;
         TRY(launch_gemm<T>(g, st));
-        GnSlabSrc ss;
-        ss.partial = g.partial; ss.splitk = g.splitk; ss.alpha = g.alpha; ss.bias = g.bias; ss.rowvec = g.rowvec; ss.rowvec_ld = g.rowvec_ld;
-        ss.rowvec_div = g.rowvec_div; ss.resid = g.resid; ss.ldr = g.ldr; ss.raw_out = h.p;
-        return launch_groupnorm_slabs(a, ss, st);
+        return gn_slabs_or_reduce(a, g, h.p, h.p ? h.p : out->p);
     }
 
     static int subpix_min_rows() {
@@ -138,19 +207,25 @@
     int upsample_conv(const Act& x, const Level& lv, Act* out) {
         const int minr = subpix_min_rows();
         if (!(sizeof(T) == 2 && lv.up_sp && !m.keep && minr > 0 && (long long)x.rows() >= minr))
-            return conv3(x, nullptr, lv.up, 1, 1, nullptr, 0, 1, nullptr, ACT_NONE, out);
+            return conv3(x, nullptr, lv.up, 1, 1, nullptr, 0, 1, nullptr, ACT_NONE, out, nullptr, true);
+        TRY(settle(x));
         const ConvW& cw = lv.up;
         MRISR_REQUIRE(cw.cin == x.C, "upsampler weight mismatch");
         *out = new_act(x.B, 2 * x.H, 2 * x.W, cw.cout);
         if (!out->p) return 7;
         const size_t mk = m.arena.mark();
         const long long plane = (long long)x.rows() * cw.cout;
+        GemmArgs g;
+        ga_rows(g, x); ga_conv3(g, x); g.kw = 2; g.subpix = 1; ga_batch(g, 4, 0, (long long)cw.cout * 4 * cw.cin, plane);
+        ga_weight(g, lv.up_sp, (int)x.rows(), cw.cout, 4 * x.C); g.bias = cw.b; ga_out(g, out->p, cw.cout);
+        g.alg_flops = 2.0 * 4.0 * g.M * (double)g.N * g.K;
+        if (gemm_subpix_inplace_ok(g)) {
+            g.subpix_out = 1;
+            return run_gemm(g);
+        }
         T* planes = static_cast<T*>(alloc((size_t)4 * plane * sizeof(T)));
         if (!planes) return 7;
-        GemmArgs g;
-        ga_rows(g, x); ga_conv3(g, x); g.kw = 2; g.subpix = 1; ga_batch(g, 4, 0, (long long)cw.cout * 4 * cw.cin, plane);
-        ga_weight(g, lv.up_sp, (int)x.rows(), cw.cout, 4 * x.C); g.bias = cw.b; ga_out(g, planes, cw.cout);
-        g.alg_flops = 2.0 * 4.0 * g.M * (double)g.N * g.K;
+        g.out = planes;
         TRY(run_gemm(g));
         if (!dry) TRY(launch_subpix_shuffle<T>(planes, out->p, x.B, x.H, x.W, cw.cout, st));
         m.arena.release(mk);
@@ -268,17 +343,22 @@
         GroupNormArgs a2;
         GemmArgs gt = resnet_conv2_args(kUnallocated, x.B, x.H, x.W, r.cout, r.c2sc, r.b2sc, nullptr, o.p, r.cin, &x, x1);
         const bool sc_tail = sizeof(T) == 2 && !m.keep && r.has_sc && r.c2sc && sc_fused_enabled() && x.C + (x1 ? x1->C : 0) == r.cin && gemm_sc_tail_ok(gt);
-        if (next && next_out && sizeof(T) == 2 && !m.keep && next->c == r.cout && groupnorm_slabs_ok(r.cout, m.cfg.norm_num_groups, x.H * x.W)) {
+        const bool to_next = next && next_out && sizeof(T) == 2 && !m.keep && next->c == r.cout &&
+                             groupnorm_slabs_ok(r.cout, 0, m.cfg.norm_num_groups, x.H * x.W, x.B);
+        bool owe2 = false;
+        if (to_next || may_owe(r.cout, x.H * x.W, x.B)) {
             g2 = sc_tail ? gt
                          : resnet_conv2_args(kUnallocated, x.B, x.H, x.W, r.cout, r.c2.w, r.c2.b, kUnallocated, kUnallocated);
             TRY(gemm_choose(g2, true));
-            fuse2 = g2.splitk > 1;
+            fuse2 = to_next && g2.splitk > 1;
+            owe2 = !to_next && g2.splitk > 1;
             if (fuse2) {
                 *next_out = new_act(x.B, x.H, x.W, r.cout);
                 a2.nsplit = groupnorm_nsplit(x.B, x.H * x.W);
                 a2.partial = static_cast<float*>(alloc((size_t)x.B * a2.nsplit * m.cfg.norm_num_groups * 2 * sizeof(float)));
                 if (!next_out->p || !a2.partial) return 7;
             }
+            if (owe2) TRY(gemm_alloc_partial(g2, arena_alloc()));
         }
         const size_t mk = m.arena.mark();
         Act xn, h, hn;
@@ -304,10 +384,11 @@
                 TRY(launch_gemm<T>(g2, st));
                 a2.x0 = nullptr; a2.c0 = r.cout; a2.B = x.B; a2.HW = x.H * x.W; a2.groups = m.cfg.norm_num_groups; a2.eps = next_eps;
                 a2.gamma = next->g; a2.beta = next->b; a2.silu = 0; a2.y = next_out->p;
-                GnSlabSrc ss;
-                ss.partial = g2.partial; ss.splitk = g2.splitk; ss.alpha = g2.alpha; ss.bias = g2.bias; ss.resid = res.p; ss.ldr = r.cout; ss.raw_out = o.p;
-                TRY(launch_groupnorm_slabs(a2, ss, st));
-            }
+                TRY(gn_slabs_or_reduce(a2, g2, o.p, o.p));
+            }
+        } else if (owe2) {
+            g2.a0 = hn.p; g2.resid = res.p; g2.out = o.p;
+            TRY(launch_owing(g2, &o));
         } else if (sc_tail) {
             gt.a0 = hn.p;
             TRY(run_gemm(gt));
@@ -401,9 +482,24 @@
         const HeadBuf& hb = m.head_buf(x.H * x.W, C);
         Act o = new_act(x.B, x.H, x.W, C);
         if (!o.p) return 7;
+        GemmArgs gpo;
+        const bool composed = !(xw.ff2p && !m.keep && mlp_fused_ok(C, 4 * C, C)) && sizeof(T) == 2 && !m.keep && xw.ffpo && !xw.ff2.R &&
+                              !xw.proj_out.R && ff_proj_fused_enabled();
+        bool owe_po = false;
+        if (composed) {
+            ga_rows(gpo, kUnallocated, 4 * C, 4 * C); ga_rows2(gpo, kUnallocated, C, C); ga_weight(gpo, xw.ffpo, M, C, 5 * C); gpo.bias = xw.bffpo;
+            ga_resid(gpo, x.p, C); ga_out(gpo, o.p, C);
+            gpo.no_rp = 1;
+            gpo.alg_flops = 2.0 * M * (double)C * (5 * C);
+            if (may_owe(C, x.H * x.W, x.B)) {
+                TRY(gemm_choose(gpo, true));
+                owe_po = gpo.splitk > 1;
+                if (owe_po) TRY(gemm_alloc_partial(gpo, arena_alloc()));
+            }
+        }
         const size_t mk = m.arena.mark();
         Act xn;
-        if (pre_normed && pre_normed->p) xn = *pre_normed;
+        if (pre_normed && pre_normed->p) { TRY(settle(x)); xn = *pre_normed; }
         else TRY(gn(x, nullptr, xw.norm, false, 1e-6f, &xn));
         T* t = static_cast<T*>(alloc((size_t)M * C * sizeof(T)));
         T* nrm = static_cast<T*>(alloc((size_t)M * C * sizeof(T)));
@@ -458,13 +554,10 @@
             } else {
                 TRY(linear(t, M, C, xw.ff1, ACT_GEGLU, nullptr, 0, nullptr, ff, 4 * C, nullptr, &xw.ln3, nrm));
             }
-            if (sizeof(T) == 2 && !m.keep && xw.ffpo && !xw.ff2.R && !xw.proj_out.R && ff_proj_fused_enabled()) {
-                GemmArgs g;
-                ga_rows(g, ff, 4 * C, 4 * C); ga_rows2(g, t, C, C); ga_weight(g, xw.ffpo, M, C, 5 * C); g.bias = xw.bffpo;
-                ga_resid(g, x.p, C); ga_out(g, o.p, C);
-                g.no_rp = 1;
-                g.alg_flops = 2.0 * M * (double)C * (5 * C);
-                TRY(run_gemm(g));
+            if (composed) {
+                gpo.a0 = ff; gpo.a1 = t;
+                if (owe_po) TRY(launch_owing(gpo, &o));
+                else TRY(run_gemm(gpo));
                 proj_done = true;
             } else {
                 TRY(linear(ff, M, 4 * C, xw.ff2, ACT_NONE, t, C, nullptr, t, C));
@@ -511,7 +604,7 @@
         return 0;
     }
 
-    int direct(const Act& x, const ConvW& cw, int stride, int act, const Act* add, Act* out) {
+    int direct(const Act& x, const ConvW& cw, int stride, int act, const Act* add, Act* out, bool x_nchw_f32 = false) {
         const int pad = cw.ks / 2;
         const int Ho = (x.H + 2 * pad - cw.ks) / stride + 1, Wo = (x.W + 2 * pad - cw.ks) / stride + 1;
         *out = new_act(x.B, Ho, Wo, cw.cout);
@@ -521,8 +614,24 @@
         a.x = x.p; a.w = cw.w; a.bias = cw.b; a.y = out->p; a.B = x.B; a.Hin = x.H; a.Win = x.W; a.Cin = x.C;
         a.Hout = Ho; a.Wout = Wo; a.Cout = cw.cout; a.ks = cw.ks; a.stride = stride; a.pad = pad; a.act = act;
         a.add = add ? add->p : nullptr;
+        a.x_nchw_f32 = x_nchw_f32 ? 1 : 0;
         if (dry) return 0;
         return launch_direct_conv<T>(a, st);
+    }
+    int conv_in(const mrisr_tensor& sample, const Act* add, Act* out) {
+        MRISR_REQUIRE(sample.ndim == 4, "expected a 4-D tensor");
+        Act s;
+        s.B = (int)sample.shape[0]; s.C = (int)sample.shape[1]; s.H = (int)sample.shape[2]; s.W = (int)sample.shape[3];
+        DirectConvArgs probe;
+        probe.B = s.B; probe.Hin = probe.Hout = s.H; probe.Win = probe.Wout = s.W; probe.Cin = s.C; probe.Cout = m.conv_in.cout; probe.ks = m.conv_in.ks;
+        if (sizeof(T) == 2 && !m.keep && step_edges_enabled() && sample.layout == MRISR_NCHW && sample.dtype == MRISR_F32 && m.conv_in.cin == s.C &&
+            direct_conv_takes_nchw_f32(probe, (int)sizeof(T))) {
+            if (!alloc(s.numel() * sizeof(T))) return 7;
+            s.p = sample.data;
+            return direct(s, m.conv_in, 1, ACT_NONE, add, out, true);
+        }
+        TRY(import_act(sample, &s, false));
+        return direct(s, m.conv_in, 1, ACT_NONE, add, out);
     }
 
     int import_act(const mrisr_tensor& t, Act* out, bool copy_if_nhwc) {
@@ -547,6 +656,7 @@
     int export_act(const Act& a, const mrisr_tensor& t, float scale) {
         MRISR_REQUIRE(t.ndim == 4 && t.shape[0] == a.B && t.shape[1] == a.C && t.shape[2] == a.H && t.shape[3] == a.W,
                       "output tensor shape mismatch");
+        TRY(settle(a));
         if (dry) return 0;
         if (t.layout == MRISR_NHWC) {
             MRISR_REQUIRE(t.dtype == m.cfg.compute_dtype && scale == 1.0f, "NHWC outputs: compute dtype, scale 1");
@@ -556,6 +666,7 @@
         return launch_nhwc_to_nchw<T>(a.p, t.data, t.dtype, a.B, a.C, a.H, a.W, scale, st);
     }
     int add_external(Act& x, const mrisr_tensor& t) {
+        TRY(settle_all());
         const size_t mk = m.arena.mark();
         Act r;
         TRY(import_act(t, &r, false));
@@ -588,7 +699,7 @@
             }
             if (lv.has_down && !done()) {
                 Act y;
-                TRY(conv3(x, nullptr, lv.down, 2, 0, nullptr, 0, 1, nullptr, ACT_NONE, &y));
+                TRY(conv3(x, nullptr, lv.down, 2, 0, nullptr, 0, 1, nullptr, ACT_NONE, &y, nullptr, true));
                 x = y;
                 skips->push_back(x);
             }
@@ -596,6 +707,7 @@
                 TRY(add_external(x, intrablock[ib++]));
             }
         }
+        if (last_skip >= 0) TRY(settle_all());
         *out = x;
         return 0;
     }
@@ -627,6 +739,7 @@
         MRISR_REQUIRE(!m.keep, "FreeU: not while a training forward is being recorded");
         MRISR_REQUIRE(x.B == sk.B && x.H == sk.H && x.W == sk.W, "FreeU: hidden and skip geometry differ");
         MRISR_REQUIRE(x.C % 16 == 0 && sk.C % 8 == 0, "FreeU: hidden channels must be a multiple of 16, skip channels of 8");
+        TRY(settle_all());
         if (dry) return 0;
         return launch_freeu<T>(x.p, sk.p, x.p, sk.p, x.B, x.H, x.W, x.C, sk.C, b, s, st);
     }
@@ -635,6 +748,7 @@
                      const mrisr_tensor* down_res, int n_down, const mrisr_tensor* mid_res,
                      const mrisr_tensor* intrablock, int n_intra, const mrisr_tensor& out, const UNetCache& fc = UNetCache()) {
         m.arena.reset();
+        owing_on = true;
         const int B = (int)sample.shape[0];
         const bool store = fc.mode == CACHE_STORE, use = fc.mode == CACHE_USE;
         const int q0 = m.num_skips() - 1 - fc.depth;
@@ -645,13 +759,13 @@
         if (ehs) TRY(set_context(*ehs));
         MRISR_REQUIRE(dry || m.ctx_valid, "no encoder_hidden_states given and none cached");
         TRY(time_embed(t_dev, t_scalar, B));
-        Act s, x;
-        TRY(import_act(sample, &s, false));
-        TRY(direct(s, m.conv_in, 1, ACT_NONE, nullptr, &x));
+        Act x;
+        TRY(conv_in(sample, nullptr, &x));
         std::vector<Act> skips;
         TRY(encoder(x, intrablock, n_intra, &skips, &x, use ? fc.depth : -1));
         if (n_down > 0) {
             MRISR_REQUIRE(n_down == (int)skips.size(), "down_block_additional_residuals count");
+            TRY(settle_all());
             for (int k = 0; k < n_down; ++k) {
                 if (skips[k].p == x.p) {
                     Act c = new_act(x.B, x.H, x.W, x.C);
@@ -672,10 +786,12 @@
                 if ((store || use) && q == q0) {
                     int64_t cs[4];
                     TRY(m.cache_shape(fc.depth, B, (int)sample.shape[2], (int)sample.shape[3], cs));
+                    TRY(settle(x));
                     if (store) {
                         MRISR_REQUIRE(x.B == cs[0] && x.C == cs[1] && x.H == cs[2] && x.W == cs[3], "feature cache shape");
                         if (!dry) MRISR_CHECK_HIP(hipMemcpyAsync(fc.p, x.p, x.numel() * sizeof(T), hipMemcpyDeviceToDevice, st));
                     } else {
+                        x.debt = nullptr;
                         x.p = fc.p; x.B = (int)cs[0]; x.C = (int)cs[1]; x.H = (int)cs[2]; x.W = (int)cs[3];
                     }
                 }
@@ -700,6 +816,25 @@
         }
         Act xn, y;
         TRY(gn(x, nullptr, m.norm_out, true, m.cfg.norm_eps, &xn));
+        if (m.conv_out.cout % 4 == 0 && sizeof(T) == 2 && !m.keep && step_edges_enabled() && out.layout == MRISR_NCHW && out.dtype == MRISR_F32) {
+            MRISR_REQUIRE(m.conv_out.cin == xn.C && m.conv_out.ks == 3, "conv_out weight mismatch");
+            MRISR_REQUIRE(out.ndim == 4 && out.shape[0] == xn.B && out.shape[1] == m.conv_out.cout && out.shape[2] == xn.H && out.shape[3] == xn.W,
+                          "output tensor shape mismatch");
+            GemmArgs g = conv3_args(xn, nullptr, m.conv_out, 1, 0, nullptr, 0, 1, nullptr, ACT_NONE);
+            y = new_act(xn.B, xn.H, xn.W, m.conv_out.cout);
+            if (!y.p) return 7;
+            g.out = y.p;
+            TRY(gemm_choose(g, true));
+            TRY(gemm_alloc_partial(g, arena_alloc()));
+            if (dry) return 0;
+            if (g.splitk > 1) {
+                g.defer_reduce = 1;
+                TRY(launch_gemm<T>(g, st));
+                return launch_splitk_reduce_nchw(g, static_cast<float*>(out.data), xn.H * xn.W, 1.0f, st);
+            }
+            TRY(launch_gemm<T>(g, st));
+            return export_act(y, out, 1.0f);
+        }
         if (m.conv_out.cout % 4 == 0) TRY(conv3(xn, nullptr, m.conv_out, 1, 0, nullptr, 0, 1, nullptr, ACT_NONE, &y));
         else TRY(direct(xn, m.conv_out, 1, ACT_NONE, nullptr, &y));
         return export_act(y, out, 1.0f);
@@ -728,20 +863,21 @@
                            const mrisr_tensor* cond, float scale, mrisr_tensor* down_out, int n_down,
                            mrisr_tensor* mid_out) {
         m.arena.reset();
+        owing_on = true;
         const int B = (int)sample.shape[0];
         if (ehs) TRY(set_context(*ehs));
         if (cond) TRY(set_cond(*cond));
         MRISR_REQUIRE(dry || (m.ctx_valid && m.cond_valid), "context / condition image neither given nor cached");
         TRY(time_embed(t_dev, t_scalar, B));
-        Act s, x;
-        TRY(import_act(sample, &s, false));
+        Act x;
         Act ce;
-        ce.p = m.cond_emb; ce.B = B; ce.H = s.H; ce.W = s.W; ce.C = m.cfg.block_out_channels[0];
-        TRY(direct(s, m.conv_in, 1, ACT_NONE, &ce, &x));
+        ce.p = m.cond_emb; ce.B = B; ce.H = (int)sample.shape[2]; ce.W = (int)sample.shape[3]; ce.C = m.cfg.block_out_channels[0];
+        TRY(conv_in(sample, &ce, &x));
         std::vector<Act> skips;
         TRY(encoder(x, nullptr, 0, &skips, &x));
         TRY(mid(x, &x));
         MRISR_REQUIRE(n_down == (int)skips.size(), "ControlNet output count");
+        TRY(settle_all());
         for (int k = 0; k < n_down; ++k) {
             const size_t mk = m.arena.mark();
             Act o = new_act(skips[k].B, skips[k].H, skips[k].W, skips[k].C);
diff --git a/mri-diffusion-superresolution_amd/csrc/runtime.h b/mri-diffusion-superresolution_amd/csrc/runtime.h
--- a/mri-diffusion-superresolution_amd/csrc/runtime.h
+++ b/mri-diffusion-superresolution_amd/csrc/runtime.h
@@ -110,6 +110,7 @@
 struct Act {
     void* p = nullptr;
     int B = 0, H = 0, W = 0, C = 0;
+    struct SlabDebt* debt = nullptr;
     size_t rows() const { return (size_t)B * H * W; }
     size_t numel() const { return rows() * C; }
 };
diff --git a/mri-diffusion-superresolution_amd/csrc/sampler.hip b/mri-diffusion-superresolution_amd/csrc/sampler.hip
--- a/mri-diffusion-superresolution_amd/csrc/sampler.hip
+++ b/mri-diffusion-superresolution_amd/csrc/sampler.hip
@@ -375,6 +375,11 @@
 struct mrisr_model : public Model {};
 
 __global__ void load_t_kernel(long long* cur_t, const long long* table, const int* step) { *cur_t = table[*step]; }
+__global__ void advance_load_t_kernel(int* step, long long* cur_t, const long long* table, int n) {
+    const int s = *step + 1;
+    *step = s;
+    if (s < n) *cur_t = table[s];
+}
 
 static int g_temb_table = -1;
 extern "C" void mrisr_debug_temb_table(int on) { g_temb_table = on; }
@@ -794,6 +799,8 @@
     p.d_step = static_cast<int*>(s->d_step.p);
     p.d_curt = static_cast<long long*>(s->d_curt.p);
     p.d_ts = static_cast<const long long*>(s->d_ts.p);
+    p.n_ts = s->n_steps;
+    p.edges = step_edges_enabled() ? 1 : 0;
     if (s->kind == MRISR_STEP_DDPM) p.clip = s->clip;
     if (guided) { p.guidance_scale = s->guidance_scale; p.guidance_rescale = s->guidance_rescale; }
     if (pag) { p.pag_mask = s->pag_mask; p.pag_scale = s->pag_scale; }
@@ -895,6 +902,8 @@
     }
     MRISR_CHECK_HIP(hipMemsetAsync(s->d_step.p, 0, 16, st));
     MRISR_CHECK_HIP(hipMemcpyAsync(s->d_step.p, &s->first, sizeof(int), hipMemcpyHostToDevice, st));
+    if (s->first < s->n_steps)
+        MRISR_CHECK_HIP(hipMemcpyAsync(s->d_curt.p, static_cast<const long long*>(s->d_ts.p) + s->first, sizeof(long long), hipMemcpyDeviceToDevice, st));
     return 0;
 }
 
@@ -940,7 +949,7 @@
     UNetCache fc;
     fc.mode = cache_mode; fc.depth = p.cache_depth; fc.p = p.d_cache;
 
-    hipLaunchKernelGGL(load_t_kernel, dim3(1), dim3(1), 0, st, p.d_curt, p.d_ts, static_cast<const int*>(p.d_step));
+    if (!p.edges) hipLaunchKernelGGL(load_t_kernel, dim3(1), dim3(1), 0, st, p.d_curt, p.d_ts, static_cast<const int*>(p.d_step));
     if (tiled) TRY(launch_tile_gather(canvas, p.d_xt, tg, NB, p.C, st));
     if (p.cnet) TRY(C->forward_controlnet(&xin, &tt, nullptr, nullptr, 1.0f, res, p.n_res, &res[p.n_res], st));
     TRY(U.forward_unet(&xin, &tt, nullptr, p.cnet ? res : nullptr, p.n_res, p.cnet ? &res[p.n_res] : nullptr, intra, p.n_intra, &eps_t, st,
@@ -959,7 +968,10 @@
         TRY(launch_ddpm_step(p.x, p.d_eps, p.noise, p.d_coef, p.d_step, p.clip, n, st));
     else
         TRY(launch_resshift_step(p.x, p.d_eps, p.lr, p.noise, p.d_coef, p.d_step, n, st));
-    return launch_advance_step(p.d_step, st);
+    if (!p.edges) return launch_advance_step(p.d_step, st);
+    hipLaunchKernelGGL(advance_load_t_kernel, dim3(1), dim3(1), 0, st, p.d_step, p.d_curt, p.d_ts, p.n_ts);
+    MRISR_CHECK_HIP(hipGetLastError());
+    return 0;
 }
 
 static int run_steps(mrisr_sampler* s, const StepPlan& p, int use_graph, hipStream_t st) {
diff --git a/mri-diffusion-superresolution_amd/csrc/step_plan.h b/mri-diffusion-superresolution_amd/csrc/step_plan.h
--- a/mri-diffusion-superresolution_amd/csrc/step_plan.h
+++ b/mri-diffusion-superresolution_amd/csrc/step_plan.h
@@ -57,6 +57,8 @@
     int n_disabled;
     int disabled[32];
     int cdt;
+    int n_ts;
+    int edges;
 };
 #pragma GCC diagnostic pop
 static_assert(std::is_trivially_copyable<StepPlan>::value, "StepPlan is compared and copied as bytes");
diff --git a/mri-diffusion-superresolution_amd/mrisr/_lib.py b/mri-diffusion-superresolution_amd/mrisr/_lib.py
--- a/mri-diffusion-superresolution_amd/mrisr/_lib.py
+++ b/mri-diffusion-superresolution_amd/mrisr/_lib.py
@@ -60,7 +60,7 @@
     "mrisr_sampler_set_guidance", "mrisr_sampler_run_guided", "mrisr_sampler_set_cache", "mrisr_unet_cache_shape", "mrisr_unet_forward_cached", "mrisr_op_guided_step", "mrisr_sampler_set_solver", "mrisr_op_multistep_step",
     "mrisr_model_set_pag", "mrisr_model_num_transformer_blocks", "mrisr_sampler_set_pag", "mrisr_sampler_run_pag", "mrisr_sampler_num_captures",
     "mrisr_op_attn_identity", "mrisr_op_pag_step", "mrisr_op_pag_multistep_step",
-    "mrisr_model_set_freeu", "mrisr_op_freeu",
+    "mrisr_model_set_freeu", "mrisr_op_freeu", "mrisr_op_groupnorm_slabs",
     "mrisr_tile_tables", "mrisr_sampler_set_tiles", "mrisr_op_tile_gather", "mrisr_op_tile_blend",
     "mrisr_adapter_train_prepare", "mrisr_adapter_train_num_trainable", "mrisr_adapter_train_num_tensors",
     "mrisr_adapter_train_tensor_info", "mrisr_adapter_train_bind", "mrisr_adapter_train_refresh", "mrisr_adapter_backward", "mrisr_adapter_backward_level", "mrisr_adapter_train_level_range",
@@ -142,6 +142,7 @@
         L.mrisr_op_pag_multistep_step.argtypes = [I, P, P, P, P, P, P, P, I, I, F, F, F, P]
         L.mrisr_model_set_freeu.argtypes = [P, I, F, F, F, F]
         L.mrisr_op_freeu.argtypes = [I, P, P, P, P, I, I, I, I, I, F, F, P]
+        L.mrisr_op_groupnorm_slabs.argtypes = [P, I, P, P, I, I, P, P, I, I, I, I, P, P, I, F, I, I, P, P, P]
         L.mrisr_resize_scratch_bytes.restype = C.c_size_t
         L.mrisr_resize_scratch_bytes.argtypes = [C.c_int] * 6
         L.mrisr_resize_slices.argtypes = [C.c_void_p, C.c_int, C.c_int, C.c_int, C.c_void_p, C.c_int, C.c_int, C.c_int, C.c_void_p,
```

After: 66.92 slices/s, median of 2. No clear change (-0.0%).
